# sota-zk-labs/zkp-implementation

Hardware: AMD Instinct MI355X
Metric: G1 MSM scalar-muls/sec (higher is better)
Workload: dtype u32 (unsaturated 28-bit-limb Montgomery, 381-bit Fq; 64-bit accumulate)

## Files before the change

include/zkp_hip.h:

```cpp
#ifndef ZKP_HIP_H
#define ZKP_HIP_H
#include <stddef.h>
#include <stdint.h>

#ifdef __cplusplus
extern "C" {
#endif

#define ZKP_OK 0
#define ZKP_E_ARG (-1)
#define ZKP_E_NOMEM (-2)
#define ZKP_E_DEVICE (-3)
#define ZKP_E_SIZE (-4)

typedef struct zkp_bases zkp_bases;

int zkp_init(int device);
int zkp_init_devices(const int *devices, int n_devices);
int zkp_device_count(void);
int zkp_set_device(int slot);
void zkp_shutdown(void);
const char *zkp_last_error(void);
int zkp_abi_version(void);

void zkp_profile_enable(int on);
void zkp_profile_reset(void);
int zkp_profile_read(const char *name, double *total_ms, uint64_t *count);
int zkp_profile_clock_read(const char *name, uint64_t *cycles, uint64_t *ref_ticks, uint64_t *waves);
int zkp_probe_mad_rate(unsigned launches, double *lane_mads_per_s, double *clock_mhz, double *ms_per_launch);

int zkp_g1_bases_create(const uint64_t *xy, const uint8_t *is_inf, size_t n, zkp_bases **out);
int zkp_g1_bases_create_dev(const void *d_xy, const uint8_t *d_is_inf, size_t n, void *stream, zkp_bases **out);
int zkp_g1_bases_precompute(zkp_bases *b, unsigned window_bits);
size_t zkp_g1_bases_len(const zkp_bases *b);
int zkp_g1_bases_info(const zkp_bases *b, unsigned *window_bits, unsigned *slices);
void zkp_g1_bases_destroy(zkp_bases *b);

int zkp_msm_g1(const zkp_bases *bases, const uint64_t *scalars, size_t n, uint64_t out_xy[12], uint8_t *out_is_inf);
int zkp_msm_g1_dev(const zkp_bases *bases, const void *d_scalars, size_t n, void *stream, uint64_t out_xy[12],
                   uint8_t *out_is_inf);
int zkp_msm_g1_batch_dev(const zkp_bases *bases, const void *const *d_scalars, size_t count, size_t n, void *stream,
                         uint64_t *out_xy, uint8_t *out_is_inf);
int zkp_msm_g1_partial_dev(const zkp_bases *bases, const void *d_scalars, size_t n, void *stream, uint64_t out_xyzz[24]);
int zkp_msm_g1_partial(const zkp_bases *bases, const uint64_t *scalars, size_t n, uint64_t out_xyzz[24]);
int zkp_g1_bases_shard_count(const zkp_bases *b);
int zkp_g1_bases_shard(const zkp_bases *b, size_t i, int *slot, int *device, size_t *offset, size_t *len);
int zkp_msm_g1_sharded_dev(const zkp_bases *bases, const void *const *d_scalars, size_t n, uint64_t out_xy[12],
                           uint8_t *out_is_inf);
int zkp_msm_g1_sharded_dev_after(const zkp_bases *bases, const void *const *d_scalars, void *const *ready_events, size_t n,
                                 uint64_t out_xy[12], uint8_t *out_is_inf);
int zkp_g1_xyzz_sum(const uint64_t *partials, size_t count, uint64_t out_xy[12], uint8_t *out_is_inf);

int zkp_kzg_commit(const zkp_bases *srs, const uint64_t *coeffs, size_t len, uint64_t out_xy[12], uint8_t *out_is_inf);
int zkp_kzg_open(const zkp_bases *srs, const uint64_t *coeffs, size_t len, const uint64_t z[4], uint64_t out_xy[12],
                 uint8_t *out_is_inf, uint64_t out_eval[4]);

int zkp_g1_mul(const uint64_t base_xy[12], uint8_t base_is_inf, const uint64_t scalar[4], uint64_t out_xy[12],
               uint8_t *out_is_inf);
int zkp_g1_fixed_base_mul_dev(const void *d_scalars, size_t n, void *d_out_xy, uint8_t *d_out_is_inf, void *stream);
int zkp_selftest_fq_inverse_dev(const void *d_in, size_t n, int form, void *d_out, void *stream);
int zkp_srs_g1(const uint64_t secret[4], size_t n, uint64_t *out_xy);

int zkp_ntt_fr(uint64_t *data, unsigned log_n, int inverse, const uint64_t *coset );
int zkp_ntt_fr_dev(void *d_data, unsigned log_n, size_t batch, int inverse, const uint64_t *coset, void *stream);

int zkp_ntt_fr_twiddle_dev(void *d_data, size_t rows, size_t cols, size_t row0, unsigned log_n, int inverse, void *stream);

typedef struct {
    unsigned lo_bits, mid_bits;
    size_t mid_stride, hi_stride, batch_stride;
} zkp_ntt_layout;
int zkp_ntt_fr_axis0_dev(const void *d_in, void *d_out, unsigned log_len, size_t cols, int inverse, unsigned tw_log_n,
                         size_t tw_col0, void *stream);
int zkp_ntt_fr_layout_dev(const void *d_in, void *d_out, unsigned log_n, size_t batch, int inverse,
                          const zkp_ntt_layout *in_layout, const zkp_ntt_layout *out_layout, unsigned tw_log_n, size_t tw_row0,
                          void *stream);

#define ZKP_NTT_NATURAL 0
#define ZKP_NTT_K1SLAB 1
#define ZKP_NTT_COLUMNS 2
typedef struct {
    unsigned slots, log_n1, log_n2, chunks;
    size_t r1, r2, cw, slab;
} zkp_ntt_shard_geometry;
int zkp_ntt_fr_sharded_geometry(unsigned log_n, unsigned slots , unsigned chunks,
                                zkp_ntt_shard_geometry *out);
int zkp_ntt_fr_sharded_dev(void *const *d_slabs, unsigned log_n, int inverse, int layout_in, int layout_out, unsigned chunks,
                           void *const *streams);
int zkp_ntt_fr_sharded(uint64_t *data, unsigned log_n, int inverse, const uint64_t *coset );

int zkp_ntt_goldilocks(uint64_t *data, unsigned log_n, int inverse, const uint64_t *coset );
int zkp_ntt_goldilocks_dev(void *d_data, unsigned log_n, size_t batch, int inverse, const uint64_t *coset, void *stream);
int zkp_fri_layer_eval(const uint64_t *coeffs, size_t d, uint64_t coset, unsigned log_D, uint64_t *out);
int zkp_fri_fold(const uint64_t *coeffs, size_t d, uint64_t r, uint64_t *out);

size_t zkp_fri_merkle_node_count(size_t n);
int zkp_fri_merkle_tree(const uint64_t *leaves, size_t n, uint64_t *nodes_out);
int zkp_fri_merkle_tree_dev(const void *d_leaves, size_t n, void *d_nodes, void *stream);
int zkp_fri_challenges(const uint64_t *roots, size_t layers, uint64_t const_val, size_t num_queries, uint64_t *r_out,
                       uint64_t *q_out);
int zkp_fri_prove(const uint64_t *coeffs, size_t d, size_t blowup_factor, size_t num_queries, uint64_t **out_proof,
                  size_t *out_words);
int zkp_fri_verify(const uint64_t *proof, size_t words);
void zkp_free(void *p);

int zkp_fri_layer_eval_fr(const uint64_t *coeffs, size_t d, const uint64_t coset[4], unsigned log_D, uint64_t *out);
int zkp_fri_fold_fr(const uint64_t *coeffs, size_t d, const uint64_t r[4], uint64_t *out);
int zkp_fri_merkle_tree_fr(const uint64_t *leaves, size_t n, uint64_t *nodes_out);
int zkp_fri_merkle_tree_fr_dev(const void *d_leaves, size_t n, void *d_nodes, void *stream);
int zkp_fri_challenges_fr(const uint64_t *roots, size_t layers, const uint64_t const_val[4], size_t num_queries, uint64_t *r_out,
                          uint64_t *q_out);
int zkp_fri_prove_fr(const uint64_t *coeffs, size_t d, size_t blowup_factor, size_t num_queries, uint64_t **out_proof,
                     size_t *out_words);
int zkp_fri_verify_fr(const uint64_t *proof, size_t words);

typedef struct zkp_plonk_transcript zkp_plonk_transcript;
int zkp_plonk_transcript_create(zkp_plonk_transcript **out);
void zkp_plonk_transcript_destroy(zkp_plonk_transcript *t);
int zkp_plonk_transcript_feed(zkp_plonk_transcript *t, const uint64_t xy[12], uint8_t is_inf);
int zkp_plonk_transcript_challenges(zkp_plonk_transcript *t, size_t n, uint64_t *out);

int zkp_poly_mul_fr(const uint64_t *a, size_t la, const uint64_t *b, size_t lb, uint64_t *out);

typedef struct zkp_plonk_prover zkp_plonk_prover;
int zkp_plonk_prover_create(const zkp_bases *srs, unsigned log_n, const uint64_t *const polys[12], const size_t lens[12],
                            const uint64_t k1[4], const uint64_t k2[4], zkp_plonk_prover **out);
void zkp_plonk_prover_destroy(zkp_plonk_prover *p);
int zkp_plonk_round1(zkp_plonk_prover *p, const uint64_t *blinders, uint64_t *out_xy, uint8_t *out_is_inf);
int zkp_plonk_round2(zkp_plonk_prover *p, const uint64_t beta[4], const uint64_t gamma[4], const uint64_t *blinders,
                     uint64_t out_xy[12], uint8_t *out_is_inf);
int zkp_plonk_round3(zkp_plonk_prover *p, const uint64_t alpha[4], uint64_t *out_xy, uint8_t *out_is_inf, size_t *out_degree);
int zkp_plonk_round4(zkp_plonk_prover *p, const uint64_t zeta[4], uint64_t *out_bars);
int zkp_plonk_round5(zkp_plonk_prover *p, const uint64_t v[4], uint64_t *out_xy, uint8_t *out_is_inf);
typedef struct {
    uint64_t commit_xy[9][12];
    uint8_t commit_is_inf[9];
    uint64_t bars[6][4];
    uint64_t u[4];
    uint64_t degree;
} zkp_plonk_proof;
int zkp_plonk_prove(zkp_plonk_prover *p, const uint64_t *blinders, zkp_plonk_proof *out);

int zkp_g2_generator(uint64_t out_xy[24]);
int zkp_g2_mul(const uint64_t q_xy[24], uint8_t q_is_inf, const uint64_t scalar[4], uint64_t out_xy[24], uint8_t *out_is_inf);
int zkp_pairing(const uint64_t p_xy[12], uint8_t p_is_inf, const uint64_t q_xy[24], uint8_t q_is_inf, uint64_t out_fq12[72]);
int zkp_kzg_verify(const uint64_t g2s_xy[24], const uint64_t commit_xy[12], uint8_t commit_is_inf, const uint64_t w_xy[12],
                   uint8_t w_is_inf, const uint64_t y[4], const uint64_t z[4], int *accepted);
int zkp_kzg_batch_verify(const uint64_t g2s_xy[24], size_t n, const uint64_t *commits_xy, const uint8_t *commits_is_inf,
                         const uint64_t *points, const uint64_t *openings_xy, const uint8_t *openings_is_inf,
                         const uint64_t *evals, const uint64_t *r_primes, int *accepted);
int zkp_kzg_aggregate_commitments(const uint64_t *commits_xy, const uint8_t *commits_is_inf, size_t n, const uint64_t challenge[4],
                                  uint64_t out_xy[12], uint8_t *out_is_inf);
int zkp_plonk_verify(zkp_plonk_prover *p, const uint64_t g2s_xy[24], const zkp_plonk_proof *proof, int *accepted);

int zkp_plonk_get_poly(zkp_plonk_prover *p, int which, uint64_t *out, size_t cap_elems, size_t *len);

typedef struct zkp_nova_r1cs zkp_nova_r1cs;
typedef struct {
    const uint64_t *row_ptr;
    const uint32_t *cols;
    const uint64_t *vals;
} zkp_csr;
int zkp_nova_r1cs_create(const zkp_bases *srs, size_t rows, size_t num_vars, size_t num_io, const zkp_csr *a, const zkp_csr *b,
                         const zkp_csr *c, zkp_nova_r1cs **out);
void zkp_nova_r1cs_destroy(zkp_nova_r1cs *r);
typedef struct {
    uint64_t com_e_xy[12];
    uint8_t com_e_is_inf;
    uint64_t u[4];
    uint64_t com_w_xy[12];
    uint8_t com_w_is_inf;
    uint64_t *x;
} zkp_nova_instance;
typedef struct {
    uint64_t r[4];
    uint64_t opening_point[4];
    uint64_t open_e_xy[12];
    uint8_t open_e_is_inf;
    uint64_t eval_e[4];
    uint64_t open_w_xy[12];
    uint8_t open_w_is_inf;
    uint64_t eval_w[4];
} zkp_nova_proof;
int zkp_nova_cross_term_dev(zkp_nova_r1cs *r, const void *d_w1, const uint64_t *x1, const uint64_t u1[4], const void *d_w2,
                            const uint64_t *x2, const uint64_t u2[4], void *d_t, void *stream);
int zkp_nova_fold_witness_dev(zkp_nova_r1cs *r, const uint64_t rr[4], const void *d_e1, const void *d_w1, const void *d_e2,
                              const void *d_w2, const void *d_t, void *d_e_out, void *d_w_out, void *stream);
int zkp_nova_relaxed_residual_dev(zkp_nova_r1cs *r, const void *d_w, const uint64_t *x, const uint64_t u[4], const void *d_e,
                                  void *stream, uint64_t *bad_rows);

typedef struct zkp_nova_transcript zkp_nova_transcript;
int zkp_nova_transcript_create(zkp_nova_transcript **out);
void zkp_nova_transcript_destroy(zkp_nova_transcript *t);
int zkp_nova_transcript_feed(zkp_nova_transcript *t, const uint64_t xy[12], uint8_t is_inf);
int zkp_nova_transcript_feed_scalar(zkp_nova_transcript *t, const uint64_t s[4]);
int zkp_nova_transcript_challenges(zkp_nova_transcript *t, size_t n, uint64_t *out);

int zkp_nova_nifs_prover_dev(zkp_nova_r1cs *r, const void *d_e1, const void *d_w1, const void *d_e2, const void *d_w2,
                             const zkp_nova_instance *fi1, const zkp_nova_instance *fi2, zkp_nova_transcript *t, void *d_e_out,
                             void *d_w_out, void *stream, zkp_nova_instance *out, uint64_t com_t_xy[12], uint8_t *com_t_is_inf,
                             uint64_t r_out[4]);
int zkp_nova_nifs_prover(zkp_nova_r1cs *r, const uint64_t *e1, const uint64_t *w1, const uint64_t *e2, const uint64_t *w2,
                         const zkp_nova_instance *fi1, const zkp_nova_instance *fi2, zkp_nova_transcript *t, uint64_t *e_out,
                         uint64_t *w_out, zkp_nova_instance *out, uint64_t com_t_xy[12], uint8_t *com_t_is_inf, uint64_t r_out[4]);
int zkp_nova_nifs_prove_dev(zkp_nova_r1cs *r, const uint64_t rr[4], const void *d_e, const void *d_w, const zkp_nova_instance *fi,
                            zkp_nova_transcript *t, void *stream, zkp_nova_proof *out);
int zkp_nova_nifs_prove(zkp_nova_r1cs *r, const uint64_t rr[4], const uint64_t *e, const uint64_t *w, const zkp_nova_instance *fi,
                        zkp_nova_transcript *t, zkp_nova_proof *out);
int zkp_nova_nifs_verify(const uint64_t g2s_xy[24], const zkp_nova_proof *proof, const zkp_nova_instance *fi1,
                         const zkp_nova_instance *fi2, const zkp_nova_instance *fi3, const uint64_t com_t_xy[12], uint8_t com_t_is_inf,
                         zkp_nova_transcript *t, int *accepted);

#ifdef __cplusplus
}
#endif
#endif
```

rust/zkp-hip-sys/src/lib.rs:

```rust
#![allow(non_camel_case_types)]
use core::ffi::{c_char, c_void};

pub const ZKP_OK: i32 = 0;
pub const ZKP_E_ARG: i32 = -1;
pub const ZKP_E_NOMEM: i32 = -2;
pub const ZKP_E_DEVICE: i32 = -3;
pub const ZKP_E_SIZE: i32 = -4;

#[repr(C)] pub struct zkp_bases { _private: [u8; 0] }
#[repr(C)] pub struct zkp_plonk_prover { _private: [u8; 0] }
#[repr(C)] pub struct zkp_plonk_transcript { _private: [u8; 0] }
#[repr(C)] pub struct zkp_nova_r1cs { _private: [u8; 0] }
#[repr(C)] pub struct zkp_nova_transcript { _private: [u8; 0] }

#[repr(C)]
pub struct zkp_plonk_proof {
    pub commit_xy: [[u64; 12]; 9],
    pub commit_is_inf: [u8; 9],
    pub bars: [[u64; 4]; 6],
    pub u: [u64; 4],
    pub degree: u64,
}

#[repr(C)]
pub struct zkp_ntt_layout {
    pub lo_bits: u32,
    pub mid_bits: u32,
    pub mid_stride: usize,
    pub hi_stride: usize,
    pub batch_stride: usize,
}

#[repr(C)]
pub struct zkp_ntt_shard_geometry {
    pub slots: u32,
    pub log_n1: u32,
    pub log_n2: u32,
    pub chunks: u32,
    pub r1: usize,
    pub r2: usize,
    pub cw: usize,
    pub slab: usize,
}
#[repr(C)]
pub struct zkp_csr {
    pub row_ptr: *const u64,
    pub cols: *const u32,
    pub vals: *const u64,
}

#[repr(C)]
pub struct zkp_nova_instance {
    pub com_e_xy: [u64; 12],
    pub com_e_is_inf: u8,
    pub u: [u64; 4],
    pub com_w_xy: [u64; 12],
    pub com_w_is_inf: u8,
    pub x: *mut u64,
}

#[repr(C)]
pub struct zkp_nova_proof {
    pub r: [u64; 4],
    pub opening_point: [u64; 4],
    pub open_e_xy: [u64; 12],
    pub open_e_is_inf: u8,
    pub eval_e: [u64; 4],
    pub open_w_xy: [u64; 12],
    pub open_w_is_inf: u8,
    pub eval_w: [u64; 4],
}

pub const ZKP_NTT_NATURAL: i32 = 0;
pub const ZKP_NTT_K1SLAB: i32 = 1;
pub const ZKP_NTT_COLUMNS: i32 = 2;

extern "C" {
    pub fn zkp_init(device: i32) -> i32;
    pub fn zkp_init_devices(devices: *const i32, n_devices: i32) -> i32;
    pub fn zkp_device_count() -> i32;
    pub fn zkp_set_device(slot: i32) -> i32;
    pub fn zkp_shutdown();
    pub fn zkp_last_error() -> *const c_char;
    pub fn zkp_abi_version() -> i32;
    pub fn zkp_profile_enable(on: i32);
    pub fn zkp_profile_reset();
    pub fn zkp_profile_read(name: *const c_char, total_ms: *mut f64, count: *mut u64) -> i32;
    pub fn zkp_profile_clock_read(name: *const c_char, cycles: *mut u64, ref_ticks: *mut u64, waves: *mut u64) -> i32;
    pub fn zkp_probe_mad_rate(launches: u32, lane_mads_per_s: *mut f64, clock_mhz: *mut f64, ms_per_launch: *mut f64) -> i32;
    pub fn zkp_g1_bases_create(xy: *const u64, is_inf: *const u8, n: usize, out: *mut *mut zkp_bases) -> i32;
    pub fn zkp_g1_bases_create_dev(d_xy: *const c_void, d_is_inf: *const u8, n: usize, stream: *mut c_void, out: *mut *mut zkp_bases) -> i32;
    pub fn zkp_g1_bases_precompute(b: *mut zkp_bases, window_bits: u32) -> i32;
    pub fn zkp_g1_bases_len(b: *const zkp_bases) -> usize;
    pub fn zkp_g1_bases_info(b: *const zkp_bases, window_bits: *mut u32, slices: *mut u32) -> i32;
    pub fn zkp_g1_bases_destroy(b: *mut zkp_bases);
    pub fn zkp_msm_g1(bases: *const zkp_bases, scalars: *const u64, n: usize, out_xy: *mut u64, out_is_inf: *mut u8) -> i32;
    pub fn zkp_msm_g1_dev(bases: *const zkp_bases, d_scalars: *const c_void, n: usize, stream: *mut c_void, out_xy: *mut u64, out_is_inf: *mut u8) -> i32;
    pub fn zkp_msm_g1_batch_dev(bases: *const zkp_bases, d_scalars: *const *const c_void, count: usize, n: usize, stream: *mut c_void, out_xy: *mut u64, out_is_inf: *mut u8) -> i32;
    pub fn zkp_msm_g1_partial_dev(bases: *const zkp_bases, d_scalars: *const c_void, n: usize, stream: *mut c_void, out_xyzz: *mut u64) -> i32;
    pub fn zkp_msm_g1_partial(bases: *const zkp_bases, scalars: *const u64, n: usize, out_xyzz: *mut u64) -> i32;
    pub fn zkp_g1_bases_shard_count(b: *const zkp_bases) -> i32;
    pub fn zkp_g1_bases_shard(b: *const zkp_bases, i: usize, slot: *mut i32, device: *mut i32, offset: *mut usize, len: *mut usize) -> i32;
    pub fn zkp_msm_g1_sharded_dev(bases: *const zkp_bases, d_scalars: *const *const c_void, n: usize, out_xy: *mut u64, out_is_inf: *mut u8) -> i32;
    pub fn zkp_msm_g1_sharded_dev_after(bases: *const zkp_bases, d_scalars: *const *const c_void, ready_events: *mut *mut c_void, n: usize, out_xy: *mut u64, out_is_inf: *mut u8) -> i32;
    pub fn zkp_g1_xyzz_sum(partials: *const u64, count: usize, out_xy: *mut u64, out_is_inf: *mut u8) -> i32;
    pub fn zkp_kzg_commit(srs: *const zkp_bases, coeffs: *const u64, len: usize, out_xy: *mut u64, out_is_inf: *mut u8) -> i32;
    pub fn zkp_kzg_open(srs: *const zkp_bases, coeffs: *const u64, len: usize, z: *const u64, out_xy: *mut u64, out_is_inf: *mut u8, out_eval: *mut u64) -> i32;
    pub fn zkp_g1_mul(base_xy: *const u64, base_is_inf: u8, scalar: *const u64, out_xy: *mut u64, out_is_inf: *mut u8) -> i32;
    pub fn zkp_g1_fixed_base_mul_dev(d_scalars: *const c_void, n: usize, d_out_xy: *mut c_void, d_out_is_inf: *mut u8, stream: *mut c_void) -> i32;
    pub fn zkp_selftest_fq_inverse_dev(d_in: *const c_void, n: usize, form: i32, d_out: *mut c_void, stream: *mut c_void) -> i32;
    pub fn zkp_srs_g1(secret: *const u64, n: usize, out_xy: *mut u64) -> i32;
    pub fn zkp_ntt_fr(data: *mut u64, log_n: u32, inverse: i32, coset: *const u64) -> i32;
    pub fn zkp_ntt_fr_dev(d_data: *mut c_void, log_n: u32, batch: usize, inverse: i32, coset: *const u64, stream: *mut c_void) -> i32;
    pub fn zkp_ntt_fr_twiddle_dev(d_data: *mut c_void, rows: usize, cols: usize, row0: usize, log_n: u32, inverse: i32, stream: *mut c_void) -> i32;
    pub fn zkp_ntt_fr_axis0_dev(d_in: *const c_void, d_out: *mut c_void, log_len: u32, cols: usize, inverse: i32, tw_log_n: u32, tw_col0: usize, stream: *mut c_void) -> i32;
    pub fn zkp_ntt_fr_layout_dev(d_in: *const c_void, d_out: *mut c_void, log_n: u32, batch: usize, inverse: i32, in_layout: *const zkp_ntt_layout, out_layout: *const zkp_ntt_layout, tw_log_n: u32, tw_row0: usize, stream: *mut c_void) -> i32;
    pub fn zkp_ntt_fr_sharded_geometry(log_n: u32, slots: u32, chunks: u32, out: *mut zkp_ntt_shard_geometry) -> i32;
    pub fn zkp_ntt_fr_sharded_dev(d_slabs: *mut *mut c_void, log_n: u32, inverse: i32, layout_in: i32, layout_out: i32, chunks: u32, streams: *mut *mut c_void) -> i32;
    pub fn zkp_ntt_fr_sharded(data: *mut u64, log_n: u32, inverse: i32, coset: *const u64) -> i32;
    pub fn zkp_ntt_goldilocks(data: *mut u64, log_n: u32, inverse: i32, coset: *const u64) -> i32;
    pub fn zkp_ntt_goldilocks_dev(d_data: *mut c_void, log_n: u32, batch: usize, inverse: i32, coset: *const u64, stream: *mut c_void) -> i32;
    pub fn zkp_fri_layer_eval(coeffs: *const u64, d: usize, coset: u64, log_D: u32, out: *mut u64) -> i32;
    pub fn zkp_fri_fold(coeffs: *const u64, d: usize, r: u64, out: *mut u64) -> i32;
    pub fn zkp_fri_merkle_node_count(n: usize) -> usize;
    pub fn zkp_fri_merkle_tree(leaves: *const u64, n: usize, nodes_out: *mut u64) -> i32;
    pub fn zkp_fri_merkle_tree_dev(d_leaves: *const c_void, n: usize, d_nodes: *mut c_void, stream: *mut c_void) -> i32;
    pub fn zkp_fri_challenges(roots: *const u64, layers: usize, const_val: u64, num_queries: usize, r_out: *mut u64, q_out: *mut u64) -> i32;
    pub fn zkp_fri_prove(coeffs: *const u64, d: usize, blowup_factor: usize, num_queries: usize, out_proof: *mut *mut u64, out_words: *mut usize) -> i32;
    pub fn zkp_fri_verify(proof: *const u64, words: usize) -> i32;
    pub fn zkp_free(p: *mut c_void);
    pub fn zkp_fri_layer_eval_fr(coeffs: *const u64, d: usize, coset: *const u64, log_D: u32, out: *mut u64) -> i32;
    pub fn zkp_fri_fold_fr(coeffs: *const u64, d: usize, r: *const u64, out: *mut u64) -> i32;
    pub fn zkp_fri_merkle_tree_fr(leaves: *const u64, n: usize, nodes_out: *mut u64) -> i32;
    pub fn zkp_fri_merkle_tree_fr_dev(d_leaves: *const c_void, n: usize, d_nodes: *mut c_void, stream: *mut c_void) -> i32;
    pub fn zkp_fri_challenges_fr(roots: *const u64, layers: usize, const_val: *const u64, num_queries: usize, r_out: *mut u64, q_out: *mut u64) -> i32;
    pub fn zkp_fri_prove_fr(coeffs: *const u64, d: usize, blowup_factor: usize, num_queries: usize, out_proof: *mut *mut u64, out_words: *mut usize) -> i32;
    pub fn zkp_fri_verify_fr(proof: *const u64, words: usize) -> i32;
    pub fn zkp_plonk_transcript_create(out: *mut *mut zkp_plonk_transcript) -> i32;
    pub fn zkp_plonk_transcript_destroy(t: *mut zkp_plonk_transcript);
    pub fn zkp_plonk_transcript_feed(t: *mut zkp_plonk_transcript, xy: *const u64, is_inf: u8) -> i32;
    pub fn zkp_plonk_transcript_challenges(t: *mut zkp_plonk_transcript, n: usize, out: *mut u64) -> i32;
    pub fn zkp_poly_mul_fr(a: *const u64, la: usize, b: *const u64, lb: usize, out: *mut u64) -> i32;
    pub fn zkp_plonk_prover_create(srs: *const zkp_bases, log_n: u32, polys: *const *const u64, lens: *const usize, k1: *const u64, k2: *const u64, out: *mut *mut zkp_plonk_prover) -> i32;
    pub fn zkp_plonk_prover_destroy(p: *mut zkp_plonk_prover);
    pub fn zkp_plonk_round1(p: *mut zkp_plonk_prover, blinders: *const u64, out_xy: *mut u64, out_is_inf: *mut u8) -> i32;
    pub fn zkp_plonk_round2(p: *mut zkp_plonk_prover, beta: *const u64, gamma: *const u64, blinders: *const u64, out_xy: *mut u64, out_is_inf: *mut u8) -> i32;
    pub fn zkp_plonk_round3(p: *mut zkp_plonk_prover, alpha: *const u64, out_xy: *mut u64, out_is_inf: *mut u8, out_degree: *mut usize) -> i32;
    pub fn zkp_plonk_round4(p: *mut zkp_plonk_prover, zeta: *const u64, out_bars: *mut u64) -> i32;
    pub fn zkp_plonk_round5(p: *mut zkp_plonk_prover, v: *const u64, out_xy: *mut u64, out_is_inf: *mut u8) -> i32;
    pub fn zkp_plonk_prove(p: *mut zkp_plonk_prover, blinders: *const u64, out: *mut zkp_plonk_proof) -> i32;
    pub fn zkp_g2_generator(out_xy: *mut u64) -> i32;
    pub fn zkp_g2_mul(q_xy: *const u64, q_is_inf: u8, scalar: *const u64, out_xy: *mut u64, out_is_inf: *mut u8) -> i32;
    pub fn zkp_pairing(p_xy: *const u64, p_is_inf: u8, q_xy: *const u64, q_is_inf: u8, out_fq12: *mut u64) -> i32;
    pub fn zkp_kzg_verify(g2s_xy: *const u64, commit_xy: *const u64, commit_is_inf: u8, w_xy: *const u64, w_is_inf: u8, y: *const u64, z: *const u64, accepted: *mut i32) -> i32;
    pub fn zkp_kzg_batch_verify(g2s_xy: *const u64, n: usize, commits_xy: *const u64, commits_is_inf: *const u8, points: *const u64, openings_xy: *const u64, openings_is_inf: *const u8, evals: *const u64, r_primes: *const u64, accepted: *mut i32) -> i32;
    pub fn zkp_kzg_aggregate_commitments(commits_xy: *const u64, commits_is_inf: *const u8, n: usize, challenge: *const u64, out_xy: *mut u64, out_is_inf: *mut u8) -> i32;
    pub fn zkp_plonk_verify(p: *mut zkp_plonk_prover, g2s_xy: *const u64, proof: *const zkp_plonk_proof, accepted: *mut i32) -> i32;
    pub fn zkp_plonk_get_poly(p: *mut zkp_plonk_prover, which: i32, out: *mut u64, cap_elems: usize, len: *mut usize) -> i32;
    pub fn zkp_nova_r1cs_create(srs: *const zkp_bases, rows: usize, num_vars: usize, num_io: usize, a: *const zkp_csr, b: *const zkp_csr, c: *const zkp_csr, out: *mut *mut zkp_nova_r1cs) -> i32;
    pub fn zkp_nova_r1cs_destroy(r: *mut zkp_nova_r1cs);
    pub fn zkp_nova_cross_term_dev(r: *mut zkp_nova_r1cs, d_w1: *const c_void, x1: *const u64, u1: *const u64, d_w2: *const c_void, x2: *const u64, u2: *const u64, d_t: *mut c_void, stream: *mut c_void) -> i32;
    pub fn zkp_nova_fold_witness_dev(r: *mut zkp_nova_r1cs, rr: *const u64, d_e1: *const c_void, d_w1: *const c_void, d_e2: *const c_void, d_w2: *const c_void, d_t: *const c_void, d_e_out: *mut c_void, d_w_out: *mut c_void, stream: *mut c_void) -> i32;
    pub fn zkp_nova_relaxed_residual_dev(r: *mut zkp_nova_r1cs, d_w: *const c_void, x: *const u64, u: *const u64, d_e: *const c_void, stream: *mut c_void, bad_rows: *mut u64) -> i32;
    pub fn zkp_nova_transcript_create(out: *mut *mut zkp_nova_transcript) -> i32;
    pub fn zkp_nova_transcript_destroy(t: *mut zkp_nova_transcript);
    pub fn zkp_nova_transcript_feed(t: *mut zkp_nova_transcript, xy: *const u64, is_inf: u8) -> i32;
    pub fn zkp_nova_transcript_feed_scalar(t: *mut zkp_nova_transcript, s: *const u64) -> i32;
    pub fn zkp_nova_transcript_challenges(t: *mut zkp_nova_transcript, n: usize, out: *mut u64) -> i32;
    pub fn zkp_nova_nifs_prover_dev(r: *mut zkp_nova_r1cs, d_e1: *const c_void, d_w1: *const c_void, d_e2: *const c_void, d_w2: *const c_void, fi1: *const zkp_nova_instance, fi2: *const zkp_nova_instance, t: *mut zkp_nova_transcript, d_e_out: *mut c_void, d_w_out: *mut c_void, stream: *mut c_void, out: *mut zkp_nova_instance, com_t_xy: *mut u64, com_t_is_inf: *mut u8, r_out: *mut u64) -> i32;
    pub fn zkp_nova_nifs_prover(r: *mut zkp_nova_r1cs, e1: *const u64, w1: *const u64, e2: *const u64, w2: *const u64, fi1: *const zkp_nova_instance, fi2: *const zkp_nova_instance, t: *mut zkp_nova_transcript, e_out: *mut u64, w_out: *mut u64, out: *mut zkp_nova_instance, com_t_xy: *mut u64, com_t_is_inf: *mut u8, r_out: *mut u64) -> i32;
    pub fn zkp_nova_nifs_prove_dev(r: *mut zkp_nova_r1cs, rr: *const u64, d_e: *const c_void, d_w: *const c_void, fi: *const zkp_nova_instance, t: *mut zkp_nova_transcript, stream: *mut c_void, out: *mut zkp_nova_proof) -> i32;
    pub fn zkp_nova_nifs_prove(r: *mut zkp_nova_r1cs, rr: *const u64, e: *const u64, w: *const u64, fi: *const zkp_nova_instance, t: *mut zkp_nova_transcript, out: *mut zkp_nova_proof) -> i32;
    pub fn zkp_nova_nifs_verify(g2s_xy: *const u64, proof: *const zkp_nova_proof, fi1: *const zkp_nova_instance, fi2: *const zkp_nova_instance, fi3: *const zkp_nova_instance, com_t_xy: *const u64, com_t_is_inf: u8, t: *mut zkp_nova_transcript, accepted: *mut i32) -> i32;
}

pub fn last_error() -> String {
    unsafe { std::ffi::CStr::from_ptr(zkp_last_error()).to_string_lossy().into_owned() }
}
```

zkp-implementation_amd/build.py:

```python
#!/usr/bin/env python3
import os
import subprocess
import sys

HERE = os.path.dirname(os.path.abspath(__file__))
SRC = os.path.join(HERE, "csrc")
OUT = os.path.join(HERE, "libzkp_hip.so")
SOURCES = ["api.hip"]
DEPS = ["api.hip", "ff.hpp", "fq28.hpp", "fq28_inv.hpp", "fr29.hpp", "fr29_mul2_asm.inc", "fq28_mul_asm.inc", "fq28_mul2x_asm.inc", "fq28_sqr_asm.inc", "fq28_mul2_asm.inc", "g1.hpp", "g1_28.hpp", "msm.hpp", "ntt.hpp", "plonk.hpp",
        "plonk_host.inc", "ntt_sharded.inc", "fri.hpp", "fri_host.inc", "fri_fr.hpp", "fri_fr_host.inc", "transcript_host.hpp", "pairing_host.hpp", "verify_host.inc", "host_ff.hpp", "kzg_host.hpp", "host_threads.hpp", "msm_plan.hpp", "msm_host.inc", "nova.hpp", "nova_host.inc", "dev_res.hpp",
        os.path.join("..", "..", "include", "zkp_hip.h")]


STAMP = OUT + ".srchash"


def source_hash():
    import hashlib
    h = hashlib.sha256()
    for d in DEPS:
        path = os.path.join(SRC, d)
        if os.path.exists(path):
            h.update(d.encode())
            h.update(open(path, "rb").read())
    return h.hexdigest()


def stale():
    if not os.path.exists(OUT) or not os.path.exists(STAMP):
        return True
    return open(STAMP).read().strip() != source_hash()


def build(force=False, verbose=False, defines=(), out=None):
    variant = out is not None
    if not variant and not force and not stale():
        return OUT
    hipcc = os.environ.get("HIPCC", "/opt/rocm/bin/hipcc")
    cmd = [hipcc, "--offload-arch=gfx950", "-O3", "-std=c++17", "-fPIC", "-shared",
           "-Wno-unused-result", "-pthread"] + [f"-D{d}" for d in defines] + [os.path.join(SRC, s) for s in SOURCES] + ["-o", out or OUT]
    if verbose:
        print(" ".join(cmd))
    subprocess.check_call(cmd)
    if not variant:
        with open(STAMP, "w") as f:
            f.write(source_hash())
    return out or OUT


if __name__ == "__main__":
    defs = [a[2:] for a in sys.argv[1:] if a.startswith("-D")]
    outs = [a[2:] for a in sys.argv[1:] if a.startswith("-o")]
    print(build(force="--force" in sys.argv, verbose=True, defines=defs, out=outs[0] if outs else None))
```

zkp-implementation_amd/csrc/api.hip:

```cpp
#include <hip/hip_runtime.h>

#include <algorithm>
#include <array>
#include <atomic>
#include <chrono>
#include <cstdio>
#include <cstdlib>
#include <cstring>
#include <condition_variable>
#include <functional>
#include <map>
#include <memory>
#include <mutex>
#include <new>
#include <string>
#include <thread>
#include <tuple>
#include <vector>

#include "../../include/zkp_hip.h"
#include "host_ff.hpp"
#include "kzg_host.hpp"
#include "msm.hpp"
#include "ntt.hpp"
#include "plonk.hpp"
#include "nova.hpp"
#include "fri.hpp"
#include "transcript_host.hpp"
#include "pairing_host.hpp"

using namespace zkp;
using namespace zkp::host;

namespace {

thread_local std::string g_err;

int fail(int code, const std::string& msg) {
    g_err = msg;
    return code;
}

int on_exception() noexcept {
    try {
        throw;
    } catch (const std::bad_alloc&) {
        try { g_err = "host allocation failed"; } catch (...) {}
        return ZKP_E_NOMEM;
    } catch (const std::exception& e) {
        try { g_err = std::string("internal error: ") + e.what(); } catch (...) {}
        return ZKP_E_DEVICE;
    } catch (...) {
        try { g_err = "internal error: unknown exception"; } catch (...) {}
        return ZKP_E_DEVICE;
    }
}
#define ZKP_CATCH_INT catch (...) { return on_exception(); }

#define HIPCHK(expr)                                                                                        \
    do {                                                                                                    \
        hipError_t e_ = (expr);                                                                             \
        if (e_ != hipSuccess)                                                                               \
            return fail(e_ == hipErrorOutOfMemory ? ZKP_E_NOMEM : ZKP_E_DEVICE,                             \
                        std::string(#expr) + ": " + hipGetErrorString(e_));                                 \
    } while (0)
int hip_fail(hipError_t e, const std::string& what) {
    return fail(e == hipErrorOutOfMemory ? ZKP_E_NOMEM : ZKP_E_DEVICE, what + hipGetErrorString(e));
}
#define HIPCHK_BARE(expr)                            \
    do {                                             \
        hipError_t e_ = (expr);                      \
        if (e_ != hipSuccess) return hip_fail(e_, ""); \
    } while (0)
#define ZCHK(expr)             \
    do {                       \
        int r_ = (expr);       \
        if (r_ != ZKP_OK) return r_; \
    } while (0)

#include "host_threads.hpp"
#include "dev_res.hpp"
static_assert(ZKP_HOST_THREADS_E_DEVICE == ZKP_E_DEVICE && ZKP_HOST_THREADS_OK == ZKP_OK, "host_threads.hpp error codes");

class DeviceWorkers {
    struct W {
        std::thread th;
        std::mutex mu;
        std::condition_variable cv;
        const std::function<void()>* job = nullptr;
        bool busy = false, quit = false;
    };
    std::mutex run_mu;
    std::vector<W*> ws;
    static void loop(W* w) {
        std::unique_lock<std::mutex> lk(w->mu);
        for (;;) {
            w->cv.wait(lk, [&] { return w->job != nullptr || w->quit; });
            if (w->quit) return;
            const std::function<void()>* j = w->job;
            lk.unlock();
            (*j)();
            lk.lock();
            w->job = nullptr;
            w->busy = false;
            w->cv.notify_all();
        }
    }

public:
    void run(const std::vector<std::function<void()>>& jobs) {
        std::lock_guard<std::mutex> one(run_mu);
        while (ws.size() < jobs.size()) {
            W* w = new W;
            w->th = std::thread(loop, w);
            ws.push_back(w);
        }
        for (size_t i = 0; i < jobs.size(); i++) {
            std::lock_guard<std::mutex> lk(ws[i]->mu);
            ws[i]->job = &jobs[i];
            ws[i]->busy = true;
            ws[i]->cv.notify_all();
        }
        for (size_t i = 0; i < jobs.size(); i++) {
            std::unique_lock<std::mutex> lk(ws[i]->mu);
            ws[i]->cv.wait(lk, [&] { return !ws[i]->busy; });
        }
    }
    void stop() {
        std::lock_guard<std::mutex> one(run_mu);
        for (W* w : ws) {
            {
                std::lock_guard<std::mutex> lk(w->mu);
                w->quit = true;
                w->cv.notify_all();
            }
            w->th.join();
            delete w;
        }
        ws.clear();
    }
};
DeviceWorkers g_workers;
void device_workers_stop() { g_workers.stop(); }

struct ProfRec {
    const char* name = nullptr;
    hipEvent_t a = nullptr;
    Event own_a, b;
    double host_ms = 0;
};
std::atomic<int> g_prof_on{0};
struct Ctx;
Ctx& ctx();
std::vector<ProfRec>& prof_records();
hipStream_t& prof_last_stream();

struct ProfScope {
    ProfRec rec;
    hipStream_t st;
    bool on;
    ProfScope(const char* name, hipStream_t s, bool chain = false) : st(s), on(false) {
        const int level = g_prof_on.load(std::memory_order_relaxed);
        on = level == 1 || (level == 2 && std::strcmp(name, "msm_accumulate") == 0);
        if (!on) return;
        if (level == 2) chain = false;
        rec.name = name;
        std::vector<ProfRec>& recs = prof_records();
        if (chain && !recs.empty() && recs.back().b && prof_last_stream() == s) {
            rec.a = recs.back().b;
            if (rec.b.make(hipEventDefault) != hipSuccess) on = false;
            return;
        }
        if (rec.own_a.make(hipEventDefault) != hipSuccess || rec.b.make(hipEventDefault) != hipSuccess) { on = false; return; }
        rec.a = rec.own_a;
        (void)hipEventRecord(rec.a, st);
    }
    ~ProfScope() {
        if (!on) return;
        (void)hipEventRecord(rec.b, st);
        prof_records().push_back(std::move(rec));
        prof_last_stream() = st;
    }
};
void prof_host(const char* name, double ms) {
    if (g_prof_on.load(std::memory_order_relaxed) != 1) return;
    ProfRec r;
    r.name = name;
    r.host_ms = ms;
    prof_records().push_back(std::move(r));
}

template <class F> struct HostField;
template <> struct HostField<Fr> {
    typedef HFr H;
    static Fr dev(const HFr& x) { Fr r; std::memcpy(r.l, x.l, 32); return r; }
    static Fr29 tw(const HFr& x) {
        HFr y = x;
        for (int i = 0; i < 5; i++) y = y.dbl();
        Fr29 r;
        for (int i = 0; i < 9; i++) {
            const int bit = 29 * i, w = bit >> 6, sh = bit & 63;
            unsigned __int128 v = y.l[w];
            if (w + 1 < 4) v |= (unsigned __int128)y.l[w + 1] << 64;
            r.l[i] = (uint32_t)(v >> sh) & MASK29;
        }
        return r;
    }
    static HFr root(unsigned log_n) { return fr_root_of_unity(log_n); }
    static constexpr int ID = 0;
};
template <> struct HostField<Gl> {
    typedef HGl H;
    static Gl dev(const HGl& x) { return Gl{x.from_mont().l[0]}; }
    static Gl tw(const HGl& x) { return dev(x); }
    static HGl root(unsigned log_n) { return gl_root_of_unity(log_n); }
    static constexpr int ID = 1;
};

template <class F>
struct NttPlan {
    unsigned log_n = 0;
    int passes = 0;
    int r[4] = {0, 0, 0, 0};
    const typename NttOps<F>::W* tw[4] = {nullptr, nullptr, nullptr, nullptr};
    TypedBuf<typename NttOps<F>::W> inter_lo, inter_hi;
    TypedBuf<typename NttOps<F>::W> inter_lo_ninv;
    uint32_t h = 0;
    TypedBuf<typename NttOps<F>::W> direct[4];
    TypedBuf<F> tw_matrix[2];
    typename HostField<F>::H n_inv;
};

template <class F>
struct CosetCache {
    bool valid = false;
    unsigned log_n = 0;
    int inverse = 0;
    uint64_t key[4] = {0, 0, 0, 0};
    uint64_t ckey[4] = {0, 0, 0, 0};
    TypedBuf<typename NttOps<F>::W> lo, hi;
    uint32_t h = 0;
};

struct Ctx {
    int slot = 0;
    int device = -1;
    std::mutex mu;
    Stream stream;
    Stream copy_stream;
    Stream sort_stream;
    Stream xstream;
    Event ws_event;
    hipStream_t ws_stream = nullptr;
    bool ws_pending = false;
    std::vector<ProfRec> prof;
    hipStream_t prof_last = nullptr;
    std::map<std::pair<int, int>, DevBuf> radix_tw[2];
    std::map<std::pair<unsigned, int>, NttPlan<Fr>> plans_fr;
    std::map<std::pair<unsigned, int>, NttPlan<Gl>> plans_gl;
    static constexpr int COSET_WAYS = 8;
    CosetCache<Fr> coset_fr[COSET_WAYS];
    CosetCache<Gl> coset_gl[COSET_WAYS];
    unsigned coset_victim[2] = {0, 0};
    DevBuf ntt_scratch;
    std::map<std::pair<unsigned, int>, DevBuf> axis0_tw[2];
    DevBuf scalars, over;
    TypedBuf<uint32_t> digits, sorted, counts, start, perm, result;
    TypedBuf<uint2> entries;
    TypedBuf<uint4> pieces, buckets, parts, pyr1, odd0, odd1;
    PinnedBuf host_result;
    PinnedBuf fri_small;
    DevBuf fb_table;
    bool fb_ready = false;
    DevBuf tmp;
    Event copy_event;
    std::vector<Event> copy_events;
    Event ev_sort[2], ev_acc[2], ev_begin;
    DevBuf fri_arena, fri_meta;
    DevBuf clk;
    uint32_t tail_max_waves = 2048;
    DevBuf xchg_a, xchg_b;
    std::vector<Event> xev;
    bool peers_enabled = false;
    ~Ctx() {
        std::lock_guard<std::mutex> lk(mu);
        (void)hipSetDevice(device);
        (void)hipDeviceSynchronize();
    }
};
enum { CLK_MSM_ACCUMULATE = 0, CLK_MAD_PROBE = 1, CLK_NTT_FR = 2, CLK_NTT_GL = 3, CLK_COUNT = 4 };
static const char* const kClkNames[CLK_COUNT] = {"msm_accumulate", "mad_probe", "ntt_fr_pass", "ntt_gl_pass"};

struct Runtime {
    std::mutex mu;
    std::vector<std::unique_ptr<Ctx>> slots;
    bool multi = false;
};
Runtime& g_rt = *new Runtime;

ClkRec* clk_record(int which) {
    if (!g_prof_on.load(std::memory_order_relaxed)) return nullptr;
    Ctx& c = ctx();
    if (!c.clk.p) {
        if (c.clk.ensure(sizeof(ClkRec) * CLK_COUNT) != ZKP_OK) return nullptr;
        if (hipMemset(c.clk.p, 0, sizeof(ClkRec) * CLK_COUNT) != hipSuccess) return nullptr;
    }
    return reinterpret_cast<ClkRec*>(c.clk.p) + which;
}
thread_local int t_slot = -1;
thread_local Ctx* t_cur = nullptr;
Ctx& ctx() { return *t_cur; }
std::vector<ProfRec>& prof_records() { return ctx().prof; }
hipStream_t& prof_last_stream() { return ctx().prof_last; }

int create_slot_locked(int device);

struct CtxScope {
    Ctx* prev;
    std::unique_lock<std::mutex> lk;
    int rc = ZKP_OK;
    int restore_device = -1;
    explicit CtxScope(int slot) : prev(t_cur) {
        Ctx* c = nullptr;
        {
            std::lock_guard<std::mutex> g(g_rt.mu);
            if (g_rt.slots.empty()) {
                int dev = 0;
                if (hipGetDevice(&dev) != hipSuccess) dev = 0;
                rc = create_slot_locked(dev);
                if (rc != ZKP_OK) return;
            }
            const int s = slot >= 0 ? slot : (t_slot >= 0 ? t_slot : 0);
            if (s >= (int)g_rt.slots.size()) {
                rc = fail(ZKP_E_ARG, "device slot out of range (zkp_init_devices / zkp_set_device)");
                return;
            }
            c = g_rt.slots[(size_t)s].get();
        }
        lk = std::unique_lock<std::mutex>(c->mu);
        t_cur = c;
        int cur = -1;
        if (hipGetDevice(&cur) == hipSuccess && cur != c->device) restore_device = cur;
        if (cur != c->device && hipSetDevice(c->device) != hipSuccess) rc = fail(ZKP_E_DEVICE, "hipSetDevice failed");
    }
    ~CtxScope() {
        t_cur = prev;
        if (restore_device >= 0 && !prev) (void)hipSetDevice(restore_device);
    }
};
#define CTX_ENTER(slot)           \
    CtxScope ctx_scope_(slot);    \
    if (ctx_scope_.rc != ZKP_OK) return ctx_scope_.rc

struct WsOrder {
    hipStream_t st;
    explicit WsOrder(hipStream_t s) : st(s) {
        Ctx& c = ctx();
        if (c.ws_pending && c.ws_stream != st) (void)hipStreamWaitEvent(st, c.ws_event, 0);
    }
    ~WsOrder() {
        Ctx& c = ctx();
        if (c.ws_event.make(hipEventDisableTiming) != hipSuccess) {
            (void)hipStreamSynchronize(st);
            c.ws_pending = false;
            return;
        }
        (void)hipEventRecord(c.ws_event, st);
        c.ws_stream = st;
        c.ws_pending = true;
    }
};

template <class K>
int allow_big_lds(K kernel) {
    HIPCHK(hipFuncSetAttribute(reinterpret_cast<const void*>(kernel), hipFuncAttributeMaxDynamicSharedMemorySize,
                               160 * 1024));
    return ZKP_OK;
}

template <class F>
std::map<std::pair<unsigned, int>, NttPlan<F>>& plan_map();
template <> std::map<std::pair<unsigned, int>, NttPlan<Fr>>& plan_map<Fr>() { return ctx().plans_fr; }
template <> std::map<std::pair<unsigned, int>, NttPlan<Gl>>& plan_map<Gl>() { return ctx().plans_gl; }
template <class F> CosetCache<F>* coset_cache();
template <> CosetCache<Fr>* coset_cache<Fr>() { return ctx().coset_fr; }
template <> CosetCache<Gl>* coset_cache<Gl>() { return ctx().coset_gl; }

template <class F>
int make_pow_table(const typename HostField<F>::H& base, const typename HostField<F>::H& c, uint32_t shift,
                   uint32_t count, typename NttOps<F>::W* out, hipStream_t st) {
    hipLaunchKernelGGL(pow_table_kernel<F>, dim3((count + 255) / 256), dim3(256), 0, st, HostField<F>::dev(base),
                       HostField<F>::dev(c), shift, count, out);
    HIPCHK(hipGetLastError());
    return ZKP_OK;
}

template <class F>
int build_pow_table(const typename HostField<F>::H& w, uint32_t count, DevBuf* out, hipStream_t st) {
    typedef typename NttOps<F>::W W;
    DevBuf tab;
    ZCHK(tab.ensure(sizeof(W) * count));
    int rc = make_pow_table<F>(w, HostField<F>::H::one(), 0, count, static_cast<W*>(tab.p), st);
    if (rc == ZKP_OK) {
        const hipError_t e = hipStreamSynchronize(st);
        if (e != hipSuccess) rc = hip_fail(e, "hipStreamSynchronize(st): ");
    }
    if (rc != ZKP_OK) {
        (void)hipStreamSynchronize(st);
        return rc;
    }
    *out = std::move(tab);
    return ZKP_OK;
}

template <class F>
int get_radix_table(int log_r, int inverse, const typename NttOps<F>::W** out, hipStream_t st) {
    typedef typename HostField<F>::H H;
    typedef typename NttOps<F>::W W;
    auto& m = ctx().radix_tw[HostField<F>::ID];
    auto key = std::make_pair(log_r, inverse);
    auto it = m.find(key);
    if (it == m.end()) {
        uint32_t count = log_r ? (1u << (log_r - 1)) : 1u;
        H w = HostField<F>::root((unsigned)log_r);
        if (inverse) w = w.inverse();
        DevBuf tab;
        ZCHK(build_pow_table<F>(w, count, &tab, st));
        it = m.emplace(key, std::move(tab)).first;
    }
    *out = static_cast<const W*>(it->second.p);
    return ZKP_OK;
}

static unsigned pass0_matrix_max_log() {
    static const unsigned v = [] {
        const char* e = getenv("ZKP_NTT_TW_MATRIX_MAX_LOG");
        return e ? (unsigned)std::min(30, std::max(0, atoi(e))) : 24u;
    }();
    return v;
}

template <class F>
int get_plan(unsigned log_n, int inverse, bool allow_wide, NttPlan<F>** out, hipStream_t st) {
    typedef typename HostField<F>::H H;
    typedef typename NttOps<F>::W W;
    auto& m = plan_map<F>();
    auto key = std::make_pair(log_n, inverse | (allow_wide ? 2 : 0));
    auto it = m.find(key);
    if (it == m.end()) {
        NttPlan<F> pl;
        pl.log_n = log_n;
        pl.passes = (int)log_n <= NttOps<F>::MAX_TILE_LOG ? 1 : (int)((log_n + NttOps<F>::MAX_PASS_LOG - 1) / NttOps<F>::MAX_PASS_LOG);
        if (pl.passes > 1 && allow_wide && !getenv("ZKP_NTT_NO_WIDE_PASS")) {
            for (int maxr = NttOps<F>::MAX_PASS_LOG + 1; maxr <= NttOps<F>::WIDE_PASS_LOG; maxr++) {
                if ((int)log_n > NttOps<F>::wide_max_log_n(maxr)) break;
                const int wide = (int)((log_n + maxr - 1) / maxr);
                if (wide < pl.passes) pl.passes = wide;
            }
        }
        int base = (int)log_n / pl.passes, rem = (int)log_n % pl.passes;
        for (int p = 0; p < pl.passes; p++) pl.r[p] = base + (p < rem ? 1 : 0);
        for (int p = 0; p < pl.passes; p++) ZCHK(get_radix_table<F>(pl.r[p], inverse, &pl.tw[p], st));
        H w = HostField<F>::root(log_n);
        if (inverse) w = w.inverse();
        H two = H::from_u64(2), ninv = H::one(), half = two.inverse();
        for (unsigned i = 0; i < log_n; i++) ninv = ninv * half;
        pl.n_inv = ninv;
        if (pl.passes > 1) {
            pl.h = (log_n + 1) / 2;
            uint32_t nlo = 1u << pl.h, nhi = 1u << (log_n - pl.h);
            auto build = [&]() -> int {
                ZCHK(pl.inter_lo.ensure(sizeof(W) * nlo));
                ZCHK(pl.inter_hi.ensure(sizeof(W) * nhi));
                ZCHK(make_pow_table<F>(w, H::one(), 0, nlo, pl.inter_lo.get(), st));
                ZCHK(make_pow_table<F>(w, H::one(), pl.h, nhi, pl.inter_hi.get(), st));
                if (inverse) {
                    ZCHK(pl.inter_lo_ninv.ensure(sizeof(W) * nlo));
                    ZCHK(make_pow_table<F>(w, ninv, 0, nlo, pl.inter_lo_ninv.get(), st));
                }
                unsigned outer = pl.r[0];
                for (int p = 1; p + 1 < pl.passes; p++) {
                    const unsigned log_m = log_n - outer;
// ... 824 lines not shown
    }
    *out = b;
    return ZKP_OK;
} ZKP_CATCH_INT

int zkp_g1_bases_precompute(zkp_bases* b, unsigned window_bits) try {
    if (!b) return fail(ZKP_E_ARG, "null argument");
    if (b->shards.empty()) return precompute_single(b, window_bits);
    size_t nmax = 0, expanded = 0;
    for (const auto& sh : b->shards) nmax = std::max(nmax, sh->n), expanded += sh->pre_c ? 1 : 0;
    if (window_bits == 0) {
        if (expanded == b->shards.size() || !(window_bits = auto_window_bits(nmax))) return ZKP_OK;
        if (expanded) window_bits = b->shards[0]->pre_req ? b->shards[0]->pre_req : window_bits;
    }
    ZCHK(for_each_shard(b, [&](size_t i) { return precompute_single(b->shards[i].get(), window_bits, true); }));
    std::vector<uint8_t> was(b->shards.size());
    for (size_t i = 0; i < b->shards.size(); i++) was[i] = b->shards[i]->pre_c ? 1 : 0;
    const int rc = for_each_shard(b, [&](size_t i) { return precompute_single(b->shards[i].get(), window_bits); });
    if (rc != ZKP_OK) {
        const std::string why = zkp_last_error();
        bool mixed = false;
        for (size_t i = 0; i < b->shards.size(); i++)
            if (!was[i] && b->shards[i]->pre_c && unexpand_single(b->shards[i].get()) != ZKP_OK) mixed = true;
        return fail(rc, why + (mixed ? " -- and a finished chunk could not be rolled back: the handle is expanded in part (still usable)"
                                     : " -- every chunk is back to the plain points"));
    }
    return ZKP_OK;
} ZKP_CATCH_INT

size_t zkp_g1_bases_len(const zkp_bases* b) { return b ? b->n : 0; }

int zkp_g1_bases_info(const zkp_bases* b, unsigned* window_bits, unsigned* slices) try {
    if (!b || !window_bits || !slices) return fail(ZKP_E_ARG, "null argument");
    const zkp_bases* s = b->shards.empty() ? b : b->shards[0].get();
    if (!s) return fail(ZKP_E_ARG, "empty handle");
    *window_bits = s->pre_req;
    *slices = s->pre_c ? s->pre_planes : 0;
    return ZKP_OK;
} ZKP_CATCH_INT

void zkp_g1_bases_destroy(zkp_bases* b) {
    if (!b) return;
    for (auto& s : b->shards) zkp_g1_bases_destroy(s.release());
    DeviceRestore restore;
    (void)hipSetDevice(b->device);
    delete b;
}

}

namespace {

const char* const kShardedDev = "bases are sharded over several devices: device-pointer entries take single-device bases "
                                "(zkp_set_device + zkp_g1_bases_create*); use zkp_msm_g1 with host scalars";

int msm_host_scalars(const zkp_bases* bases, const uint64_t* scalars, size_t n, HXyzz* r) {
    CTX_ENTER(bases->slot);
    hipStream_t st = g_rt.multi ? ctx().stream : nullptr;
    WsOrder ord(st);
    if (n > bases->n) return fail(ZKP_E_SIZE, "more scalars than bases (kzg/src/scheme.rs:86)");
    *r = HXyzz::infinity();
    if (!n) return ZKP_OK;
    ZCHK(ctx().scalars.ensure(32 * n));
    const Fr* d_sc = reinterpret_cast<const Fr*>(ctx().scalars.p);
    const bool shared = bases->pre_c != 0;
    if (shared && n >= (1u << 19)) {
        ZCHK(ctx().copy_stream.ensure(hipStreamNonBlocking));
        ZCHK(ctx().copy_event.ensure(hipEventDisableTiming));
        const MsmFeed feed{scalars, ctx().copy_stream, ctx().copy_event, msm_feed_ranges(n)};
        return msm_partial_batch(bases, &d_sc, 1, n, st, r, &feed);
    }
    HIPCHK(hipMemcpyAsync(ctx().scalars.p, scalars, 32 * n, hipMemcpyHostToDevice, st));
    return msm_partial(bases, d_sc, n, st, r);
}

int msm_host_scalars_any(const zkp_bases* bases, const uint64_t* scalars, size_t n, HXyzz* r) {
    if (bases->shards.empty()) return msm_host_scalars(bases, scalars, n, r);
    if (n > bases->n) return fail(ZKP_E_SIZE, "more scalars than bases (kzg/src/scheme.rs:86)");
    const size_t k = bases->shards.size();
    std::vector<HXyzz> part(k, HXyzz::infinity());
    ZCHK(for_each_shard(bases, [&](size_t i) {
        const size_t lo = bases->shard_off[i];
        if (lo >= n) return (int)ZKP_OK;
        const size_t len = std::min(bases->shards[i]->n, n - lo);
        return msm_host_scalars(bases->shards[i].get(), scalars + 4 * lo, len, &part[i]);
    }));
    HXyzz acc = HXyzz::infinity();
    for (size_t i = 0; i < k; i++) acc = acc.add(part[i]);
    *r = acc;
    return ZKP_OK;
}

}

extern "C" {

int zkp_msm_g1_partial_dev(const zkp_bases* bases, const void* d_scalars, size_t n, void* stream, uint64_t out_xyzz[24]) try {
    if (!bases || !out_xyzz || (n && !d_scalars)) return fail(ZKP_E_ARG, "null argument");
    if (!bases->shards.empty()) return fail(ZKP_E_ARG, kShardedDev);
    CTX_ENTER(bases->slot);
    WsOrder ord(reinterpret_cast<hipStream_t>(stream));
    HXyzz r;
    ZCHK(msm_partial(bases, reinterpret_cast<const Fr*>(d_scalars), n, reinterpret_cast<hipStream_t>(stream), &r));
    r.store(out_xyzz);
    return ZKP_OK;
} ZKP_CATCH_INT

int zkp_msm_g1_dev(const zkp_bases* bases, const void* d_scalars, size_t n, void* stream, uint64_t out_xy[12],
                   uint8_t* out_is_inf) try {
    if (!bases || !out_xy || !out_is_inf || (n && !d_scalars)) return fail(ZKP_E_ARG, "null argument");
    if (!bases->shards.empty()) return fail(ZKP_E_ARG, kShardedDev);
    CTX_ENTER(bases->slot);
    WsOrder ord(reinterpret_cast<hipStream_t>(stream));
    HXyzz r;
    ZCHK(msm_partial(bases, reinterpret_cast<const Fr*>(d_scalars), n, reinterpret_cast<hipStream_t>(stream), &r));
    r.to_affine(out_xy, out_is_inf);
    return ZKP_OK;
} ZKP_CATCH_INT

int zkp_msm_g1(const zkp_bases* bases, const uint64_t* scalars, size_t n, uint64_t out_xy[12], uint8_t* out_is_inf) try {
    if (!bases || !out_xy || !out_is_inf || (n && !scalars)) return fail(ZKP_E_ARG, "null argument");
    HXyzz r;
    ZCHK(msm_host_scalars_any(bases, scalars, n, &r));
    r.to_affine(out_xy, out_is_inf);
    return ZKP_OK;
} ZKP_CATCH_INT

int zkp_g1_bases_shard_count(const zkp_bases* b) { return !b ? 0 : b->shards.empty() ? 1 : (int)b->shards.size(); }

int zkp_g1_bases_shard(const zkp_bases* b, size_t i, int* slot, int* device, size_t* offset, size_t* len) try {
    if (!b || !slot || !device || !offset || !len) return fail(ZKP_E_ARG, "null argument");
    if (i >= (size_t)zkp_g1_bases_shard_count(b)) return fail(ZKP_E_ARG, "chunk index out of range");
    const zkp_bases* s = b->shards.empty() ? b : b->shards[i].get();
    *slot = s->slot;
    *device = s->device;
    *offset = b->shards.empty() ? 0 : b->shard_off[i];
    *len = s->n;
    return ZKP_OK;
} ZKP_CATCH_INT

static int order_after_producer(hipStream_t st, void* ready_event) {
    if (ready_event) HIPCHK(hipStreamWaitEvent(st, reinterpret_cast<hipEvent_t>(ready_event), 0));
    else HIPCHK(hipDeviceSynchronize());
    return ZKP_OK;
}

int zkp_msm_g1_sharded_dev_after(const zkp_bases* bases, const void* const* d_scalars, void* const* ready_events, size_t n,
                                 uint64_t out_xy[12], uint8_t* out_is_inf) try {
    if (!bases || !out_xy || !out_is_inf || (n && !d_scalars)) return fail(ZKP_E_ARG, "null argument");
    if (n > bases->n) return fail(ZKP_E_SIZE, "more scalars than bases (kzg/src/scheme.rs:86)");
    HXyzz acc = HXyzz::infinity();
    if (bases->shards.empty()) {
        if (n) {
            if (!d_scalars[0]) return fail(ZKP_E_ARG, "null scalar pointer");
            CTX_ENTER(bases->slot);
            hipStream_t st = g_rt.multi ? ctx().stream : nullptr;
            ZCHK(order_after_producer(st, ready_events ? ready_events[0] : nullptr));
            WsOrder ord(st);
            ZCHK(msm_partial(bases, reinterpret_cast<const Fr*>(d_scalars[0]), n, st, &acc));
        }
    } else {
        const size_t k = bases->shards.size();
        for (size_t i = 0; i < k; i++)
            if (bases->shard_off[i] < n && bases->shards[i]->n && !d_scalars[i]) return fail(ZKP_E_ARG, "null scalar pointer for a chunk in use");
        std::vector<HXyzz> part(k, HXyzz::infinity());
        ZCHK(for_each_shard(bases, [&](size_t i) {
            const size_t lo = bases->shard_off[i];
            const zkp_bases* sh = bases->shards[i].get();
            if (lo >= n || !sh->n) return (int)ZKP_OK;
            const size_t len = std::min(sh->n, n - lo);
            CTX_ENTER(sh->slot);
            ZCHK(order_after_producer(ctx().stream, ready_events ? ready_events[i] : nullptr));
            WsOrder ord(ctx().stream);
            return msm_partial(sh, reinterpret_cast<const Fr*>(d_scalars[i]), len, ctx().stream, &part[i]);
        }));
        for (size_t i = 0; i < k; i++) acc = acc.add(part[i]);
    }
    acc.to_affine(out_xy, out_is_inf);
    return ZKP_OK;
} ZKP_CATCH_INT

int zkp_msm_g1_sharded_dev(const zkp_bases* bases, const void* const* d_scalars, size_t n, uint64_t out_xy[12],
                           uint8_t* out_is_inf) {
    return zkp_msm_g1_sharded_dev_after(bases, d_scalars, nullptr, n, out_xy, out_is_inf);
}

int zkp_msm_g1_partial(const zkp_bases* bases, const uint64_t* scalars, size_t n, uint64_t out_xyzz[24]) try {
    if (!bases || !out_xyzz || (n && !scalars)) return fail(ZKP_E_ARG, "null argument");
    HXyzz r;
    ZCHK(msm_host_scalars_any(bases, scalars, n, &r));
    r.store(out_xyzz);
    return ZKP_OK;
} ZKP_CATCH_INT

int zkp_msm_g1_batch_dev(const zkp_bases* bases, const void* const* d_scalars, size_t count, size_t n, void* stream,
                         uint64_t* out_xy, uint8_t* out_is_inf) try {
    if (!bases || (count && (!d_scalars || !out_xy || !out_is_inf))) return fail(ZKP_E_ARG, "null argument");
    if (!bases->shards.empty()) return fail(ZKP_E_ARG, kShardedDev);
    CTX_ENTER(bases->slot);
    WsOrder ord(reinterpret_cast<hipStream_t>(stream));
    std::vector<HXyzz> r(count);
    ZCHK(msm_partial_batch(bases, reinterpret_cast<const Fr* const*>(d_scalars), count, n, reinterpret_cast<hipStream_t>(stream),
                           r.data()));
    std::vector<HFq> prefix(count);
    HFq run = HFq::one();
    for (size_t m = 0; m < count; m++) {
        prefix[m] = run;
        if (!r[m].is_inf()) run = run * r[m].zzz;
    }
    HFq inv = run.inverse();
    for (size_t m = count; m-- > 0;) {
        if (r[m].is_inf()) {
            std::memset(out_xy + 12 * m, 0, 96);
            out_is_inf[m] = 1;
            continue;
        }
        const HFq zi3 = inv * prefix[m];
        inv = inv * r[m].zzz;
        HFq zi2 = zi3 * r[m].zz;
        zi2 = zi2.sqr();
        (r[m].x * zi2).store(out_xy + 12 * m);
        (r[m].y * zi3).store(out_xy + 12 * m + 6);
        out_is_inf[m] = 0;
    }
    return ZKP_OK;
} ZKP_CATCH_INT

int zkp_g1_xyzz_sum(const uint64_t* partials, size_t count, uint64_t out_xy[12], uint8_t* out_is_inf) try {
    if ((count && !partials) || !out_xy || !out_is_inf) return fail(ZKP_E_ARG, "null argument");
    HXyzz acc = HXyzz::infinity();
    for (size_t i = 0; i < count; i++) acc = acc.add(HXyzz::load(partials + 24 * i));
    acc.to_affine(out_xy, out_is_inf);
    return ZKP_OK;
} ZKP_CATCH_INT

int zkp_kzg_commit(const zkp_bases* srs, const uint64_t* coeffs, size_t len, uint64_t out_xy[12], uint8_t* out_is_inf) try {
    if (!srs || !out_xy || !out_is_inf || (len && !coeffs)) return fail(ZKP_E_ARG, "null argument");
    KzgScheme scheme(srs);
    KzgCommitment cm;
    int rc = scheme.commit(coeffs, len, &cm);
    if (rc == ZKP_E_SIZE && g_err.empty()) g_err = "SRS shorter than the polynomial (kzg/src/scheme.rs:86)";
    if (rc != ZKP_OK) return rc;
    std::memcpy(out_xy, cm.p.xy, 96);
    *out_is_inf = cm.p.infinity;
    return ZKP_OK;
} ZKP_CATCH_INT

int kzg_open_device(const zkp_bases* srs, const uint64_t* coeffs, size_t len, const uint64_t z[4], uint64_t out_xy[12],
                    uint8_t* out_is_inf, uint64_t out_eval[4]);

int zkp_kzg_open(const zkp_bases* srs, const uint64_t* coeffs, size_t len, const uint64_t z[4], uint64_t out_xy[12],
                 uint8_t* out_is_inf, uint64_t out_eval[4]) try {
    if (!srs || !out_xy || !out_is_inf || !out_eval || !z || (len && !coeffs)) return fail(ZKP_E_ARG, "null argument");
    if (len == 0) return fail(ZKP_E_ARG, "open of an empty polynomial (kzg/src/scheme.rs:112 expects at least 1)");
    if (len >= 4096) return kzg_open_device(srs, coeffs, len, z, out_xy, out_is_inf, out_eval);
    KzgScheme scheme(srs);
    KzgOpening op;
    int rc = scheme.open(coeffs, len, z, &op);
    if (rc != ZKP_OK) return rc;
    std::memcpy(out_xy, op.p.xy, 96);
    *out_is_inf = op.p.infinity;
    op.eval.store(out_eval);
    return ZKP_OK;
} ZKP_CATCH_INT

int zkp_g1_mul(const uint64_t base_xy[12], uint8_t base_is_inf, const uint64_t scalar[4], uint64_t out_xy[12],
               uint8_t* out_is_inf) try {
    if (!base_xy || !scalar || !out_xy || !out_is_inf) return fail(ZKP_E_ARG, "null argument");
    HFr k = HFr::load(scalar).from_mont();
    HXyzz r = HXyzz::from_affine(base_xy, base_is_inf != 0).mul(k.l);
    r.to_affine(out_xy, out_is_inf);
    return ZKP_OK;
} ZKP_CATCH_INT

static int fixed_base_mul_locked(const void* d_scalars, size_t n, void* d_out_xy, uint8_t* d_out_is_inf, hipStream_t st) {
    ZCHK(ensure_fixed_base_table(st));
    hipLaunchKernelGGL(g1_fixed_base_kernel, dim3((unsigned)((n + MSM_THREADS - 1) / MSM_THREADS)), dim3(MSM_THREADS), 0,
                       st, reinterpret_cast<const Fr*>(d_scalars), (uint64_t)n,
                       reinterpret_cast<const uint4*>(ctx().fb_table.p), reinterpret_cast<uint4*>(d_out_xy), d_out_is_inf);
    HIPCHK(hipGetLastError());
    return ZKP_OK;
}

int zkp_g1_fixed_base_mul_dev(const void* d_scalars, size_t n, void* d_out_xy, uint8_t* d_out_is_inf, void* stream) try {
    if (n && (!d_scalars || !d_out_xy)) return fail(ZKP_E_ARG, "null argument");
    CTX_ENTER(-1);
    if (!n) return ZKP_OK;
    WsOrder ord(reinterpret_cast<hipStream_t>(stream));
    return fixed_base_mul_locked(d_scalars, n, d_out_xy, d_out_is_inf, reinterpret_cast<hipStream_t>(stream));
} ZKP_CATCH_INT

int zkp_selftest_fq_inverse_dev(const void* d_in, size_t n, int form, void* d_out, void* stream) try {
    if (n && (!d_in || !d_out)) return fail(ZKP_E_ARG, "null argument");
    if (form != 0 && form != 1) return fail(ZKP_E_ARG, "form must be 0 (12 x u32, radix 2^384) or 1 (14 x 28 bit + 2 pad words, radix 2^392)");
    CTX_ENTER(-1);
    if (!n) return ZKP_OK;
    hipLaunchKernelGGL(fq_inverse_selftest_kernel, dim3((unsigned)((n + MSM_THREADS - 1) / MSM_THREADS)), dim3(MSM_THREADS), 0,
                       reinterpret_cast<hipStream_t>(stream), reinterpret_cast<const uint32_t*>(d_in), reinterpret_cast<uint32_t*>(d_out),
                       (uint64_t)n, form);
    HIPCHK(hipGetLastError());
    return ZKP_OK;
} ZKP_CATCH_INT

int zkp_srs_g1(const uint64_t secret[4], size_t n, uint64_t* out_xy) try {
    if (!secret || (n && !out_xy)) return fail(ZKP_E_ARG, "null argument");
    if (!n) return ZKP_OK;
    std::vector<uint64_t> pw(4 * n);
    HFr s = HFr::load(secret), cur = HFr::one();
    for (size_t i = 0; i < n; i++) {
        cur.store(&pw[4 * i]);
        cur = cur * s;
    }
    CTX_ENTER(-1);
    WsOrder ord(nullptr);
    ZCHK(ctx().tmp.ensure(32 * n + 96 * n));
    char* d = reinterpret_cast<char*>(ctx().tmp.p);
    HIPCHK(hipMemcpy(d, pw.data(), 32 * n, hipMemcpyHostToDevice));
    ZCHK(fixed_base_mul_locked(d, n, d + 32 * n, nullptr, nullptr));
    HIPCHK(hipMemcpy(out_xy, d + 32 * n, 96 * n, hipMemcpyDeviceToHost));
    return ZKP_OK;
} ZKP_CATCH_INT

}
bool ntt_should_shard(unsigned log_n);
int ntt_fr_sharded_host(uint64_t* data, unsigned log_n, int inverse, const uint64_t* coset);
extern "C" {
int zkp_ntt_fr(uint64_t* data, unsigned log_n, int inverse, const uint64_t* coset) try {
    if (ntt_should_shard(log_n)) return ntt_fr_sharded_host(data, log_n, inverse, coset);
    return ntt_host_entry<Fr>(data, log_n, inverse, coset);
} ZKP_CATCH_INT
int zkp_ntt_goldilocks(uint64_t* data, unsigned log_n, int inverse, const uint64_t* coset) try {
    return ntt_host_entry<Gl>(data, log_n, inverse, coset);
} ZKP_CATCH_INT
int zkp_ntt_fr_dev(void* d_data, unsigned log_n, size_t batch, int inverse, const uint64_t* coset, void* stream) try {
    if (!d_data) return fail(ZKP_E_ARG, "data is null");
    CTX_ENTER(-1);
    WsOrder ord(reinterpret_cast<hipStream_t>(stream));
    return run_ntt<Fr>(reinterpret_cast<Fr*>(d_data), log_n, batch, inverse, coset, reinterpret_cast<hipStream_t>(stream));
} ZKP_CATCH_INT
int zkp_ntt_goldilocks_dev(void* d_data, unsigned log_n, size_t batch, int inverse, const uint64_t* coset, void* stream) try {
    if (!d_data) return fail(ZKP_E_ARG, "data is null");
    CTX_ENTER(-1);
    WsOrder ord(reinterpret_cast<hipStream_t>(stream));
    return run_ntt<Gl>(reinterpret_cast<Gl*>(d_data), log_n, batch, inverse, coset, reinterpret_cast<hipStream_t>(stream));
} ZKP_CATCH_INT

int zkp_ntt_fr_twiddle_dev(void* d_data, size_t rows, size_t cols, size_t row0, unsigned log_n, int inverse, void* stream) try {
    if (!d_data) return fail(ZKP_E_ARG, "data is null");
    if (log_n > 32 || log_n == 0) return fail(ZKP_E_ARG, "log_n out of range");
    if ((uint64_t)(row0 + rows - 1) * (cols - 1) >= (1ull << log_n) && rows && cols)
        return fail(ZKP_E_ARG, "twiddle exponent (row0 + rows - 1) * (cols - 1) must stay below n");
    CTX_ENTER(-1);
    if (!rows || !cols) return ZKP_OK;
    hipStream_t st = reinterpret_cast<hipStream_t>(stream);
    WsOrder ord(st);
    PowTab<Fr> tab;
    HFr w = fr_root_of_unity(log_n);
    ZCHK(get_coset_tables<Fr>(log_n, inverse ? 1 : 0, w.l, HFr::one(), &tab, st));
    const uint64_t total = (uint64_t)rows * cols;
    hipLaunchKernelGGL(twiddle_rows_kernel<Fr>, dim3((unsigned)((total + 255) / 256)), dim3(256), 0, st,
                       reinterpret_cast<Fr*>(d_data), (uint64_t)rows, (uint64_t)cols, (uint64_t)row0, tab);
    HIPCHK(hipGetLastError());
    return ZKP_OK;
} ZKP_CATCH_INT

int zkp_ntt_fr_axis0_dev(const void* d_in, void* d_out, unsigned log_len, size_t cols, int inverse, unsigned tw_log_n,
                         size_t tw_col0, void* stream) try {
    if (!d_in || !d_out) return fail(ZKP_E_ARG, "data is null");
    CTX_ENTER(-1);
    hipStream_t st = reinterpret_cast<hipStream_t>(stream);
    WsOrder ord(st);
    return run_ntt_axis0<Fr>(reinterpret_cast<const Fr*>(d_in), reinterpret_cast<Fr*>(d_out), log_len, cols, inverse, tw_log_n,
                             (uint64_t)tw_col0, st);
} ZKP_CATCH_INT

int zkp_ntt_fr_layout_dev(const void* d_in, void* d_out, unsigned log_n, size_t batch, int inverse, const zkp_ntt_layout* in_layout,
                          const zkp_ntt_layout* out_layout, unsigned tw_log_n, size_t tw_row0, void* stream) try {
    if (!d_in || !d_out) return fail(ZKP_E_ARG, "data is null");
    if (log_n > 32) return fail(ZKP_E_ARG, "log_n > 32");
    NttRemap rin, rout;
    const zkp_ntt_layout* ls[2] = {in_layout, out_layout};
    NttRemap* rs[2] = {&rin, &rout};
    for (int i = 0; i < 2; i++) {
        std::memset(rs[i], 0, sizeof(NttRemap));
        if (!ls[i]) continue;
        if (ls[i]->lo_bits + ls[i]->mid_bits > log_n || ls[i]->lo_bits < 2)
            return fail(ZKP_E_ARG, "layout: lo_bits must be >= 2 (16-byte runs of four elements) and lo_bits + mid_bits <= log_n");
        rs[i]->on = 1;
        rs[i]->lo_bits = ls[i]->lo_bits;
        rs[i]->mid_bits = ls[i]->mid_bits;
        rs[i]->mid_stride = ls[i]->mid_stride;
        rs[i]->hi_stride = ls[i]->hi_stride;
        rs[i]->batch_stride = ls[i]->batch_stride;
    }
    if (d_in == d_out && (in_layout || out_layout))
        return fail(ZKP_E_ARG, "a transform with a gathered or scattered layout cannot run in place");
    CTX_ENTER(-1);
    hipStream_t st = reinterpret_cast<hipStream_t>(stream);
    WsOrder ord(st);
    NttIo io;
    io.in_remap = in_layout ? &rin : nullptr;
    io.out_remap = out_layout ? &rout : nullptr;
    io.tw_log_n = tw_log_n;
    io.tw_row0 = (uint64_t)tw_row0;
    return run_ntt<Fr>(reinterpret_cast<const Fr*>(d_in), reinterpret_cast<Fr*>(d_out), log_n, batch, inverse, nullptr, st, &io);
} ZKP_CATCH_INT

int zkp_fri_layer_eval(const uint64_t* coeffs, size_t d, uint64_t coset, unsigned log_D, uint64_t* out) try {
    if ((d && !coeffs) || !out) return fail(ZKP_E_ARG, "null argument");
    if (log_D > 32) return fail(ZKP_E_ARG, "log_D > 32");
    const size_t D = (size_t)1 << log_D;
    if (d > D) return fail(ZKP_E_ARG, "more coefficients than domain points");
    CTX_ENTER(-1);
    WsOrder ord(nullptr);
    ZCHK(ctx().tmp.ensure(8 * D));
    HIPCHK(hipMemsetAsync(ctx().tmp.p, 0, 8 * D, nullptr));
    if (d) HIPCHK(hipMemcpyAsync(ctx().tmp.p, coeffs, 8 * d, hipMemcpyHostToDevice, nullptr));
    ZCHK(run_ntt<Gl>(reinterpret_cast<Gl*>(ctx().tmp.p), log_D, 1, 0, &coset, nullptr));
    HIPCHK(hipMemcpyAsync(out, ctx().tmp.p, 8 * D, hipMemcpyDeviceToHost, nullptr));
    HIPCHK(hipStreamSynchronize(nullptr));
    return ZKP_OK;
} ZKP_CATCH_INT

}

namespace {
__global__ void fri_fold_kernel(const uint64_t* c, uint64_t d, uint64_t r, uint64_t* out) {
    uint64_t j = (uint64_t)blockIdx.x * blockDim.x + threadIdx.x;
    if (2 * j >= d) return;
    Gl v{c[2 * j]};
    if (2 * j + 1 < d) v = v + Gl{r} * Gl{c[2 * j + 1]};
    out[j] = v.v;
}
}

extern "C" {

int zkp_fri_fold(const uint64_t* coeffs, size_t d, uint64_t r, uint64_t* out) try {
    if (d && (!coeffs || !out)) return fail(ZKP_E_ARG, "null argument");
    if (!d) return ZKP_OK;
    CTX_ENTER(-1);
    WsOrder ord(nullptr);
    const size_t m = (d + 1) / 2;
    ZCHK(ctx().tmp.ensure(8 * d + 8 * m));
    uint64_t* dc = reinterpret_cast<uint64_t*>(ctx().tmp.p);
    HIPCHK(hipMemcpyAsync(dc, coeffs, 8 * d, hipMemcpyHostToDevice, nullptr));
    HGl rr = HGl::load(&r).from_mont();
    hipLaunchKernelGGL(fri_fold_kernel, dim3((unsigned)((m + 255) / 256)), dim3(256), 0, nullptr, dc, (uint64_t)d, rr.l[0],
                       dc + d);
    HIPCHK(hipGetLastError());
    HIPCHK(hipMemcpyAsync(out, dc + d, 8 * m, hipMemcpyDeviceToHost, nullptr));
    HIPCHK(hipStreamSynchronize(nullptr));
    return ZKP_OK;
} ZKP_CATCH_INT

int zkp_poly_mul_fr(const uint64_t* a, size_t la, const uint64_t* b, size_t lb, uint64_t* out) try {
    if (la == 0 || lb == 0) return ZKP_OK;
    if (!a || !b || !out) return fail(ZKP_E_ARG, "null argument");
    const size_t lo = la + lb - 1;
    unsigned log_n = 0;
    while (((size_t)1 << log_n) < lo) log_n++;
    const size_t n = (size_t)1 << log_n;
    CTX_ENTER(-1);
    WsOrder ord(nullptr);
    ZCHK(ctx().tmp.ensure(2 * 32 * n));
    char* d = reinterpret_cast<char*>(ctx().tmp.p);
    HIPCHK(hipMemsetAsync(d, 0, 2 * 32 * n, nullptr));
    HIPCHK(hipMemcpyAsync(d, a, 32 * la, hipMemcpyHostToDevice, nullptr));
    HIPCHK(hipMemcpyAsync(d + 32 * n, b, 32 * lb, hipMemcpyHostToDevice, nullptr));
    ZCHK(run_ntt<Fr>(reinterpret_cast<Fr*>(d), log_n, 2, 0, nullptr, nullptr));
    hipLaunchKernelGGL(pointwise_mul_kernel<Fr>, dim3((unsigned)((n + 255) / 256)), dim3(256), 0, nullptr,
                       reinterpret_cast<const Fr*>(d), reinterpret_cast<const Fr*>(d + 32 * n), reinterpret_cast<Fr*>(d),
                       (uint64_t)n);
    HIPCHK(hipGetLastError());
    ZCHK(run_ntt<Fr>(reinterpret_cast<Fr*>(d), log_n, 1, 1, nullptr, nullptr));
    HIPCHK(hipMemcpyAsync(out, d, 32 * lo, hipMemcpyDeviceToHost, nullptr));
    HIPCHK(hipStreamSynchronize(nullptr));
    return ZKP_OK;
} ZKP_CATCH_INT

}

#include "ntt_sharded.inc"
#include "plonk_host.inc"
#include "fri_host.inc"
#include "verify_host.inc"
#include "nova_host.inc"
#include "fri_fr.hpp"
#include "fri_fr_host.inc"
```

zkp-implementation_amd/csrc/msm.hpp:

```cpp
#pragma once
#include "g1.hpp"
#include "g1_28.hpp"
#include "fq28_inv.hpp"
#include "msm_plan.hpp"

namespace zkp {

constexpr int MSM_THREADS = 256;
constexpr int ACC_THREADS = 256;
#define ZKP_AT(f, o) offsetof(MsmGeom, f) == o
static_assert(sizeof(MsmGeom) == 152 && ZKP_AT(c, 0) && ZKP_AT(nwin, 4) && ZKP_AT(nb, 8) && ZKP_AT(nchunk, 12) && ZKP_AT(n, 16) && ZKP_AT(chunk, 24) &&
              ZKP_AT(ns, 32) && ZKP_AT(plane_stride, 40) && ZKP_AT(nslice, 48) && ZKP_AT(shared, 52) && ZKP_AT(run_limit, 56) && ZKP_AT(piece, 60) &&
              ZKP_AT(resume, 64) && ZKP_AT(off, 68) && ZKP_AT(interleave, 140) && ZKP_AT(split_log, 144) && ZKP_AT(more, 148), "MsmGeom layout");
#undef ZKP_AT
static_assert(sizeof(SortGeom) == 8 && offsetof(SortGeom, lo_bits) == 0 && offsetof(SortGeom, nhi) == 4, "SortGeom layout");

ZKP_DEV uint64_t bucket_cap(const MsmGeom& g) { return (uint64_t)g.nwin * g.nb; }

#ifdef ZKP_MSM_CHECK
__device__ uint32_t g_msm_check[32];
ZKP_DEV bool msm_check_fail(int cls, uint32_t v0, uint32_t v1) {
    if (atomicAdd(&g_msm_check[cls * 4], 1u) == 0) { g_msm_check[cls * 4 + 1] = v0; g_msm_check[cls * 4 + 2] = v1; }
    return true;
}
#endif
struct DigitSources {
    const Fr* scalars[MSM_MAX_BATCH];
};
__global__ __launch_bounds__(MSM_THREADS) void msm_digits_kernel(DigitSources src, const uint8_t* __restrict__ base_inf, MsmGeom g,
                                                                uint32_t nwin1, uint32_t* __restrict__ digits) {
    const uint64_t i = (uint64_t)blockIdx.x * MSM_THREADS + threadIdx.x;
    if (i >= g.ns) return;
    const uint32_t win_off = blockIdx.y * nwin1;
    Fr k = from_mont(src.scalars[blockIdx.y][i]);
    const bool skip = base_inf != nullptr && base_inf[i] != 0;
    uint32_t carry = 0;
    for (uint32_t w = 0; w < nwin1; w++) {
        const uint32_t lo = g.off[w], width = (uint32_t)g.off[w + 1] - lo;
        const uint32_t limb = lo >> 5, sh = lo & 31;
        uint64_t v = 0;
#pragma unroll
        for (int q = 0; q < 8; q++) {
            if (q == (int)limb) v |= (uint64_t)k.l[q];
            if (q == (int)limb + 1) v |= (uint64_t)k.l[q] << 32;
        }
        uint32_t u = ((uint32_t)(v >> sh) & ((1u << width) - 1)) + carry;
        uint32_t enc;
        if (u > (1u << (width - 1))) {
            enc = (((1u << width) - u) << 1) | 1u;
            carry = 1;
        } else {
            enc = u << 1;
            carry = 0;
        }
        digits[(uint64_t)(win_off + w) * g.ns + i] = skip ? 0u : enc;
    }
}


ZKP_DEV void wave_exclusive_scan(const uint32_t* cnt, uint32_t* base, uint32_t nbins, uint32_t lane) {
    const uint32_t per = (nbins + 63) / 64;
    const uint32_t b0 = lane * per < nbins ? lane * per : nbins;
    const uint32_t b1 = b0 + per < nbins ? b0 + per : nbins;
    uint32_t sum = 0;
    for (uint32_t k = b0; k < b1; k++) sum += cnt[k];
    uint32_t inc = sum;
#pragma unroll
    for (int off = 1; off < 64; off <<= 1) {
        const uint32_t t = __shfl_up(inc, off);
        if (lane >= (uint32_t)off) inc += t;
    }
    uint32_t run = inc - sum;
    for (uint32_t k = b0; k < b1; k++) {
        const uint32_t v = cnt[k];
        base[k] = run;
        run += v;
    }
    if (lane == 63) base[nbins] = run;
}

__global__ __launch_bounds__(1024) void msm_parthist_kernel(const uint32_t* __restrict__ digits, MsmGeom g, SortGeom sg,
                                                            uint32_t* __restrict__ cntA) {
    __shared__ uint32_t h[SORT_MAX_PART];
    const uint32_t q = blockIdx.x, w = blockIdx.y;
    for (uint32_t k = threadIdx.x; k < sg.nhi; k += blockDim.x) h[k] = 0;
    __syncthreads();
    const uint64_t begin = (uint64_t)q * g.chunk;
    const uint64_t end = begin + g.chunk < g.n ? begin + g.chunk : g.n;
    const uint32_t* d = digits + (uint64_t)w * g.n;
    const uint64_t nt = blockDim.x;
    for (uint64_t i = begin + threadIdx.x; i < end; i += 4 * nt) {
        uint32_t e[4];
#pragma unroll
        for (int k = 0; k < 4; k++) e[k] = i + k * nt < end ? d[i + k * nt] : 0u;
#pragma unroll
        for (int k = 0; k < 4; k++) {
            const uint32_t b = e[k] >> 1;
            if (b) atomicAdd(&h[(b - 1) >> sg.lo_bits], 1u);
        }
    }
    __syncthreads();
    uint32_t* out = cntA + ((uint64_t)w * g.nchunk + q) * sg.nhi;
    for (uint32_t k = threadIdx.x; k < sg.nhi; k += blockDim.x) out[k] = h[k];
}

__global__ __launch_bounds__(1024) void msm_partprefix_kernel(uint32_t* __restrict__ cntA, MsmGeom g, SortGeom sg,
                                                              uint32_t* __restrict__ tot) {
    __shared__ uint32_t part[16][64];
    const uint32_t w = blockIdx.y, h = threadIdx.x & 63, qg = threadIdx.x >> 6;
    const uint32_t hi = blockIdx.x * 64 + h;
    const bool live = hi < sg.nhi;
    uint32_t* cw = cntA + (uint64_t)w * g.nchunk * sg.nhi;
    const uint32_t per = (g.nchunk + 15) / 16;
    const uint32_t q0 = qg * per < g.nchunk ? qg * per : g.nchunk;
    const uint32_t q1 = q0 + per < g.nchunk ? q0 + per : g.nchunk;
    uint32_t sum = 0;
    if (live)
        for (uint32_t q = q0; q < q1; q++) sum += cw[(uint64_t)q * sg.nhi + hi];
    part[qg][h] = sum;
    __syncthreads();
    uint32_t run = 0, total = 0;
    for (uint32_t k = 0; k < 16; k++) {
        if (k < qg) run += part[k][h];
        total += part[k][h];
    }
    if (live) {
        for (uint32_t q = q0; q < q1; q++) {
            uint32_t* p = cw + (uint64_t)q * sg.nhi + hi;
            const uint32_t v = *p;
            *p = run;
            run += v;
        }
        if (qg == 0) tot[(uint64_t)w * sg.nhi + hi] = total;
    }
}

__global__ __launch_bounds__(64) void msm_partstart_kernel(const uint32_t* __restrict__ tot, SortGeom sg,
                                                           uint32_t* __restrict__ pstart, uint32_t* __restrict__ ghist,
                                                           uint32_t* __restrict__ tail_barrier) {
    __shared__ uint32_t t[SORT_MAX_PART + 1];
    uint32_t* base = t;
    const uint32_t w = blockIdx.x;
    for (uint32_t k = threadIdx.x; k < 256; k += 64) {
        ghist[w * 256 + k] = 0;
        ghist[(gridDim.x + w) * 256 + k] = 0;
    }
    if (threadIdx.x == 0) tail_barrier[w * PYR_BAR_STRIDE] = 0;
    for (uint32_t k = threadIdx.x; k < sg.nhi; k += 64) t[k] = tot[(uint64_t)w * sg.nhi + k];
    __syncthreads();
    wave_exclusive_scan(t, base, sg.nhi, threadIdx.x);
    __syncthreads();
    for (uint32_t k = threadIdx.x; k <= sg.nhi; k += 64) pstart[(uint64_t)w * (sg.nhi + 1) + k] = base[k];
}

#ifndef ZKP_BS_TILE
#define ZKP_BS_TILE 16384
#endif
constexpr int BS_TILE = ZKP_BS_TILE;
constexpr int BS_PER = BS_TILE / 1024;
constexpr int SORT_MAX_BINS = 1024;
#ifndef ZKP_PS_TILE
#define ZKP_PS_TILE 12288
#endif
constexpr int PS_TILE_BIG = ZKP_PS_TILE, PS_TILE_MID = 8192, PS_TILE_SMALL = 4096;
ZKP_HD size_t partscatter_lds_bytes(uint32_t nhi, int tile) { return 8 * (size_t)tile + 2 * (size_t)tile + 4 * (size_t)(3 * nhi + 1); }
ZKP_HD int partscatter_tile(uint32_t nhi) { return nhi <= 2048 ? PS_TILE_BIG : nhi <= 4096 ? PS_TILE_MID : PS_TILE_SMALL; }

template <int PS_TILE>
__global__ __launch_bounds__(1024) void msm_partscatter_kernel(const uint32_t* __restrict__ digits, MsmGeom g, SortGeom sg,
                                                               const uint32_t* __restrict__ cntA,
                                                               const uint32_t* __restrict__ pstart,
                                                               uint2* __restrict__ entries) {
    constexpr int PS_PER = PS_TILE / 1024;
    extern __shared__ uint4 zkp_smem[];
    uint2* stage = reinterpret_cast<uint2*>(zkp_smem);
    uint16_t* part = reinterpret_cast<uint16_t*>(stage + PS_TILE);
    uint32_t* cur = reinterpret_cast<uint32_t*>(part + PS_TILE);
    uint32_t* cnt = cur + sg.nhi;
    uint32_t* base = cnt + sg.nhi;
    const uint32_t q = blockIdx.x, w = blockIdx.y, tid = threadIdx.x;
    for (uint32_t k = tid; k < sg.nhi; k += 1024)
        cur[k] = pstart[(uint64_t)w * (sg.nhi + 1) + k] + cntA[((uint64_t)w * g.nchunk + q) * sg.nhi + k];
    const uint64_t begin = (uint64_t)q * g.chunk;
    const uint64_t end = begin + g.chunk < g.n ? begin + g.chunk : g.n;
    const uint32_t* d = digits + (uint64_t)w * g.n;
    uint2* out = entries + (uint64_t)w * g.n;
    const uint32_t lo_mask = (1u << sg.lo_bits) - 1;
    for (uint64_t t0 = begin; t0 < end; t0 += PS_TILE) {
        for (uint32_t k = tid; k < sg.nhi; k += 1024) cnt[k] = 0;
        __syncthreads();
        uint32_t e[PS_PER], rk[PS_PER];
#pragma unroll
        for (int k = 0; k < PS_PER; k++) {
            const uint64_t i = t0 + tid + (uint64_t)k * 1024;
            e[k] = i < end ? d[i] : 0u;
        }
#pragma unroll
        for (int k = 0; k < PS_PER; k++) {
            const uint32_t b = e[k] >> 1;
            rk[k] = b ? atomicAdd(&cnt[(b - 1) >> sg.lo_bits], 1u) : 0u;
        }
        __syncthreads();
        if (tid < 64) wave_exclusive_scan(cnt, base, sg.nhi, tid);
        __syncthreads();
#pragma unroll
        for (int k = 0; k < PS_PER; k++) {
            const uint32_t b = e[k] >> 1;
            if (b) {
                const uint32_t p = (b - 1) >> sg.lo_bits;
                const uint32_t pos = base[p] + rk[k];
                stage[pos] = make_uint2((uint32_t)(t0 - 0 + tid + (uint64_t)k * 1024) | ((e[k] & 1u) << 31), (b - 1) & lo_mask);
                part[pos] = (uint16_t)p;
            }
        }
        __syncthreads();
        const uint32_t total = base[sg.nhi];
        for (uint32_t j = tid; j < total; j += 1024) {
            const uint32_t p = part[j];
#ifdef ZKP_MSM_CHECK
            if ((uint64_t)cur[p] + (j - base[p]) >= g.n && msm_check_fail(0, cur[p] + (j - base[p]), p)) continue;
#endif
            out[cur[p] + (j - base[p])] = stage[j];
        }
        __syncthreads();
        for (uint32_t k = tid; k < sg.nhi; k += 1024) cur[k] += cnt[k];
    }
}

__global__ __launch_bounds__(1024) void msm_binsort_kernel(const uint2* __restrict__ entries, MsmGeom g, SortGeom sg,
                                                           const uint32_t* __restrict__ pstart,
                                                           uint32_t* __restrict__ start, uint32_t* __restrict__ sorted,
                                                           uint32_t* __restrict__ ghist) {
    __shared__ uint32_t h[SORT_MAX_BINS + 1], cnt[SORT_MAX_BINS], base[SORT_MAX_BINS + 1];
    __shared__ uint32_t szh[256];
    __shared__ uint32_t stage[BS_TILE];
    __shared__ uint16_t bin[BS_TILE];
    const uint32_t hi = blockIdx.x, w = blockIdx.y, tid = threadIdx.x;
    const uint32_t lo_n = 1u << sg.lo_bits;
    const uint32_t* ps = pstart + (uint64_t)w * (sg.nhi + 1);
    const uint32_t begin = ps[hi], end = ps[hi + 1];
    const uint2* in = entries + (uint64_t)w * g.n;
    if (tid < lo_n) cnt[tid] = 0;
    if (tid < 256) szh[tid] = 0;
    __syncthreads();
    const uint32_t nt = blockDim.x;
    for (uint32_t i = begin + tid; i < end; i += 4 * nt) {
        uint32_t y[4];
#pragma unroll
        for (int k = 0; k < 4; k++) y[k] = i + k * nt < end ? in[i + k * nt].y : 0xffffffffu;
#pragma unroll
        for (int k = 0; k < 4; k++)
            if (y[k] != 0xffffffffu) atomicAdd(&cnt[y[k]], 1u);
    }
    __syncthreads();
    if (tid < lo_n) atomicAdd(&szh[255 - (cnt[tid] < 255 ? cnt[tid] : 255)], 1u);
    if (tid < 64) wave_exclusive_scan(cnt, h, lo_n, tid);
    __syncthreads();
    if (tid < 256 && szh[tid]) atomicAdd(&ghist[w * 256 + tid], szh[tid]);
    if (tid < lo_n) h[tid] += begin;
    __syncthreads();
    uint32_t* sw = start + (uint64_t)w * (g.nb + 2);
    if (tid < lo_n) sw[(hi << sg.lo_bits) + tid + 1] = h[tid];
    if (hi == 0 && tid == 0) sw[0] = 0;
    if (hi == sg.nhi - 1 && tid == 0) sw[g.nb + 1] = end;
    __syncthreads();
    uint32_t* out = sorted + (uint64_t)w * g.n;
    for (uint32_t t0 = begin; t0 < end; t0 += BS_TILE) {
        if (tid < lo_n) cnt[tid] = 0;
        __syncthreads();
        uint2 e[BS_PER];
        uint32_t rk[BS_PER];
#pragma unroll
        for (int k = 0; k < BS_PER; k++) {
            const uint32_t i = t0 + tid + k * 1024;
            e[k] = i < end ? in[i] : make_uint2(0u, 0xffffffffu);
        }
#pragma unroll
        for (int k = 0; k < BS_PER; k++) rk[k] = e[k].y != 0xffffffffu ? atomicAdd(&cnt[e[k].y], 1u) : 0u;
        __syncthreads();
        if (tid < 64) wave_exclusive_scan(cnt, base, lo_n, tid);
        __syncthreads();
#pragma unroll
        for (int k = 0; k < BS_PER; k++)
            if (e[k].y != 0xffffffffu) {
                const uint32_t pos = base[e[k].y] + rk[k];
                stage[pos] = e[k].x;
                bin[pos] = (uint16_t)e[k].y;
            }
        __syncthreads();
        const uint32_t total = base[lo_n];
        for (uint32_t j = tid; j < total; j += 1024) {
            const uint32_t p = bin[j];
#ifdef ZKP_MSM_CHECK
            if ((uint64_t)h[p] + (j - base[p]) >= g.n && msm_check_fail(1, h[p] + (j - base[p]), p)) continue;
#endif
            out[h[p] + (j - base[p])] = stage[j];
        }
        __syncthreads();
        if (tid < lo_n) h[tid] += cnt[tid];
    }
}


__global__ __launch_bounds__(1024) void msm_rank_kernel(const uint32_t* __restrict__ start, MsmGeom g,
                                                        const uint32_t* __restrict__ ghist, uint32_t* __restrict__ gcur,
                                                        uint32_t* __restrict__ perm) {
    __shared__ uint32_t hist[256], base[256], gh[256], first[257];
    const uint32_t w = blockIdx.y, tid = threadIdx.x;
    const uint32_t* sw = start + (uint64_t)w * (g.nb + 2);
    if (tid < 256) {
        hist[tid] = 0;
        gh[tid] = ghist[w * 256 + tid];
    }
    __syncthreads();
    if (tid < 64) wave_exclusive_scan(gh, first, 256, tid);
    const uint32_t b = 1 + blockIdx.x * 1024 + tid;
    uint32_t bin = 0, rk = 0;
    if (b <= g.nb) {
        const uint32_t sz = sw[b + 1] - sw[b];
        bin = 255 - (sz < 255 ? sz : 255);
        rk = atomicAdd(&hist[bin], 1u);
    }
    __syncthreads();
    if (tid < 256 && hist[tid]) base[tid] = first[tid] + atomicAdd(&gcur[w * 256 + tid], hist[tid]);
    __syncthreads();
#ifdef ZKP_MSM_CHECK
    if (b <= g.nb && base[bin] + rk >= g.nb && msm_check_fail(5, base[bin] + rk, b)) return;
#endif
    if (b <= g.nb) perm[(uint64_t)w * g.nb + base[bin] + rk] = b;
}

__global__ __launch_bounds__(1024) void msm_order_kernel(const uint32_t* __restrict__ start, MsmGeom g,
                                                         const uint32_t* __restrict__ ghist,
                                                         const uint32_t* __restrict__ perm, uint32_t* __restrict__ over,
                                                         uint32_t* __restrict__ over_b, uint32_t* __restrict__ over_off,
                                                         uint4* __restrict__ desc, uint32_t over_cap, uint32_t desc_cap) {
    __shared__ uint32_t s_over[2], gh[256], first[257];
    const uint32_t w = blockIdx.x, tid = threadIdx.x, nt = blockDim.x;
    const uint32_t* sw = start + (uint64_t)w * (g.nb + 2);
    const uint32_t* pw = perm + (uint64_t)w * g.nb;
    if (tid < 256) gh[tid] = ghist[w * 256 + tid];
    __syncthreads();
    if (tid < 64) wave_exclusive_scan(gh, first, 256, tid);
    __syncthreads();
    if (tid == 0) {
        const uint32_t limit_bin = g.run_limit < 254 ? g.run_limit : 254;
        s_over[0] = first[255 - limit_bin];
    }
    __syncthreads();
    const uint32_t n_over = s_over[0] < over_cap ? s_over[0] : over_cap;
#ifdef ZKP_MSM_CHECK
    if (tid == 0 && s_over[0] > g.nb) msm_check_fail(7, s_over[0], over_cap);
#endif
    uint32_t* ob = over_b + (uint64_t)w * over_cap;
    uint32_t* oo = over_off + (uint64_t)w * (over_cap + 1);
    {
        __shared__ uint32_t part[1024];
        const uint32_t per = (n_over + nt - 1) / nt;
        const uint32_t r0 = tid * per < n_over ? tid * per : n_over;
        const uint32_t r1 = r0 + per < n_over ? r0 + per : n_over;
        uint32_t local = 0;
        for (uint32_t r = r0; r < r1; r++) {
            const uint32_t b = pw[r];
#ifdef ZKP_MSM_CHECK
            if ((b == 0 || b > g.nb) && msm_check_fail(6, b, r)) continue;
#endif
            const uint32_t sz = sw[b + 1] - sw[b];
            local += sz > g.run_limit ? (sz + g.piece - 1) / g.piece : 0;
        }
        part[tid] = local;
        __syncthreads();
        for (uint32_t off = 1; off < nt; off <<= 1) {
            const uint32_t v = tid >= off ? part[tid - off] : 0;
            __syncthreads();
            part[tid] += v;
            __syncthreads();
        }
        uint32_t run = tid ? part[tid - 1] : 0;
        for (uint32_t r = r0; r < r1; r++) {
            const uint32_t b = pw[r];
#ifdef ZKP_MSM_CHECK
            if (b == 0 || b > g.nb) { ob[r] = 1; oo[r] = run; continue; }
#endif
            const uint32_t sz = sw[b + 1] - sw[b];
            ob[r] = b;
            oo[r] = run;
            run += sz > g.run_limit ? (sz + g.piece - 1) / g.piece : 0;
        }
        if (tid == nt - 1) {
            const uint32_t total = part[nt - 1];
            oo[n_over] = total;
            s_over[1] = total;
            over[2 * w] = n_over;
            over[2 * w + 1] = total < desc_cap ? total : desc_cap;
        }
    }
    __syncthreads();
    const uint32_t n_pieces = s_over[1] < desc_cap ? s_over[1] : desc_cap;
    uint4* dw = desc + (uint64_t)w * desc_cap;
    for (uint32_t j = tid; j < n_pieces; j += nt) {
        uint32_t lo = 0, hi = n_over;
        while (hi - lo > 1) {
            const uint32_t mid = (lo + hi) >> 1;
            if (oo[mid] <= j) lo = mid; else hi = mid;
        }
        const uint32_t b = ob[lo], p = j - oo[lo];
        const uint32_t first = sw[b] + p * g.piece;
        const uint32_t last = first + g.piece < sw[b + 1] ? first + g.piece : sw[b + 1];
        dw[j] = make_uint4(b, p, first, last);
    }
}

__global__ __launch_bounds__(MSM_THREADS) void g1_to_internal_kernel(const uint4* __restrict__ in, uint64_t n,
                                                                    uint4* __restrict__ out) {
    const uint64_t i = (uint64_t)blockIdx.x * MSM_THREADS + threadIdx.x;
    if (i >= n) return;
    G1Affine p = G1Affine::load(in + i * 6);
#pragma unroll 1
    for (int k = 0; k < 8; k++) {
        p.x = dbl(p.x);
        p.y = dbl(p.y);
    }
    A28 q;
    q.x = fq28_from_sat(p.x);
    q.y = fq28_from_sat(p.y);
    q.store(out + i * 8);
}

struct SliceOffsets {
    uint16_t off[36];
};
__global__ __launch_bounds__(MSM_THREADS) void g1_expand_planes_kernel(uint4* __restrict__ planes, uint4* __restrict__ scratch,
                                                                      uint64_t off, uint64_t cnt, uint64_t plane_stride,
                                                                      uint32_t nplanes, SliceOffsets so) {
    const uint64_t j = (uint64_t)blockIdx.x * MSM_THREADS + threadIdx.x;
    if (j >= cnt) return;
    const uint64_t i = off + j;
    auto slot = [&](uint32_t s, uint32_t t) { return scratch + (((uint64_t)s * 3 + t) * cnt + j) * 4; };
    const A28 p0 = A28::load(planes + i * 8);
    X28 x = g1_28_double_affine(p0);
    Fq28 run = Fq28::one();
#pragma unroll 1
    for (uint32_t s = 1; s < nplanes; s++) {
#pragma unroll 1
        for (uint32_t k = (s == 1 ? 1u : 0u), c = (uint32_t)so.off[s] - so.off[s - 1]; k < c; k++) x = g1_28_double(x);
        A28 raw;
        raw.x = x.x;
        raw.y = x.y;
        raw.store(planes + (s * plane_stride + i) * 8);
        run.store(slot(s, 2));
        x.zz.store(slot(s, 0));
        x.zzz.store(slot(s, 1));
        run = run * x.zzz;
    }
    Fq28 inv = fq28_inverse_gcd(run);
// ... 90 lines not shown
    const uint32_t slot = g.interleave ? blockIdx.x / g.nwin : blockIdx.x % per_set;
    const uint32_t* sw = start + (uint64_t)w * (g.nb + 2);
    const uint32_t* idx = sorted + (uint64_t)w * g.n;
    if (slot < bucket_blocks) {
        const uint32_t unit = slot * ACC_THREADS + threadIdx.x;
        const uint32_t rank = unit >> g.split_log, part = unit & ((1u << g.split_log) - 1);
        if (rank >= g.nb) return;
        const uint32_t b = perm[(uint64_t)w * g.nb + rank];
#ifdef ZKP_MSM_CHECK
        if ((b == 0 || b > g.nb) && msm_check_fail(3, b, rank | 0x80000000u)) return;
#endif
        uint32_t lo = sw[b], hi = sw[b + 1];
        const uint64_t e = (uint64_t)w * g.nb + pyr_pos(b - 1, g.nb);
        uint4* dst = g.more ? carry + e * 16 : split_dst(g, buckets, parts, part) + e;
        if (hi - lo > g.run_limit && rank < over[2 * w]) {
            if (part) hi = lo;
            else return;
        }
        split_run(g, part, lo, hi);
        msm_accumulate_run(bases28, idx, lo, hi, g, dst, g.more ? 1 : bucket_cap(g), g.resume != 0, carry + e * 16, 1);
    } else {
        const uint32_t n_pieces = over[2 * w + 1];
#ifdef ZKP_MSM_CHECK
        if (n_pieces > desc_cap && msm_check_fail(4, n_pieces, desc_cap)) return;
#endif
        const uint32_t stride = extra_blocks * ACC_THREADS;
        for (uint32_t j = (slot - bucket_blocks) * ACC_THREADS + threadIdx.x; j < n_pieces; j += stride) {
            const uint4 d = desc[(uint64_t)w * desc_cap + j];
            msm_accumulate_run(bases28, idx, d.z, d.w, g, pieces + ((uint64_t)w * desc_cap + j) * 16, 1, false);
        }
    }
}

__global__ __launch_bounds__(ACC_THREADS) __attribute__((amdgpu_waves_per_eu(3))) void msm_accumulate_kernel(const uint4* __restrict__ bases28,
                                                                    const uint32_t* __restrict__ sorted,
                                                                    const uint32_t* __restrict__ start,
                                                                    const uint32_t* __restrict__ perm,
                                                                    const uint32_t* __restrict__ over,
                                                                    const uint4* __restrict__ desc, uint32_t desc_cap,
                                                                    uint32_t bucket_blocks, uint32_t extra_blocks, MsmGeom g,
                                                                    uint4* __restrict__ buckets,
                                                                    uint4* __restrict__ pieces, uint4* __restrict__ parts,
                                                                    uint4* __restrict__ carry, ClkRec* __restrict__ clk) {
    uint64_t t0 = 0, r0 = 0;
    clk_begin(clk, t0, r0);
    msm_accumulate_body(bases28, sorted, start, perm, over, desc, desc_cap, bucket_blocks, extra_blocks, g, buckets, pieces, parts, carry);
    clk_end(clk, t0, r0);
}

constexpr int MAD_PROBE_ITERS = 8192, MAD_PROBE_CHAINS = 8;
__global__ __launch_bounds__(256) void mad_rate_probe_kernel(uint32_t* __restrict__ out, uint32_t seed, ClkRec* __restrict__ clk) {
    uint64_t t0 = 0, r0 = 0;
    clk_begin(clk, t0, r0);
    const uint32_t a = seed + threadIdx.x, b = seed * 3 + blockIdx.x;
    uint64_t acc[MAD_PROBE_CHAINS];
    uint32_t lo[MAD_PROBE_CHAINS];
#pragma unroll
    for (int c = 0; c < MAD_PROBE_CHAINS; c++) { acc[c] = a + c; lo[c] = b + c; }
#pragma unroll 1
    for (int it = 0; it < MAD_PROBE_ITERS; it++) {
#pragma unroll
        for (int c = 0; c < MAD_PROBE_CHAINS; c++)
            asm volatile("v_mad_u64_u32 %0, vcc, %1, %2, %0" : "+v"(acc[c]) : "v"(a), "v"(lo[c]) : "vcc");
    }
    uint32_t r = 0;
#pragma unroll
    for (int c = 0; c < MAD_PROBE_CHAINS; c++) r ^= (uint32_t)acc[c] ^ (uint32_t)(acc[c] >> 32);
    out[blockIdx.x * blockDim.x + threadIdx.x] = r;
    clk_end(clk, t0, r0);
}

ZKP_DEV void msm_accumulate_quad_run(const uint4* __restrict__ bases28, const uint32_t* __restrict__ idx, uint32_t lo,
                                     uint32_t hi, const MsmGeom& g, uint4* __restrict__ dst, uint64_t dst_stride, int j) {
    const bool odd = (j & 1) != 0, up = (j & 2) != 0;
    Fq28 own = Fq28::zero();
    bool inf = true, fresh = false;
    auto point_of = [&](uint32_t e) -> const uint4* {
        uint64_t pt = e & 0x7fffffffu;
        if (g.shared) {
            const uint32_t ns32 = (uint32_t)g.ns, s = (uint32_t)pt / ns32;
            pt = (uint64_t)s * g.plane_stride + ((uint32_t)pt - s * ns32);
        }
        return bases28 + pt * 8;
    };
    uint32_t e_next = lo < hi ? idx[lo] : 0u, e_next2 = lo + 1 < hi ? idx[lo + 1] : 0u;
    Fq28 c_next = Fq28::zero();
    if (lo < hi) c_next = Fq28::load(point_of(e_next) + (up ? 4 : 0));
    for (uint32_t k = lo; k < hi; k++) {
        const uint32_t e = e_next;
        const uint4* src = point_of(e);
        Fq28 coord = c_next;
        if (k + 1 < hi) {
            e_next = e_next2;
            c_next = Fq28::load(point_of(e_next) + (up ? 4 : 0));
        }
        if (k + 2 < hi) e_next2 = idx[k + 2];
        if (up && (e >> 31)) coord = neg4(coord);
        if (inf) {
            own = odd ? Fq28::one() : (up ? normalise(coord) : coord);
            inf = false;
            fresh = true;
            continue;
        }
        Fq28 m1;
        if (fresh) m1 = normalise(coord);
        else m1 = coord * own;
        fresh = false;
        const Fq28 d = sub16(quad_xor1(m1), own);
        const Fq28 m2 = d * d;
        const Fq28 pp = quad_bcast(m2, 0);
        if (quad_bcast0(tight_is_zero_mod_p(m2) ? 1 : 0)) {
            X28 acc;
            acc.x = quad_bcast(own, 0); acc.zz = quad_bcast(own, 1); acc.y = quad_bcast(own, 2); acc.zzz = quad_bcast(own, 3);
            A28 q = A28::load(src);
            if (e >> 31) q.y = neg4(q.y);
            g1_28_madd(acc, q);
            inf = acc.is_inf();
            own = up ? (odd ? acc.zzz : acc.y) : (odd ? acc.zz : acc.x);
            continue;
        }
        const Fq28 x1 = quad_bcast(own, 0);
        const Fq28 m3 = fq28_select(j == 0, d, fq28_select(j == 3, x1, own)) * pp;
        const Fq28 ppp = quad_bcast(m3, 0), q = quad_bcast(m3, 3);
        const Fq28 x3 = normalise(sub8w(sub4(m2, ppp), q + q));
        const Fq28 t = sub16(q, x3);
        const Fq28 y1 = quad_bcast(own, 2);
        const Fq28 m4 = fq28_select(j == 0, y1, fq28_select(j == 2, d, own)) * fq28_select(j == 2, t, ppp);
        const Fq28 v = quad_bcast(m4, 0);
        const Fq28 x3b = quad_bcast(x3, 2);
        own = up ? (odd ? m4 : normalise(sub4(m4, v))) : (odd ? m3 : x3b);
    }
    uint4* part = dst + (up ? (odd ? 12 : 4) : (odd ? 8 : 0)) * dst_stride;
    if (inf) own = Fq28::zero();
    own.store_s(part, dst_stride);
}

ZKP_DEV void msm_accumulate_quad_body(const uint4* __restrict__ bases28, const uint32_t* __restrict__ sorted,
                                      const uint32_t* __restrict__ start, const uint32_t* __restrict__ perm,
                                      const uint32_t* __restrict__ over, const uint4* __restrict__ desc, uint32_t desc_cap,
                                      uint32_t bucket_blocks, uint32_t extra_blocks, const MsmGeom& g, uint4* __restrict__ buckets,
                                      uint4* __restrict__ pieces, uint4* __restrict__ parts) {
    constexpr uint32_t QUADS = ACC_THREADS / 4;
    const uint32_t per_set = bucket_blocks + extra_blocks;
    const uint32_t w = g.interleave ? blockIdx.x % g.nwin : blockIdx.x / per_set;
    const uint32_t slot = g.interleave ? blockIdx.x / g.nwin : blockIdx.x % per_set;
    const uint32_t* sw = start + (uint64_t)w * (g.nb + 2);
    const uint32_t* idx = sorted + (uint64_t)w * g.n;
    const int j = threadIdx.x & 3;
    const uint32_t quad = threadIdx.x >> 2;
    if (slot < bucket_blocks) {
        const uint32_t unit = slot * QUADS + quad;
        const uint32_t rank = unit >> g.split_log, part = unit & ((1u << g.split_log) - 1);
        if (rank >= g.nb) return;
        const uint32_t b = perm[(uint64_t)w * g.nb + rank];
        uint32_t lo = sw[b], hi = sw[b + 1];
        uint4* dst = split_dst(g, buckets, parts, part) + ((uint64_t)w * g.nb + pyr_pos(b - 1, g.nb));
        if (hi - lo > g.run_limit && rank < over[2 * w]) {
            if (part) hi = lo;
            else return;
        }
        split_run(g, part, lo, hi);
        msm_accumulate_quad_run(bases28, idx, lo, hi, g, dst, bucket_cap(g), j);
    } else {
        const uint32_t n_pieces = over[2 * w + 1];
        const uint32_t stride = extra_blocks * QUADS;
        for (uint32_t p = (slot - bucket_blocks) * QUADS + quad; p < n_pieces; p += stride) {
            const uint4 d = desc[(uint64_t)w * desc_cap + p];
            msm_accumulate_quad_run(bases28, idx, d.z, d.w, g, pieces + ((uint64_t)w * desc_cap + p) * 16, 1, j);
        }
    }
}
__global__ __launch_bounds__(ACC_THREADS) void msm_accumulate_quad_kernel(const uint4* __restrict__ bases28,
                                                                         const uint32_t* __restrict__ sorted,
                                                                         const uint32_t* __restrict__ start,
                                                                         const uint32_t* __restrict__ perm,
                                                                         const uint32_t* __restrict__ over,
                                                                         const uint4* __restrict__ desc, uint32_t desc_cap,
                                                                         uint32_t bucket_blocks, uint32_t extra_blocks, MsmGeom g,
                                                                         uint4* __restrict__ buckets,
                                                                         uint4* __restrict__ pieces, uint4* __restrict__ parts,
                                                                         ClkRec* __restrict__ clk) {
    uint64_t t0 = 0, r0 = 0;
    clk_begin(clk, t0, r0);
    msm_accumulate_quad_body(bases28, sorted, start, perm, over, desc, desc_cap, bucket_blocks, extra_blocks, g, buckets, pieces, parts);
    clk_end(clk, t0, r0);
}

__global__ __launch_bounds__(MSM_THREADS) void msm_fold_parts_kernel(uint4* __restrict__ buckets, uint4* __restrict__ parts,
                                                                    uint64_t cap, uint32_t step) {
    const uint64_t e = (uint64_t)blockIdx.x * (MSM_THREADS / 4) + (threadIdx.x >> 2);
    if (e >= cap) return;
    const uint32_t ia = blockIdx.y << (step + 1), ib = ia + (1u << step);
    uint4* pa = (ia ? parts + (uint64_t)(ia - 1) * 16 * cap : buckets) + e;
    const uint4* pb = parts + (uint64_t)(ib - 1) * 16 * cap + e;
    g1_28_add_quad(pa, pb, pa, cap, threadIdx.x & 3);
}

__global__ __launch_bounds__(MSM_THREADS) void msm_fold_parts_lane_kernel(uint4* __restrict__ buckets, uint4* __restrict__ parts,
                                                                         uint64_t cap, uint32_t step) {
    const uint64_t e = (uint64_t)blockIdx.x * MSM_THREADS + threadIdx.x;
    if (e >= cap) return;
    const uint32_t ia = blockIdx.y << (step + 1), ib = ia + (1u << step);
    uint4* pa = (ia ? parts + (uint64_t)(ia - 1) * 16 * cap : buckets) + e;
    const uint4* pb = parts + (uint64_t)(ib - 1) * 16 * cap + e;
    g1_28_add_stream_inplace<ACC_CHAIN>(pa, pb, cap);
}

__global__ __launch_bounds__(64) void msm_combine_kernel(const uint32_t* __restrict__ over, const uint32_t* __restrict__ over_b,
                                                         const uint32_t* __restrict__ over_off, uint32_t over_cap,
                                                         uint32_t desc_cap, MsmGeom g, const uint4* __restrict__ pieces,
                                                         uint4* __restrict__ buckets, uint4* __restrict__ carry) {
    __shared__ uint4 sh[64 * 16];
    const uint32_t w = blockIdx.y, lane = threadIdx.x;
    for (uint32_t r = blockIdx.x; r < over[2 * w]; r += gridDim.x) {
    const uint32_t b = over_b[(uint64_t)w * over_cap + r];
    const uint32_t* oo = over_off + (uint64_t)w * (over_cap + 1);
    uint32_t p0 = oo[r], p1 = oo[r + 1];
    if (p1 > desc_cap) p1 = desc_cap;
    if (p1 <= p0) continue;
    const uint4* pw = pieces + (uint64_t)w * desc_cap * 16;
    X28 acc = X28::infinity();
    for (uint32_t p = p0 + lane; p < p1; p += 64) {
        X28 x = X28::load(pw + (uint64_t)p * 16);
        g1_28_add(acc, x);
    }
    for (uint32_t off = 32; off > 0; off >>= 1) {
        acc.store(sh + lane * 16);
        __syncthreads();
        if (lane < off) {
            X28 x = X28::load(sh + (lane + off) * 16);
            g1_28_add(acc, x);
        }
        __syncthreads();
    }
    if (lane == 0) {
        const uint64_t e = (uint64_t)w * g.nb + pyr_pos(b - 1, g.nb);
        if (g.resume) {
            X28 x = X28::load_s(carry + e * 16, 1);
            g1_28_add(acc, x);
        }
        if (g.more) acc.store_s(carry + e * 16, 1);
        else acc.store_s(buckets + e, bucket_cap(g));
    }
    __syncthreads();
    }
}

struct PyrLevel {
    uint32_t level;
    uint32_t half;
    uint32_t nb;
    uint32_t nwin;
};
ZKP_DEV uint64_t odd_off(uint32_t nb, uint32_t j) { return (uint64_t)nb - (nb >> j); }
struct PyrItem {
    uint64_t a, b, d;
    bool src_is_pyr_out;
};
ZKP_DEV PyrItem pyr_item(uint32_t nb, uint32_t level, uint32_t half, uint32_t kind, uint32_t s, uint64_t wbase) {
    PyrItem it;
    if (kind == 0) {
        it.a = wbase + s;
        it.b = wbase + half + s;
        it.d = wbase + pyr_pos(s, half);
        it.src_is_pyr_out = false;
    } else {
        const uint64_t o = wbase + odd_off(nb, kind - 1);
        it.src_is_pyr_out = kind == level;
        const uint64_t src = it.src_is_pyr_out ? wbase + 2 * (uint64_t)half : o;
        it.a = src + s;
        it.b = src + half + s;
        it.d = o + s;
    }
    return it;
}

__global__ __launch_bounds__(MSM_THREADS) void msm_pyramid_kernel(const uint4* __restrict__ pyr_in,
                                                                  uint4* pyr_out,
                                                                  const uint4* __restrict__ odd_in,
                                                                  uint4* __restrict__ odd_out, PyrLevel L) {
    const uint32_t s = blockIdx.x * MSM_THREADS + threadIdx.x;
    if (s >= L.half) return;
    const uint32_t kind = blockIdx.y, w = blockIdx.z;
    const uint64_t cap = (uint64_t)L.nwin * L.nb;
    const PyrItem it = pyr_item(L.nb, L.level, L.half, kind, s, (uint64_t)w * L.nb);
    const uint4* src = kind == 0 ? pyr_in : (it.src_is_pyr_out ? pyr_out : odd_in);
    g1_28_add_stream<ACC_CHAIN>(src + it.a, src + it.b, (kind ? odd_out : pyr_out) + it.d, cap);
}

__global__ __launch_bounds__(MSM_THREADS) void msm_pyramid_quad_kernel(const uint4* __restrict__ pyr_in,
                                                                       uint4* pyr_out,
                                                                       const uint4* __restrict__ odd_in,
                                                                       uint4* __restrict__ odd_out, PyrLevel L) {
    const uint32_t s = blockIdx.x * (MSM_THREADS / 4) + (threadIdx.x >> 2);
    const int j = threadIdx.x & 3;
    if (s >= L.half) return;
    const uint32_t kind = blockIdx.y, w = blockIdx.z;
    const uint64_t cap = (uint64_t)L.nwin * L.nb;
    const PyrItem it = pyr_item(L.nb, L.level, L.half, kind, s, (uint64_t)w * L.nb);
    const uint4* src = kind == 0 ? pyr_in : (it.src_is_pyr_out ? pyr_out : odd_in);
    g1_28_add_quad(src + it.a, src + it.b, (kind ? odd_out : pyr_out) + it.d, cap, j);
}

constexpr uint32_t MSM_TAIL_TIMEOUT = 0x80000000u;
constexpr uint32_t MSM_FLAG_PENDING = 0x40000000u;
constexpr uint32_t MSM_FLAG_PENDING_MASK = 0x40000000u;
constexpr uint32_t PYR_TAIL_THREADS = 256;
constexpr uint32_t PYR_TAIL_BLOCKS = 16;
constexpr uint32_t PYR_TAIL_SPIN_LIMIT = 1u << 24;
__global__ __launch_bounds__(512) void msm_pyramid_tail_kernel(uint4* __restrict__ pyr0, uint4* __restrict__ pyr1,
                                                               uint4* __restrict__ odd0, uint4* __restrict__ odd1,
                                                               uint32_t level0, uint32_t c, uint32_t nb,
                                                               uint32_t* __restrict__ barrier ,
                                                               uint4* __restrict__ result ,
                                                               uint32_t* __restrict__ flags ,
                                                               uint32_t expect_blocks ,
                                                               uint32_t spin_limit) {
    const uint32_t w = blockIdx.y;
    const uint64_t wbase = (uint64_t)w * nb;
    const uint64_t cap = (uint64_t)gridDim.y * nb;
    const int j = threadIdx.x & 3;
    const uint32_t quad = blockIdx.x * (blockDim.x >> 2) + (threadIdx.x >> 2), nquad = gridDim.x * (blockDim.x >> 2);
    uint32_t epoch = 0;
    for (uint32_t l = level0; l + 1 < c; l++) {
        const uint32_t half = nb >> (l + 1);
        const uint4* pyr_in = (l & 1) ? pyr1 : pyr0;
        uint4* pyr_out = (l & 1) ? pyr0 : pyr1;
        const uint4* odd_in = (l & 1) ? odd1 : odd0;
        uint4* odd_out = (l & 1) ? odd0 : odd1;
        for (uint32_t item = quad; item < (l + 1) * half; item += nquad) {
            const uint32_t kind = item / half, s = item % half;
            const PyrItem it = pyr_item(nb, l, half, kind, s, wbase);
            const uint4* src = kind == 0 ? pyr_in : (it.src_is_pyr_out ? pyr_out : odd_in);
            g1_28_add_quad(src + it.a, src + it.b, (kind ? odd_out : pyr_out) + it.d, cap, j);
        }
        epoch++;
        __syncthreads();
        if (threadIdx.x == 0) {
            uint32_t* bar = barrier + (uint64_t)w * PYR_BAR_STRIDE;
            __builtin_amdgcn_fence(__ATOMIC_RELEASE, "agent");
            __hip_atomic_fetch_add(bar, 1u, __ATOMIC_RELAXED, __HIP_MEMORY_SCOPE_AGENT);
            bool arrived = false;
            for (uint32_t spin = 0; spin < spin_limit; spin++) {
                if (__hip_atomic_load(bar, __ATOMIC_RELAXED, __HIP_MEMORY_SCOPE_AGENT) >= epoch * expect_blocks) {
                    arrived = true;
                    break;
                }
                __builtin_amdgcn_s_sleep(1);
            }
            if (!arrived) __hip_atomic_fetch_or(bar, MSM_TAIL_TIMEOUT, __ATOMIC_RELAXED, __HIP_MEMORY_SCOPE_AGENT);
            __builtin_amdgcn_fence(__ATOMIC_ACQUIRE, "agent");
        }
        __syncthreads();
    }
    if (blockIdx.x == 0) {
        const uint4* pyr_final = ((c - 1) & 1) ? pyr1 : pyr0;
        const uint4* pyr_prev = ((c - 1) & 1) ? pyr0 : pyr1;
        const uint4* odd_final = ((c - 1) & 1) ? odd1 : odd0;
        for (uint32_t t = threadIdx.x; t < c * 16; t += blockDim.x) {
            const uint32_t e = t >> 4, q = t & 15;
            const uint4* src = e == 0 ? pyr_final + wbase : e == c - 1 ? pyr_prev + (wbase + 1) : odd_final + (wbase + odd_off(nb, e - 1));
            result[((uint64_t)w * c + e) * 16 + q] = src[q * cap];
        }
        __threadfence_system();
        __syncthreads();
        if (threadIdx.x == 0) {
            const uint32_t v = __hip_atomic_load(barrier + (uint64_t)w * PYR_BAR_STRIDE, __ATOMIC_RELAXED, __HIP_MEMORY_SCOPE_AGENT);
            __hip_atomic_store(flags + w, v & ~MSM_FLAG_PENDING_MASK, __ATOMIC_RELEASE, __HIP_MEMORY_SCOPE_SYSTEM);
        }
    }
}

__global__ void msm_collect_kernel(const uint4* __restrict__ pyr_final, const uint4* __restrict__ pyr_prev,
                                   const uint4* __restrict__ odd_final, uint32_t nb, uint32_t c, uint4* __restrict__ result,
                                   uint32_t* __restrict__ flags) {
    const uint32_t w = blockIdx.x, j = threadIdx.x;
    if (j < c) {
        const uint64_t wbase = (uint64_t)w * nb;
        const uint64_t cap = (uint64_t)gridDim.x * nb;
        const uint4* src = j == 0 ? pyr_final + wbase : j == c - 1 ? pyr_prev + (wbase + 1) : odd_final + (wbase + odd_off(nb, j - 1));
        uint4* dst = result + ((uint64_t)w * c + j) * 16;
        for (int q = 0; q < 16; q++) dst[q] = src[q * cap];
    }
    __threadfence_system();
    __syncthreads();
    if (j == 0) __hip_atomic_store(flags + w, 0u, __ATOMIC_RELEASE, __HIP_MEMORY_SCOPE_SYSTEM);
}

__global__ __launch_bounds__(MSM_THREADS) void g1_fixed_base_kernel(const Fr* __restrict__ scalars, uint64_t n,
                                                                   const uint4* __restrict__ table,
                                                                   uint4* __restrict__ out_xy,
                                                                   uint8_t* __restrict__ out_inf) {
    const uint64_t i = (uint64_t)blockIdx.x * MSM_THREADS + threadIdx.x;
    if (i >= n) return;
    Fr k = from_mont(scalars[i]);
    G1Xyzz acc = G1Xyzz::infinity();
#pragma unroll 1
    for (int w = 0; w < 32; w++) {
        uint32_t limb = 0;
#pragma unroll
        for (int q = 0; q < 8; q++)
            if (q == (w >> 2)) limb = k.l[q];
        const uint32_t d = (limb >> ((w & 3) * 8)) & 0xffu;
        if (d) {
            G1Affine p = G1Affine::load(table + ((uint64_t)w * 255 + (d - 1)) * 6);
            g1_madd(acc, p);
        }
    }
    G1Affine r;
    const bool inf = acc.is_inf();
    if (inf) {
        r.x = Fq::zero();
        r.y = Fq::zero();
    } else {
        Fq zi3 = fq_inverse_gcd(acc.zzz);
        Fq zi2 = sqr(zi3 * acc.zz);
        r.x = acc.x * zi2;
        r.y = acc.y * zi3;
    }
    r.store(out_xy + i * 6);
    if (out_inf) out_inf[i] = inf ? 1 : 0;
}

__global__ __launch_bounds__(MSM_THREADS) void fq_inverse_selftest_kernel(const uint32_t* __restrict__ in, uint32_t* __restrict__ out,
                                                                         uint64_t n, int form) {
    const uint64_t i = (uint64_t)blockIdx.x * MSM_THREADS + threadIdx.x;
    if (i >= n) return;
    if (form == 0) {
        Fq a;
#pragma unroll
        for (int w = 0; w < 12; w++) a.l[w] = in[12 * i + w];
        const Fq r = fq_inverse_gcd(a);
#pragma unroll
        for (int w = 0; w < 12; w++) out[12 * i + w] = r.l[w];
    } else {
        const Fq28 a = Fq28::load(reinterpret_cast<const uint4*>(in) + 4 * i);
        fq28_inverse_gcd(a).store(reinterpret_cast<uint4*>(out) + 4 * i);
    }
}

}
```

zkp-implementation_amd/csrc/msm_host.inc:

```

#ifdef ZKP_MSM_CHECK
#define MSM_TRACE(stream, ridx, what) do { hipError_t e_ = hipStreamSynchronize(stream); fprintf(stderr, "ZKP_MSM_CHECK range %llu: %s done (%d)\n", (unsigned long long)(ridx), what, (int)e_); } while (0)
#else
#define MSM_TRACE(stream, ridx, what) do { } while (0)
#endif

struct MsmFeed {
    const uint64_t* h_scalars;
    hipStream_t copy_stream;
    hipEvent_t ev;
    MsmFeedRanges ranges;
};

struct RangeBuffers {
    uint32_t *sorted, *start, *perm;
    uint4* desc;
    uint32_t *over, *over_b, *over_off;
};

struct MsmPass {
    const MsmPlan& p;
    MsmGeom g;
    const zkp_bases* bases;
    const Fr* const* scalars;
    size_t count;
    const MsmFeed* feed;
    hipStream_t st, sst;
    Ctx& cx = ctx();
    const size_t W = p.g.nwin, nhi = p.sg.nhi;
    uint32_t *ptot, *pstart, *ghist, *gcur;
    uint4* result_out;
    uint32_t* result_flags;
    RangeUpload up;

    std::array<std::tuple<const char*, DevBuf*, size_t>, 14> buffers() {
        const MsmSizes& b = p.bytes;
        return {{{"digits", &cx.digits, b.digits}, {"sorted", &cx.sorted, b.sorted}, {"counts", &cx.counts, b.counts},
                 {"entries", &cx.entries, b.entries}, {"start", &cx.start, b.start}, {"perm", &cx.perm, b.perm}, {"over", &cx.over, b.over},
                 {"pieces", &cx.pieces, b.pieces}, {"buckets", &cx.buckets, b.buckets}, {"parts", &cx.parts, b.parts},
                 {"pyr1", &cx.pyr1, b.pyr1}, {"odd0", &cx.odd0, b.odd0}, {"odd1", &cx.odd1, b.odd1}, {"result", &cx.result, b.result}}};
    }
    int grow() {
        for (const auto& [name, buf, bytes] : buffers()) ZCHK(buf->ensure(bytes));
        ZCHK(cx.host_result.ensure(p.bytes.host_result, hipHostMallocPortable | hipHostMallocMapped));
        ptot = cx.counts.get() + W * g.nchunk * nhi;
        pstart = ptot + W * nhi;
        ghist = pstart + W * (nhi + 1);
        gcur = ghist + W * 256;
        result_out = static_cast<uint4*>(cx.host_result.p);
        result_flags = reinterpret_cast<uint32_t*>(result_out + 16 * W * g.c);
        return ZKP_OK;
    }
    RangeBuffers range_buffers(size_t par) const {
        uint4* desc = reinterpret_cast<uint4*>(static_cast<char*>(cx.over.p) + par * p.over_bytes);
        uint32_t* over = reinterpret_cast<uint32_t*>(desc + W * p.desc_cap);
        return {cx.sorted.get() + par * W * p.g.n, cx.start.get() + par * W * (p.g.nb + 2), cx.perm.get() + par * W * p.g.nb, desc, over,
                over + 2 * W, over + 2 * W + W * p.over_cap};
    }
#ifdef ZKP_MSM_CHECK
    void dump(size_t n) {
        static bool once = false;
        if (once) return;
        once = true;
        auto show = [](const char* name, const void* q, size_t bytes) {
            fprintf(stderr, "ZKP_MSM_CHECK %-10s %p .. %p (%zu bytes)\n", name, q, static_cast<const char*>(q) + bytes, bytes);
        };
        show("bases", bases->d_xy.p, (size_t)bases->n * 128 * std::max(bases->pre_planes, 1u));
        show("scalars", scalars[0], 32 * n);
        for (const auto& [name, buf, bytes] : buffers()) show(name, buf->p, buf->cap);
        show("host_res", cx.host_result.p, cx.host_result.cap);
        fprintf(stderr, "ZKP_MSM_CHECK geometry: n %zu range %llu first %llu rest %llu entries %llu nb %u nchunk %u over_cap %u desc_cap %u run_limit %u piece %u\n",
                n, (unsigned long long)p.range, (unsigned long long)p.lens[0], (unsigned long long)p.lens.back(), (unsigned long long)p.g.n,
                p.g.nb, p.g.nchunk, p.over_cap, p.desc_cap, p.g.run_limit, p.g.piece);
    }
#endif

    int feed_first_range() {
        Fr* const dst = const_cast<Fr*>(scalars[0]);
        if (p.lens.size() > 1) {
            while (cx.copy_events.size() < p.lens.size() - 1) {
                Event e;
                ZCHK(e.ensure(hipEventDisableTiming));
                cx.copy_events.push_back(std::move(e));
            }
            up.submit(uploader(cx.slot), std::vector<uint64_t>(p.lens.begin() + 1, p.lens.end()), p.lens[0],
                      [device = cx.device] { return hipSetDevice(device) == hipSuccess ? (int)ZKP_OK : (int)ZKP_E_DEVICE; },
                      [dst, f = *feed, evs = cx.copy_events.data()](size_t k, uint64_t o, uint64_t l) {
                          const bool ok = hipMemcpyAsync(dst + o, f.h_scalars + 4 * o, 32 * l, hipMemcpyHostToDevice, f.copy_stream) == hipSuccess &&
                                          hipEventRecord(evs[k], f.copy_stream) == hipSuccess;
                          return ok ? (int)ZKP_OK : (int)ZKP_E_DEVICE;
                      });
        }
        hipError_t e1 = hipMemcpyAsync(dst, feed->h_scalars, 32 * p.lens[0], hipMemcpyHostToDevice, feed->copy_stream);
        if (e1 == hipSuccess) e1 = hipEventRecord(feed->ev, feed->copy_stream);
        up.release(e1 == hipSuccess);
        HIPCHK(e1);
        return ZKP_OK;
    }

    int walk() {
        if (p.overlap) {
            ZCHK(cx.sort_stream.ensure(hipStreamNonBlocking));
            for (Event* e : {&cx.ev_sort[0], &cx.ev_sort[1], &cx.ev_acc[0], &cx.ev_acc[1], &cx.ev_begin}) ZCHK(e->ensure(hipEventDisableTiming));
            sst = cx.sort_stream;
            HIPCHK(hipEventRecord(cx.ev_begin, st));
            HIPCHK(hipStreamWaitEvent(sst, cx.ev_begin, 0));
        }
        for (size_t ridx = 0, off = 0; ridx < p.lens.size(); off += p.lens[ridx++]) {
            const uint64_t len = p.lens[ridx];
            const size_t par = p.overlap ? (ridx & 1) : 0;
            const RangeBuffers rb = range_buffers(par);
            if (p.overlap && ridx >= 2) HIPCHK(hipStreamWaitEvent(sst, cx.ev_acc[par], 0));
            if (len != g.ns) {
                g.ns = len;
                g.n = (uint64_t)p.nwin1 * len;
                g.chunk = (g.n + g.nchunk - 1) / g.nchunk;
            }
            g.resume = off ? 1u : 0u;
            g.more = ridx + 1 < p.lens.size() ? 1u : 0u;
            if (feed) {
                if (ridx == 0)
                    ZCHK(feed_first_range());
                else if (!up.wait_issued(ridx))
                    return fail(ZKP_E_DEVICE, "upload of a scalar range failed");
                HIPCHK(hipStreamWaitEvent(sst, ridx == 0 ? feed->ev : cx.copy_events[ridx - 1], 0));
            }
            launch_sort(rb, off, ridx);
            if (p.overlap) {
                HIPCHK(hipEventRecord(cx.ev_sort[par], sst));
                HIPCHK(hipStreamWaitEvent(st, cx.ev_sort[par], 0));
            }
            launch_accumulate(rb, off, ridx);
            if (p.overlap) HIPCHK(hipEventRecord(cx.ev_acc[par], st));
        }
        return ZKP_OK;
    }

    template <int TILE> void launch_partscatter() {
        hipLaunchKernelGGL(msm_partscatter_kernel<TILE>, dim3(g.nchunk, g.nwin), dim3(1024), partscatter_lds_bytes(nhi, TILE), sst,
                           cx.digits.get(), g, p.sg, cx.counts.get(), pstart, cx.entries.get());
    }
    void launch_sort(const RangeBuffers& rb, uint64_t off, size_t ridx) {
        const SortGeom& sg = p.sg;
        {
            ProfScope ps("msm_digits", sst);
            DigitSources ds;
            for (size_t m = 0; m < count; m++) ds.scalars[m] = scalars[m] + off;
            hipLaunchKernelGGL(msm_digits_kernel, dim3((unsigned)((g.ns + MSM_THREADS - 1) / MSM_THREADS), (unsigned)count), dim3(MSM_THREADS), 0,
                               sst, ds, bases->d_inf.p ? bases->d_inf.get() + off : nullptr, g, p.nwin1, cx.digits.get());
            MSM_TRACE(sst, ridx, "digits");
        }
        ProfScope ps("msm_sort", sst, true);
        hipLaunchKernelGGL(msm_parthist_kernel, dim3(g.nchunk, g.nwin), dim3(1024), 0, sst, cx.digits.get(), g, sg, cx.counts.get());
        MSM_TRACE(sst, ridx, "parthist");
        hipLaunchKernelGGL(msm_partprefix_kernel, dim3((sg.nhi + 63) / 64, g.nwin), dim3(1024), 0, sst, cx.counts.get(), g, sg, ptot);
        hipLaunchKernelGGL(msm_partstart_kernel, dim3(g.nwin), dim3(64), 0, sst, ptot, sg, pstart, ghist, cx.result.get());
        MSM_TRACE(sst, ridx, "partprefix + partstart");
        switch (partscatter_tile(sg.nhi)) {
            case PS_TILE_SMALL: launch_partscatter<PS_TILE_SMALL>(); break;
            case PS_TILE_MID: launch_partscatter<PS_TILE_MID>(); break;
            default: launch_partscatter<PS_TILE_BIG>(); break;
        }
        MSM_TRACE(sst, ridx, "partscatter");
        hipLaunchKernelGGL(msm_binsort_kernel, dim3(sg.nhi, g.nwin), dim3(1024), 0, sst, cx.entries.get(), g, sg, pstart, rb.start, rb.sorted, ghist);
        MSM_TRACE(sst, ridx, "binsort");
        hipLaunchKernelGGL(msm_rank_kernel, dim3((g.nb + 1023) / 1024, g.nwin), dim3(1024), 0, sst, rb.start, g, ghist, gcur, rb.perm);
        MSM_TRACE(sst, ridx, "rank");
        hipLaunchKernelGGL(msm_order_kernel, dim3(g.nwin), dim3(1024), 0, sst, rb.start, g, ghist, rb.perm, rb.over, rb.over_b, rb.over_off,
                           rb.desc, p.over_cap, p.desc_cap);
        MSM_TRACE(sst, ridx, "order");
    }

    void launch_accumulate(const RangeBuffers& rb, uint64_t off, size_t ridx) {
        ProfScope ps("msm_accumulate", st, true);
        const bool quad = !g.resume && !g.more && (uint64_t)g.n * g.nwin <= (1ull << 20);
        const uint32_t per_block = quad ? ACC_THREADS / 4 : ACC_THREADS;
        const uint32_t bucket_blocks = (uint32_t)((((uint64_t)g.nb << g.split_log) + per_block - 1) / per_block);
        const uint32_t extra_blocks = std::min<uint32_t>((p.desc_cap + per_block - 1) / per_block, 64);
        const dim3 grid((bucket_blocks + extra_blocks) * g.nwin);
        const uint4* xy = static_cast<const uint4*>(bases->d_xy.p) + off * 8;
        uint4 *buckets = cx.buckets.get(), *pieces = cx.pieces.get(), *parts = cx.parts.get(), *carry = cx.pyr1.get();
        if (quad)
            hipLaunchKernelGGL(msm_accumulate_quad_kernel, grid, dim3(ACC_THREADS), 0, st, xy, rb.sorted, rb.start, rb.perm, rb.over, rb.desc,
                               p.desc_cap, bucket_blocks, extra_blocks, g, buckets, pieces, parts, clk_record(CLK_MSM_ACCUMULATE));
        else
            hipLaunchKernelGGL(msm_accumulate_kernel, grid, dim3(ACC_THREADS), 0, st, xy, rb.sorted, rb.start, rb.perm, rb.over, rb.desc,
                               p.desc_cap, bucket_blocks, extra_blocks, g, buckets, pieces, parts, carry, clk_record(CLK_MSM_ACCUMULATE));
        MSM_TRACE(st, ridx, "accumulate");
        hipLaunchKernelGGL(msm_combine_kernel, dim3(std::min<uint32_t>(p.over_cap, 64), g.nwin), dim3(64), 0, st, rb.over, rb.over_b,
                           rb.over_off, p.over_cap, p.desc_cap, g, pieces, buckets, carry);
        MSM_TRACE(st, ridx, "combine");
        const uint64_t cap = (uint64_t)g.nwin * g.nb;
        static const uint64_t lane_from = getenv("ZKP_FOLD_LANE_MIN") ? strtoull(getenv("ZKP_FOLD_LANE_MIN"), nullptr, 10) : FOLD_LANE_MIN_ADDS;
        for (uint32_t t = 0; t < g.split_log; t++) {
            const unsigned pairs = 1u << (g.split_log - 1 - t), per = cap * pairs >= lane_from ? MSM_THREADS : MSM_THREADS / 4;
            hipLaunchKernelGGL(per == MSM_THREADS ? msm_fold_parts_lane_kernel : msm_fold_parts_kernel, dim3((unsigned)((cap + per - 1) / per), pairs),
                               dim3(MSM_THREADS), 0, st, buckets, parts, cap, t);
        }
    }

    int reduce() {
        static const uint32_t tail_threads = getenv("ZKP_PYR_TAIL_THREADS") ? (uint32_t)atoi(getenv("ZKP_PYR_TAIL_THREADS")) : PYR_TAIL_THREADS;
        static const uint32_t tail_blocks = getenv("ZKP_PYR_TAIL_BLOCKS") ? (uint32_t)atoi(getenv("ZKP_PYR_TAIL_BLOCKS")) : PYR_TAIL_BLOCKS;
        static const uint32_t tail_half = getenv("ZKP_PYR_TAIL_HALF") ? (uint32_t)atoi(getenv("ZKP_PYR_TAIL_HALF")) : 64u;
        if (tail_threads < 64 || tail_threads > 512 || (tail_threads & 63) || !tail_blocks || tail_blocks > 256 || !tail_half)
            return fail(ZKP_E_ARG, "ZKP_PYR_TAIL_THREADS must be a multiple of 64 up to 512, ZKP_PYR_TAIL_BLOCKS 1..256, ZKP_PYR_TAIL_HALF >= 1");
        for (size_t w = 0; w < W; w++) __atomic_store_n(result_flags + w, MSM_FLAG_PENDING, __ATOMIC_RELEASE);
        uint4* pyr[2] = {cx.buckets.get(), cx.pyr1.get()};
        uint4* odd[2] = {cx.odd0.get(), cx.odd1.get()};
        ProfScope ps("msm_bucket_reduce", st, true);
        uint32_t level_tail = 0;
        while (level_tail + 1 < g.c && (g.nb >> (level_tail + 1)) > tail_half) level_tail++;
        const uint32_t max_waves = cx.tail_max_waves;
        if ((uint64_t)g.nwin * (tail_threads / 64) > max_waves) level_tail = g.c - 1;
        for (uint32_t l = 0; l < level_tail; l++) {
            const PyrLevel L{l, g.nb >> (l + 1), g.nb, g.nwin};
            const bool quad = (uint64_t)L.half * (l + 1) * g.nwin <= (1u << 16);
            const uint32_t per = quad ? MSM_THREADS / 4 : MSM_THREADS;
            hipLaunchKernelGGL(quad ? msm_pyramid_quad_kernel : msm_pyramid_kernel, dim3((L.half + per - 1) / per, l + 1, g.nwin),
                               dim3(MSM_THREADS), 0, st, pyr[l & 1], pyr[(l + 1) & 1], odd[l & 1], odd[(l + 1) & 1], L);
        }
        if (level_tail + 1 < g.c) {
            uint32_t tb = tail_blocks;
            while (tb > 1 && (uint64_t)tb * g.nwin * (tail_threads / 64) > max_waves) tb >>= 1;
            const bool starve = getenv("ZKP_TEST_TAIL_STARVE") != nullptr;
            hipLaunchKernelGGL(msm_pyramid_tail_kernel, dim3(tb, g.nwin), dim3(tail_threads), 0, st, pyr[0], pyr[1], odd[0], odd[1], level_tail,
                               g.c, g.nb, cx.result.get(), result_out, result_flags, starve ? tb + 1 : tb, starve ? (1u << 12) : PYR_TAIL_SPIN_LIMIT);
        } else {
            const uint32_t fin = (g.c - 1) & 1;
            hipLaunchKernelGGL(msm_collect_kernel, dim3(g.nwin), dim3(64), 0, st, pyr[fin], pyr[fin ^ 1], odd[fin], g.nb, g.c, result_out,
                               result_flags);
        }
        return ZKP_OK;
    }
};

int wait_msm_result(const MsmGeom& g, const uint32_t* flags, hipStream_t st) {
    bool seen = false;
    if (g.n <= (1ull << 24) && !getenv("ZKP_MSM_NO_POLL")) {
        const auto t_poll0 = std::chrono::steady_clock::now();
        for (uint64_t spins = 0;; __builtin_ia32_pause()) {
            bool all = true;
            for (size_t w = 0; w < g.nwin && all; w++) all = (__atomic_load_n(flags + w, __ATOMIC_ACQUIRE) & MSM_FLAG_PENDING) == 0;
            if ((seen = all)) break;
            if ((++spins & 1023) == 0 && std::chrono::steady_clock::now() - t_poll0 > std::chrono::seconds(2)) break;
        }
    }
    if (!seen) HIPCHK(hipStreamSynchronize(st));
    for (size_t w = 0; w < g.nwin; w++)
        if (flags[w] & MSM_TAIL_TIMEOUT)
            return fail(ZKP_E_DEVICE, "bucket reduction: the workgroups of the last levels did not all become resident (device shared "
                                      "with another job?); no result was produced");
    return ZKP_OK;
}

void msm_host_tail(const uint32_t* host_res, size_t count, uint32_t wins_per_msm, uint32_t c, HXyzz* out) {
    const auto t_tail0 = std::chrono::steady_clock::now();
    auto tail = [&](size_t m) {
        const uint32_t* res = host_res + m * wins_per_msm * c * 64;
        HXyzz total = HXyzz::infinity();
        for (int pos = (int)(wins_per_msm * c) - 1; pos >= 0; pos--) {
            total = total.dbl();
            const int w = pos / (int)c, l = pos % (int)c;
            const uint32_t* rw = res + (size_t)w * c * 64;
            if (l <= (int)c - 2) total = total.add(xyzz_from_internal(rw + (size_t)(1 + l) * 64));
            if (l == 0) total = total.add(xyzz_from_internal(rw));
        }
        out[m] = total;
    };
    if (count == 1)
        tail(0);
    else
        host_pool().run(std::function<void(size_t)>(tail), count);
    prof_host("msm_tail_host", std::chrono::duration<double, std::milli>(std::chrono::steady_clock::now() - t_tail0).count());
}

int msm_partial_batch(const zkp_bases* bases, const Fr* const* d_scalars, size_t count, size_t n, hipStream_t st, HXyzz* out,
                      const MsmFeed* feed = nullptr) {
    MsmPlan p;
    if (const int rc = plan_msm({bases->n, bases->pre_c, bases->pre_planes, bases->pre_off}, count, n, feed ? &feed->ranges : nullptr, &p))
        return fail(rc, p.error);
    if (p.lens.empty()) {
        for (size_t m = 0; m < count; m++) out[m] = HXyzz::infinity();
        return ZKP_OK;
    }
    MsmPass pass{p, p.g, bases, d_scalars, count, feed, st, st};
    ZCHK(pass.grow());
#ifdef ZKP_MSM_CHECK
    pass.dump(n);
#endif
    const int walk_rc = pass.walk(), up_rc = pass.up.join();
    if (walk_rc != ZKP_OK || up_rc != ZKP_OK) {
        if (p.overlap) (void)hipStreamSynchronize(pass.sst);
        if (feed) (void)hipStreamSynchronize(feed->copy_stream);
        return walk_rc != ZKP_OK ? walk_rc : fail(ZKP_E_DEVICE, "upload of a scalar range failed");
    }
    HIPCHK(hipGetLastError());
    ZCHK(pass.reduce());
    HIPCHK(hipGetLastError());
#ifdef ZKP_MSM_CHECK
    {
        uint32_t chk[32];
        HIPCHK(hipStreamSynchronize(st));
        HIPCHK(hipMemcpyFromSymbol(chk, HIP_SYMBOL(g_msm_check), sizeof(chk)));
        for (int k = 0; k < 8; k++)
            if (chk[4 * k]) fprintf(stderr, "ZKP_MSM_CHECK class %d: %u violations, first (%u, %u)\n", k, chk[4 * k], chk[4 * k + 1], chk[4 * k + 2]);
    }
#endif
    if (count > 1 && !getenv("ZKP_POOL_NO_WARM")) host_pool().warm(std::chrono::microseconds(3000));
    ZCHK(wait_msm_result(pass.g, pass.result_flags, st));
    msm_host_tail(reinterpret_cast<const uint32_t*>(pass.result_out), count, p.g.shared ? 1u : p.nwin1, p.g.c, out);
    return ZKP_OK;
}

int msm_partial(const zkp_bases* bases, const Fr* d_scalars, size_t n, hipStream_t st, HXyzz* out) {
    return msm_partial_batch(bases, &d_scalars, 1, n, st, out);
}
```

zkp-implementation_amd/zkp_hip/__init__.py:

```python
import ctypes as C
import os
import sys

import numpy as np

_PKG = os.path.dirname(os.path.abspath(__file__))
_ROOT = os.path.dirname(_PKG)
LIB_PATH = os.path.join(_ROOT, "libzkp_hip.so")
if os.environ.get("ZKP_HIP_LIB"):
    LIB_PATH = os.environ["ZKP_HIP_LIB"]

ZKP_OK, ZKP_E_ARG, ZKP_E_NOMEM, ZKP_E_DEVICE, ZKP_E_SIZE = 0, -1, -2, -3, -4


class ZkpError(RuntimeError):
    def __init__(self, code, msg):
        super().__init__(f"zkp_hip error {code}: {msg}")
        self.code = code


_lib = None

_VP, _SZ, _U8P = C.c_void_p, C.c_size_t, C.c_void_p
_SIGS = {
    "zkp_init": ([C.c_int], C.c_int),
    "zkp_init_devices": ([_VP, C.c_int], C.c_int),
    "zkp_device_count": ([], C.c_int),
    "zkp_set_device": ([C.c_int], C.c_int),
    "zkp_shutdown": ([], None),
    "zkp_last_error": ([], C.c_char_p),
    "zkp_abi_version": ([], C.c_int),
    "zkp_profile_enable": ([C.c_int], None),
    "zkp_profile_reset": ([], None),
    "zkp_profile_read": ([C.c_char_p, C.POINTER(C.c_double), C.POINTER(C.c_uint64)], C.c_int),
    "zkp_profile_clock_read": ([C.c_char_p, C.POINTER(C.c_uint64), C.POINTER(C.c_uint64), C.POINTER(C.c_uint64)], C.c_int),
    "zkp_probe_mad_rate": ([C.c_uint, C.POINTER(C.c_double), C.POINTER(C.c_double), C.POINTER(C.c_double)], C.c_int),
    "zkp_g1_bases_create": ([_VP, _U8P, _SZ, C.POINTER(_VP)], C.c_int),
    "zkp_g1_bases_create_dev": ([_VP, _U8P, _SZ, _VP, C.POINTER(_VP)], C.c_int),
    "zkp_g1_bases_precompute": ([_VP, C.c_uint], C.c_int),
    "zkp_g1_bases_len": ([_VP], _SZ),
    "zkp_g1_bases_info": ([_VP, C.POINTER(C.c_uint), C.POINTER(C.c_uint)], C.c_int),
    "zkp_g1_bases_destroy": ([_VP], None),
    "zkp_msm_g1": ([_VP, _VP, _SZ, _VP, _VP], C.c_int),
    "zkp_msm_g1_dev": ([_VP, _VP, _SZ, _VP, _VP, _VP], C.c_int),
    "zkp_msm_g1_batch_dev": ([_VP, _VP, _SZ, _SZ, _VP, _VP, _VP], C.c_int),
    "zkp_msm_g1_partial_dev": ([_VP, _VP, _SZ, _VP, _VP], C.c_int),
    "zkp_msm_g1_partial": ([_VP, _VP, _SZ, _VP], C.c_int),
    "zkp_g1_bases_shard_count": ([_VP], C.c_int),
    "zkp_g1_bases_shard": ([_VP, _SZ, C.POINTER(C.c_int), C.POINTER(C.c_int), C.POINTER(_SZ), C.POINTER(_SZ)], C.c_int),
    "zkp_msm_g1_sharded_dev": ([_VP, _VP, _SZ, _VP, _VP], C.c_int),
    "zkp_msm_g1_sharded_dev_after": ([_VP, _VP, _VP, _SZ, _VP, _VP], C.c_int),
    "zkp_g1_xyzz_sum": ([_VP, _SZ, _VP, _VP], C.c_int),
    "zkp_g1_mul": ([_VP, C.c_uint8, _VP, _VP, _VP], C.c_int),
    "zkp_g1_fixed_base_mul_dev": ([_VP, _SZ, _VP, _U8P, _VP], C.c_int),
    "zkp_selftest_fq_inverse_dev": ([_VP, _SZ, C.c_int, _VP, _VP], C.c_int),
    "zkp_srs_g1": ([_VP, _SZ, _VP], C.c_int),
    "zkp_ntt_fr": ([_VP, C.c_uint, C.c_int, _VP], C.c_int),
    "zkp_ntt_fr_dev": ([_VP, C.c_uint, _SZ, C.c_int, _VP, _VP], C.c_int),
    "zkp_ntt_fr_twiddle_dev": ([_VP, _SZ, _SZ, _SZ, C.c_uint, C.c_int, _VP], C.c_int),
    "zkp_ntt_fr_axis0_dev": ([_VP, _VP, C.c_uint, _SZ, C.c_int, C.c_uint, _SZ, _VP], C.c_int),
    "zkp_ntt_fr_layout_dev": ([_VP, _VP, C.c_uint, _SZ, C.c_int, _VP, _VP, C.c_uint, _SZ, _VP], C.c_int),
    "zkp_ntt_fr_sharded_geometry": ([C.c_uint, C.c_uint, C.c_uint, _VP], C.c_int),
    "zkp_ntt_fr_sharded_dev": ([_VP, C.c_uint, C.c_int, C.c_int, C.c_int, C.c_uint, _VP], C.c_int),
    "zkp_ntt_fr_sharded": ([_VP, C.c_uint, C.c_int, _VP], C.c_int),
    "zkp_ntt_goldilocks": ([_VP, C.c_uint, C.c_int, _VP], C.c_int),
    "zkp_ntt_goldilocks_dev": ([_VP, C.c_uint, _SZ, C.c_int, _VP, _VP], C.c_int),
    "zkp_fri_layer_eval": ([_VP, _SZ, C.c_uint64, C.c_uint, _VP], C.c_int),
    "zkp_fri_fold": ([_VP, _SZ, C.c_uint64, _VP], C.c_int),
    "zkp_fri_merkle_node_count": ([_SZ], _SZ),
    "zkp_fri_merkle_tree": ([_VP, _SZ, _VP], C.c_int),
    "zkp_fri_merkle_tree_dev": ([_VP, _SZ, _VP, _VP], C.c_int),
    "zkp_fri_challenges": ([_VP, _SZ, C.c_uint64, _SZ, _VP, _VP], C.c_int),
    "zkp_fri_prove": ([_VP, _SZ, _SZ, _SZ, C.POINTER(_VP), C.POINTER(_SZ)], C.c_int),
    "zkp_fri_verify": ([_VP, _SZ], C.c_int),
    "zkp_fri_layer_eval_fr": ([_VP, _SZ, _VP, C.c_uint, _VP], C.c_int),
    "zkp_fri_fold_fr": ([_VP, _SZ, _VP, _VP], C.c_int),
    "zkp_fri_merkle_tree_fr": ([_VP, _SZ, _VP], C.c_int),
    "zkp_fri_merkle_tree_fr_dev": ([_VP, _SZ, _VP, _VP], C.c_int),
    "zkp_fri_challenges_fr": ([_VP, _SZ, _VP, _SZ, _VP, _VP], C.c_int),
    "zkp_fri_prove_fr": ([_VP, _SZ, _SZ, _SZ, C.POINTER(_VP), C.POINTER(_SZ)], C.c_int),
    "zkp_fri_verify_fr": ([_VP, _SZ], C.c_int),
    "zkp_free": ([_VP], None),
    "zkp_plonk_prove": ([_VP, _VP, _VP], C.c_int),
    "zkp_g2_generator": ([_VP], C.c_int),
    "zkp_g2_mul": ([_VP, C.c_uint8, _VP, _VP, _U8P], C.c_int),
    "zkp_pairing": ([_VP, C.c_uint8, _VP, C.c_uint8, _VP], C.c_int),
    "zkp_kzg_verify": ([_VP, _VP, C.c_uint8, _VP, C.c_uint8, _VP, _VP, C.POINTER(C.c_int)], C.c_int),
    "zkp_kzg_batch_verify": ([_VP, _SZ, _VP, _U8P, _VP, _VP, _U8P, _VP, _VP, C.POINTER(C.c_int)], C.c_int),
    "zkp_kzg_aggregate_commitments": ([_VP, _U8P, _SZ, _VP, _VP, _VP], C.c_int),
    "zkp_plonk_verify": ([_VP, _VP, _VP, C.POINTER(C.c_int)], C.c_int),
    "zkp_plonk_transcript_create": ([C.POINTER(_VP)], C.c_int),
    "zkp_plonk_transcript_destroy": ([_VP], None),
    "zkp_plonk_transcript_feed": ([_VP, _VP, C.c_uint8], C.c_int),
    "zkp_plonk_transcript_challenges": ([_VP, _SZ, _VP], C.c_int),
    "zkp_poly_mul_fr": ([_VP, _SZ, _VP, _SZ, _VP], C.c_int),
    "zkp_plonk_prover_create": ([_VP, C.c_uint, _VP, _VP, _VP, _VP, C.POINTER(_VP)], C.c_int),
    "zkp_plonk_prover_destroy": ([_VP], None),
    "zkp_plonk_round1": ([_VP, _VP, _VP, _VP], C.c_int),
    "zkp_plonk_round2": ([_VP, _VP, _VP, _VP, _VP, _VP], C.c_int),
    "zkp_plonk_round3": ([_VP, _VP, _VP, _VP, C.POINTER(C.c_size_t)], C.c_int),
    "zkp_plonk_round4": ([_VP, _VP, _VP], C.c_int),
    "zkp_plonk_round5": ([_VP, _VP, _VP, _VP], C.c_int),
    "zkp_plonk_get_poly": ([_VP, C.c_int, _VP, _SZ, C.POINTER(C.c_size_t)], C.c_int),
    "zkp_kzg_commit": ([_VP, _VP, _SZ, _VP, _VP], C.c_int),
    "zkp_kzg_open": ([_VP, _VP, _SZ, _VP, _VP, _VP, _VP], C.c_int),
    "zkp_nova_r1cs_create": ([_VP, _SZ, _SZ, _SZ, _VP, _VP, _VP, C.POINTER(_VP)], C.c_int),
    "zkp_nova_r1cs_destroy": ([_VP], None),
    "zkp_nova_cross_term_dev": ([_VP, _VP, _VP, _VP, _VP, _VP, _VP, _VP, _VP], C.c_int),
    "zkp_nova_fold_witness_dev": ([_VP, _VP, _VP, _VP, _VP, _VP, _VP, _VP, _VP, _VP], C.c_int),
    "zkp_nova_relaxed_residual_dev": ([_VP, _VP, _VP, _VP, _VP, _VP, C.POINTER(C.c_uint64)], C.c_int),
    "zkp_nova_transcript_create": ([C.POINTER(_VP)], C.c_int),
    "zkp_nova_transcript_destroy": ([_VP], None),
    "zkp_nova_transcript_feed": ([_VP, _VP, C.c_uint8], C.c_int),
    "zkp_nova_transcript_feed_scalar": ([_VP, _VP], C.c_int),
    "zkp_nova_transcript_challenges": ([_VP, _SZ, _VP], C.c_int),
    "zkp_nova_nifs_prover_dev": ([_VP] * 15, C.c_int),
    "zkp_nova_nifs_prover": ([_VP] * 14, C.c_int),
    "zkp_nova_nifs_prove_dev": ([_VP] * 8, C.c_int),
    "zkp_nova_nifs_prove": ([_VP] * 7, C.c_int),
    "zkp_nova_nifs_verify": ([_VP, _VP, _VP, _VP, _VP, _VP, C.c_uint8, _VP, C.POINTER(C.c_int)], C.c_int),
}


def exported_symbols():
    return sorted(_SIGS)


def lib():
    global _lib
    if _lib is None:
        if not os.path.exists(LIB_PATH):
            raise ZkpError(ZKP_E_DEVICE, f"{LIB_PATH} not found: run `python zkp-implementation_amd/build.py` "
                           "(hipcc --offload-arch=gfx950); there is no CPU fallback")
        if "torch" not in sys.modules:
            try:
                import torch
            except ImportError:
                pass
        l = C.CDLL(LIB_PATH)
        for name, (args, res) in _SIGS.items():
            fn = getattr(l, name)
            fn.argtypes = args
            fn.restype = res
        _lib = l
    return _lib


def _chk(code):
    if code != ZKP_OK:
        raise ZkpError(code, lib().zkp_last_error().decode())


def init(device=-1):
    _chk(lib().zkp_init(device))


def init_devices(devices=None, n=0):
    if devices is None:
        _chk(lib().zkp_init_devices(None, int(n)))
    else:
        arr = (C.c_int * len(devices))(*[int(d) for d in devices])
        _chk(lib().zkp_init_devices(C.cast(arr, C.c_void_p), len(devices)))


def device_count():
    return int(lib().zkp_device_count())


def set_device(slot):
    _chk(lib().zkp_set_device(int(slot)))


def shutdown():
    lib().zkp_shutdown()


def profile_enable(on=True):
    lib().zkp_profile_enable(2 if on == 2 and on is not True else int(bool(on)))


def profile_reset():
    lib().zkp_profile_reset()


def profile_read(name):
    ms, cnt = C.c_double(0), C.c_uint64(0)
    _chk(lib().zkp_profile_read(name.encode(), C.byref(ms), C.byref(cnt)))
    return ms.value, int(cnt.value)


def profile_clock_read(name):
    cyc, ref, waves = C.c_uint64(0), C.c_uint64(0), C.c_uint64(0)
    _chk(lib().zkp_profile_clock_read(name.encode(), C.byref(cyc), C.byref(ref), C.byref(waves)))
    return int(cyc.value), int(ref.value), int(waves.value)


def probe_mad_rate(launches=20):
    rate, mhz, ms = C.c_double(0), C.c_double(0), C.c_double(0)
    _chk(lib().zkp_probe_mad_rate(launches, C.byref(rate), C.byref(mhz), C.byref(ms)))
    return rate.value, mhz.value, ms.value


def _np(a, dtype, shape=None):
    a = np.ascontiguousarray(a, dtype=dtype)
    return a.reshape(shape) if shape is not None else a


def _ptr(a):
    return a.ctypes.data_as(C.c_void_p) if a is not None else None


def _stream_ptr(stream):
    if stream is None:
        try:
            import torch
            if torch.cuda.is_available():
                return C.c_void_p(torch.cuda.current_stream().cuda_stream)
        except ImportError:
            pass
        return None
    return C.c_void_p(int(stream))


def _dev_ptr(t, min_bytes):
    if not t.is_cuda or not t.is_contiguous():
        raise ZkpError(ZKP_E_ARG, "expected a contiguous CUDA tensor")
    if t.numel() * t.element_size() < min_bytes:
        raise ZkpError(ZKP_E_ARG, "tensor smaller than the operation needs")
    return C.c_void_p(t.data_ptr())


class G1Bases:

    def __init__(self, handle):
        self._h = handle

    @classmethod
    def from_host(cls, xy, is_inf=None):
        xy = _np(xy, np.uint64, (-1, 12))
        inf = _np(is_inf, np.uint8) if is_inf is not None else None
        h = C.c_void_p()
        _chk(lib().zkp_g1_bases_create(_ptr(xy), _ptr(inf), xy.shape[0], C.byref(h)))
        return cls(h)

    @classmethod
    def from_device(cls, xy_tensor, n, is_inf_tensor=None, stream=None):
        h = C.c_void_p()
        inf = C.c_void_p(is_inf_tensor.data_ptr()) if is_inf_tensor is not None else None
        _chk(lib().zkp_g1_bases_create_dev(_dev_ptr(xy_tensor, 96 * n), inf, n, _stream_ptr(stream), C.byref(h)))
        return cls(h)

    def precompute(self, window_bits=20):
        _chk(lib().zkp_g1_bases_precompute(self._h, window_bits))
        return self

    def shards(self):
        out = []
        for i in range(lib().zkp_g1_bases_shard_count(self._h)):
            slot, dev, off, ln = C.c_int(0), C.c_int(0), C.c_size_t(0), C.c_size_t(0)
            _chk(lib().zkp_g1_bases_shard(self._h, i, C.byref(slot), C.byref(dev), C.byref(off), C.byref(ln)))
            out.append((int(slot.value), int(dev.value), int(off.value), int(ln.value)))
        return out

    def info(self):
        w, sl = C.c_uint(0), C.c_uint(0)
        _chk(lib().zkp_g1_bases_info(self._h, C.byref(w), C.byref(sl)))
        return int(w.value), int(sl.value)

    def __len__(self):
        return int(lib().zkp_g1_bases_len(self._h))

    def close(self):
        if self._h:
            lib().zkp_g1_bases_destroy(self._h)
            self._h = None

    def __del__(self):
        try:
            self.close()
        except Exception:
            pass


def msm_g1(bases, scalars):
    scalars = _np(scalars, np.uint64, (-1, 4))
    out = np.zeros(12, dtype=np.uint64)
    inf = C.c_uint8(0)
    _chk(lib().zkp_msm_g1(bases._h, _ptr(scalars), scalars.shape[0], _ptr(out), C.byref(inf)))
    return out, int(inf.value)


def msm_g1_partial(bases, scalars):
    scalars = _np(scalars, np.uint64, (-1, 4))
    out = np.zeros(24, dtype=np.uint64)
    _chk(lib().zkp_msm_g1_partial(bases._h, _ptr(scalars), scalars.shape[0], _ptr(out)))
    return out


def msm_g1_sharded_dev(bases, scalar_tensors, n, events=None):
    k = len(scalar_tensors)
    ptrs = (C.c_void_p * k)(*[(t.data_ptr() if t is not None else None) for t in scalar_tensors])
    out = np.zeros(12, dtype=np.uint64)
    inf = C.c_uint8(0)
    if events is None:
        _chk(lib().zkp_msm_g1_sharded_dev(bases._h, ptrs, n, _ptr(out), C.byref(inf)))
    else:
        if len(events) != k:
            raise ValueError("one event (or None) per chunk")
        evs = (C.c_void_p * k)(*[(e.cuda_event if e is not None else None) for e in events])
        _chk(lib().zkp_msm_g1_sharded_dev_after(bases._h, ptrs, evs, n, _ptr(out), C.byref(inf)))
    return out, int(inf.value)


def selftest_fq_inverse_dev(in_tensor, n, form, out_tensor, stream=None):
    words = 12 if form == 0 else 16
    _chk(lib().zkp_selftest_fq_inverse_dev(_dev_ptr(in_tensor, 4 * words * n), n, form, _dev_ptr(out_tensor, 4 * words * n),
                                           _stream_ptr(stream)))


def msm_g1_dev(bases, scalars_tensor, n, stream=None):
    out = np.zeros(12, dtype=np.uint64)
    inf = C.c_uint8(0)
    _chk(lib().zkp_msm_g1_dev(bases._h, _dev_ptr(scalars_tensor, 32 * n), n, _stream_ptr(stream), _ptr(out),
                              C.byref(inf)))
    return out, int(inf.value)


def msm_g1_batch_dev(bases, scalar_tensors, n, stream=None):
    k = len(scalar_tensors)
    ptrs = (C.c_void_p * k)(*[_dev_ptr(t, 32 * n).value for t in scalar_tensors])
    xy, inf = np.zeros((k, 12), dtype=np.uint64), np.zeros(k, dtype=np.uint8)
    _chk(lib().zkp_msm_g1_batch_dev(bases._h, ptrs, k, n, _stream_ptr(stream), _ptr(xy), _ptr(inf)))
    return [(xy[i].copy(), int(inf[i])) for i in range(k)]


def msm_g1_partial_dev(bases, scalars_tensor, n, stream=None):
    out = np.zeros(24, dtype=np.uint64)
    _chk(lib().zkp_msm_g1_partial_dev(bases._h, _dev_ptr(scalars_tensor, 32 * n), n, _stream_ptr(stream), _ptr(out)))
    return out


def g1_xyzz_sum(partials):
    partials = _np(partials, np.uint64, (-1, 24))
    out = np.zeros(12, dtype=np.uint64)
    inf = C.c_uint8(0)
    _chk(lib().zkp_g1_xyzz_sum(_ptr(partials), partials.shape[0], _ptr(out), C.byref(inf)))
    return out, int(inf.value)


def g1_mul(base_xy, base_inf, scalar):
    base_xy, scalar = _np(base_xy, np.uint64, (12,)), _np(scalar, np.uint64, (4,))
    out = np.zeros(12, dtype=np.uint64)
    inf = C.c_uint8(0)
    _chk(lib().zkp_g1_mul(_ptr(base_xy), int(base_inf), _ptr(scalar), _ptr(out), C.byref(inf)))
    return out, int(inf.value)


def g1_fixed_base_mul_dev(scalars_tensor, n, out_xy_tensor, out_inf_tensor=None, stream=None):
    inf = C.c_void_p(out_inf_tensor.data_ptr()) if out_inf_tensor is not None else None
    _chk(lib().zkp_g1_fixed_base_mul_dev(_dev_ptr(scalars_tensor, 32 * n), n, _dev_ptr(out_xy_tensor, 96 * n), inf,
                                         _stream_ptr(stream)))


def srs_g1(secret, n):
    secret = _np(secret, np.uint64, (4,))
    out = np.zeros((n, 12), dtype=np.uint64)
    _chk(lib().zkp_srs_g1(_ptr(secret), n, _ptr(out)))
    return out


def _log2(n):
    lg = int(n).bit_length() - 1
    if n <= 0 or (1 << lg) != n:
        raise ZkpError(ZKP_E_ARG, "size must be a power of two")
    return lg


def ntt_fr(data, inverse=False, coset=None):
    a = _np(data, np.uint64, (-1, 4)).copy()
    cs = _np(coset, np.uint64, (4,)) if coset is not None else None
    _chk(lib().zkp_ntt_fr(_ptr(a), _log2(a.shape[0]), int(bool(inverse)), _ptr(cs)))
    return a


def ntt_goldilocks(data, inverse=False, coset=None):
    a = _np(data, np.uint64).reshape(-1).copy()
    cs = _np(coset, np.uint64, (1,)) if coset is not None else None
    _chk(lib().zkp_ntt_goldilocks(_ptr(a), _log2(a.shape[0]), int(bool(inverse)), _ptr(cs)))
    return a


def ntt_fr_dev(tensor, log_n, batch=1, inverse=False, coset=None, stream=None):
    cs = _np(coset, np.uint64, (4,)) if coset is not None else None
    _chk(lib().zkp_ntt_fr_dev(_dev_ptr(tensor, (32 << log_n) * batch), log_n, batch, int(bool(inverse)), _ptr(cs),
                              _stream_ptr(stream)))


def ntt_fr_twiddle_dev(tensor, rows, cols, row0, log_n, inverse=False, stream=None):
    _chk(lib().zkp_ntt_fr_twiddle_dev(_dev_ptr(tensor, 32 * rows * cols), rows, cols, row0, log_n, int(bool(inverse)),
                                      _stream_ptr(stream)))


class NttLayout(C.Structure):
    _fields_ = [("lo_bits", C.c_uint), ("mid_bits", C.c_uint), ("mid_stride", C.c_size_t), ("hi_stride", C.c_size_t),
                ("batch_stride", C.c_size_t)]


def ntt_fr_axis0_dev(t_in, t_out, log_len, cols, inverse=False, tw_log_n=0, tw_col0=0, stream=None):
    nbytes = 32 * (cols << log_len)
    _chk(lib().zkp_ntt_fr_axis0_dev(_dev_ptr(t_in, nbytes), _dev_ptr(t_out, nbytes), log_len, cols, int(inverse), tw_log_n,
                                    tw_col0, _stream_ptr(stream)))


def ntt_fr_layout_dev(t_in, t_out, log_n, batch, inverse=False, in_layout=None, out_layout=None, tw_log_n=0, tw_row0=0,
                      stream=None):
    nbytes = 32 * (batch << log_n)
    li = C.byref(in_layout) if in_layout is not None else None
    lo = C.byref(out_layout) if out_layout is not None else None
    _chk(lib().zkp_ntt_fr_layout_dev(_dev_ptr(t_in, nbytes), _dev_ptr(t_out, nbytes), log_n, batch, int(inverse),
                                     C.cast(li, C.c_void_p) if li is not None else None,
                                     C.cast(lo, C.c_void_p) if lo is not None else None, tw_log_n, tw_row0, _stream_ptr(stream)))


NTT_NATURAL, NTT_K1SLAB, NTT_COLUMNS = 0, 1, 2


class NttShardGeometry(C.Structure):
    _fields_ = [("slots", C.c_uint), ("log_n1", C.c_uint), ("log_n2", C.c_uint), ("chunks", C.c_uint), ("r1", C.c_size_t),
                ("r2", C.c_size_t), ("cw", C.c_size_t), ("slab", C.c_size_t)]


def ntt_fr_sharded_geometry(log_n, slots=0, chunks=0):
    g = NttShardGeometry()
    _chk(lib().zkp_ntt_fr_sharded_geometry(log_n, slots, chunks, C.cast(C.byref(g), C.c_void_p)))
    return {k: int(getattr(g, k)) for k, _ in NttShardGeometry._fields_}


def ntt_fr_sharded_dev(slab_tensors, log_n, inverse=False, layout_in=NTT_NATURAL, layout_out=NTT_K1SLAB, chunks=0, streams=None):
    k = len(slab_tensors)
    nbytes = (32 << log_n) // k
    ptrs = (C.c_void_p * k)(*[_dev_ptr(t, nbytes).value for t in slab_tensors])
    sts = None
    if streams is not None:
        if len(streams) != k:
            raise ValueError("one stream per slot")
        sts = (C.c_void_p * k)(*[int(getattr(s, "cuda_stream", s)) for s in streams])
    _chk(lib().zkp_ntt_fr_sharded_dev(ptrs, log_n, int(bool(inverse)), layout_in, layout_out, chunks, sts))


def ntt_fr_sharded(data, inverse=False, coset=None, inplace=False):
    a = _np(data, np.uint64, (-1, 4))
    if not inplace:
        a = a.copy()
    cs = _np(coset, np.uint64, (4,)) if coset is not None else None
    _chk(lib().zkp_ntt_fr_sharded(_ptr(a), _log2(a.shape[0]), int(bool(inverse)), _ptr(cs)))
    return a


def ntt_goldilocks_dev(tensor, log_n, batch=1, inverse=False, coset=None, stream=None):
    cs = _np(coset, np.uint64, (1,)) if coset is not None else None
    _chk(lib().zkp_ntt_goldilocks_dev(_dev_ptr(tensor, (8 << log_n) * batch), log_n, batch, int(bool(inverse)),
                                      _ptr(cs), _stream_ptr(stream)))


def fri_layer_eval(coeffs, coset, log_d):
    coeffs = _np(coeffs, np.uint64).reshape(-1)
    out = np.zeros(1 << log_d, dtype=np.uint64)
    _chk(lib().zkp_fri_layer_eval(_ptr(coeffs), coeffs.size, int(coset), log_d, _ptr(out)))
    return out


def fri_fold(coeffs, r):
    coeffs = _np(coeffs, np.uint64).reshape(-1)
    out = np.zeros((coeffs.size + 1) // 2, dtype=np.uint64)
    _chk(lib().zkp_fri_fold(_ptr(coeffs), coeffs.size, int(r), _ptr(out)))
    return out


def fri_merkle_node_count(n):
    return int(lib().zkp_fri_merkle_node_count(n))


def fri_merkle_tree(leaves):
    leaves = _np(leaves, np.uint64).reshape(-1)
    out = np.zeros(fri_merkle_node_count(leaves.size), dtype=np.uint64)
    _chk(lib().zkp_fri_merkle_tree(_ptr(leaves), leaves.size, _ptr(out)))
    return out


def fri_merkle_tree_dev(leaves_tensor, n, nodes_tensor, stream=None):
    _chk(lib().zkp_fri_merkle_tree_dev(_dev_ptr(leaves_tensor, 8 * n), n, _dev_ptr(nodes_tensor, 8 * fri_merkle_node_count(n)),
                                       _stream_ptr(stream)))


def fri_challenges(roots, const_val, num_queries):
    roots = _np(roots, np.uint64).reshape(-1)
    r_out = np.zeros(roots.size, dtype=np.uint64)
    q_out = np.zeros(num_queries, dtype=np.uint64)
    _chk(lib().zkp_fri_challenges(_ptr(roots), roots.size, int(const_val), num_queries, _ptr(r_out), _ptr(q_out)))
    return r_out, q_out


def fri_prove(coeffs, blowup_factor, num_queries):
    coeffs = _np(coeffs, np.uint64).reshape(-1)
    p, words = C.c_void_p(), C.c_size_t()
    _chk(lib().zkp_fri_prove(_ptr(coeffs), coeffs.size, blowup_factor, num_queries, C.byref(p), C.byref(words)))
    try:
        return np.ctypeslib.as_array(C.cast(p, C.POINTER(C.c_uint64)), shape=(words.value,)).copy()
    finally:
        lib().zkp_free(p)


def fri_verify(proof):
    proof = _np(proof, np.uint64).reshape(-1)
    _chk(lib().zkp_fri_verify(_ptr(proof), proof.size))
    return True


def fri_layer_eval_fr(coeffs, coset, log_d):
    coeffs = _np(coeffs, np.uint64, (-1, 4))
    cs = _np(coset, np.uint64, (4,))
    out = np.zeros((1 << log_d, 4), dtype=np.uint64)
    _chk(lib().zkp_fri_layer_eval_fr(_ptr(coeffs), coeffs.shape[0], _ptr(cs), log_d, _ptr(out)))
    return out


def fri_fold_fr(coeffs, r):
    coeffs = _np(coeffs, np.uint64, (-1, 4))
    rr = _np(r, np.uint64, (4,))
    out = np.zeros(((coeffs.shape[0] + 1) // 2, 4), dtype=np.uint64)
    _chk(lib().zkp_fri_fold_fr(_ptr(coeffs), coeffs.shape[0], _ptr(rr), _ptr(out)))
    return out


def fri_merkle_tree_fr(leaves):
    leaves = _np(leaves, np.uint64, (-1, 4))
    out = np.zeros((fri_merkle_node_count(leaves.shape[0]), 4), dtype=np.uint64)
    _chk(lib().zkp_fri_merkle_tree_fr(_ptr(leaves), leaves.shape[0], _ptr(out)))
    return out


def fri_merkle_tree_fr_dev(leaves_tensor, n, nodes_tensor, stream=None):
    _chk(lib().zkp_fri_merkle_tree_fr_dev(_dev_ptr(leaves_tensor, 32 * n), n,
                                          _dev_ptr(nodes_tensor, 32 * fri_merkle_node_count(n)), _stream_ptr(stream)))


def fri_challenges_fr(roots, const_val, num_queries):
    roots = _np(roots, np.uint64, (-1, 4))
    cv = _np(const_val, np.uint64, (4,))
    r_out = np.zeros((roots.shape[0], 4), dtype=np.uint64)
    q_out = np.zeros(num_queries, dtype=np.uint64)
    _chk(lib().zkp_fri_challenges_fr(_ptr(roots), roots.shape[0], _ptr(cv), num_queries, _ptr(r_out), _ptr(q_out)))
    return r_out, q_out


def fri_prove_fr(coeffs, blowup_factor, num_queries):
    coeffs = _np(coeffs, np.uint64, (-1, 4))
    p, words = C.c_void_p(), C.c_size_t()
    _chk(lib().zkp_fri_prove_fr(_ptr(coeffs), coeffs.shape[0], blowup_factor, num_queries, C.byref(p), C.byref(words)))
    try:
        return np.ctypeslib.as_array(C.cast(p, C.POINTER(C.c_uint64)), shape=(words.value,)).copy()
    finally:
        lib().zkp_free(p)


def fri_verify_fr(proof):
    proof = _np(proof, np.uint64).reshape(-1)
    _chk(lib().zkp_fri_verify_fr(_ptr(proof), proof.size))
    return True


def g2_generator():
    out = np.zeros(24, dtype=np.uint64)
    _chk(lib().zkp_g2_generator(_ptr(out)))
    return out


def g2_mul(q_xy, scalar, q_is_inf=0):
    q = _np(q_xy, np.uint64).reshape(24)
    s = _np(scalar, np.uint64).reshape(4)
    out = np.zeros(24, dtype=np.uint64)
    inf = C.c_uint8(0)
    _chk(lib().zkp_g2_mul(_ptr(q), int(q_is_inf), _ptr(s), _ptr(out), C.byref(inf)))
    return out, int(inf.value)


def pairing(p_xy, q_xy, p_is_inf=0, q_is_inf=0):
    p = _np(p_xy, np.uint64).reshape(12)
    q = _np(q_xy, np.uint64).reshape(24)
    out = np.zeros((12, 6), dtype=np.uint64)
    _chk(lib().zkp_pairing(_ptr(p), int(p_is_inf), _ptr(q), int(q_is_inf), _ptr(out)))
    return out


def kzg_verify(g2s_xy, commitment, opening, y, z):
    acc = C.c_int(0)
    g2s = _np(g2s_xy, np.uint64).reshape(24)
    c, w = _np(commitment[0], np.uint64).reshape(12), _np(opening[0], np.uint64).reshape(12)
    yy, zz = _np(y, np.uint64).reshape(4), _np(z, np.uint64).reshape(4)
    _chk(lib().zkp_kzg_verify(_ptr(g2s), _ptr(c), int(commitment[1]), _ptr(w), int(opening[1]), _ptr(yy), _ptr(zz), C.byref(acc)))
    return bool(acc.value)


def kzg_batch_verify(g2s_xy, commitments, points, openings, evals, r_primes):
    g2s = _np(g2s_xy, np.uint64).reshape(24)
    cm, op = _np(commitments, np.uint64, (-1, 12)), _np(openings, np.uint64, (-1, 12))
    pts, ev, rp = _np(points, np.uint64, (-1, 4)), _np(evals, np.uint64, (-1, 4)), _np(r_primes, np.uint64, (-1, 4))
    acc = C.c_int(0)
    _chk(lib().zkp_kzg_batch_verify(_ptr(g2s), cm.shape[0], _ptr(cm), None, _ptr(pts), _ptr(op), None, _ptr(ev), _ptr(rp), C.byref(acc)))
    return bool(acc.value)


def kzg_aggregate_commitments(commitments, challenge, is_inf=None):
    cm = _np(commitments, np.uint64, (-1, 12))
    ch = _np(challenge, np.uint64).reshape(4)
    inf = _np(is_inf, np.uint8) if is_inf is not None else None
    out = np.zeros(12, dtype=np.uint64)
    oinf = C.c_uint8(0)
    _chk(lib().zkp_kzg_aggregate_commitments(_ptr(cm), _ptr(inf) if inf is not None else None, cm.shape[0], _ptr(ch), _ptr(out), C.byref(oinf)))
    return out, int(oinf.value)


# ... 192 lines not shown
```

Before: 446.1 million.

## Add wave-per-add row-parallel XYZZ pyramid kernel and fuse partstart into partprefix

Adds a row-parallel G1 XYZZ add in which a whole wave computes one point add: each 16-lane row holds one 28-bit-limb field element and multiplies with DPP broadcasts. This is used for small pyramid levels and for the tail kernel, replacing quad-per-add mapping, and aims to cut latency when there are few adds to spread across the GPU. It also merges the partstart kernel into partprefix using a last-block atomic counter, removing one launch. Tail block and half defaults change, profiling events move into hipExtLaunchKernelGGL, and a selftest entry point is added. The row path carries a scalar fallback for special cases and adds normalisation loops that could add overhead.

```diff
diff --git a/include/zkp_hip.h b/include/zkp_hip.h
--- a/include/zkp_hip.h
+++ b/include/zkp_hip.h
@@ -59,6 +59,7 @@
                uint8_t *out_is_inf);
 int zkp_g1_fixed_base_mul_dev(const void *d_scalars, size_t n, void *d_out_xy, uint8_t *d_out_is_inf, void *stream);
 int zkp_selftest_fq_inverse_dev(const void *d_in, size_t n, int form, void *d_out, void *stream);
+int zkp_selftest_fq28_row_dev(const void *d_a, const void *d_b, size_t n, int op, void *d_out, void *stream);
 int zkp_srs_g1(const uint64_t secret[4], size_t n, uint64_t *out_xy);
 
 int zkp_ntt_fr(uint64_t *data, unsigned log_n, int inverse, const uint64_t *coset );
diff --git a/rust/zkp-hip-sys/src/lib.rs b/rust/zkp-hip-sys/src/lib.rs
--- a/rust/zkp-hip-sys/src/lib.rs
+++ b/rust/zkp-hip-sys/src/lib.rs
@@ -109,6 +109,7 @@
     pub fn zkp_g1_mul(base_xy: *const u64, base_is_inf: u8, scalar: *const u64, out_xy: *mut u64, out_is_inf: *mut u8) -> i32;
     pub fn zkp_g1_fixed_base_mul_dev(d_scalars: *const c_void, n: usize, d_out_xy: *mut c_void, d_out_is_inf: *mut u8, stream: *mut c_void) -> i32;
     pub fn zkp_selftest_fq_inverse_dev(d_in: *const c_void, n: usize, form: i32, d_out: *mut c_void, stream: *mut c_void) -> i32;
+    pub fn zkp_selftest_fq28_row_dev(d_a: *const c_void, d_b: *const c_void, n: usize, op: i32, d_out: *mut c_void, stream: *mut c_void) -> i32;
     pub fn zkp_srs_g1(secret: *const u64, n: usize, out_xy: *mut u64) -> i32;
     pub fn zkp_ntt_fr(data: *mut u64, log_n: u32, inverse: i32, coset: *const u64) -> i32;
     pub fn zkp_ntt_fr_dev(d_data: *mut c_void, log_n: u32, batch: usize, inverse: i32, coset: *const u64, stream: *mut c_void) -> i32;
diff --git a/zkp-implementation_amd/build.py b/zkp-implementation_amd/build.py
--- a/zkp-implementation_amd/build.py
+++ b/zkp-implementation_amd/build.py
@@ -7,7 +7,7 @@
 SRC = os.path.join(HERE, "csrc")
 OUT = os.path.join(HERE, "libzkp_hip.so")
 SOURCES = ["api.hip"]
-DEPS = ["api.hip", "ff.hpp", "fq28.hpp", "fq28_inv.hpp", "fr29.hpp", "fr29_mul2_asm.inc", "fq28_mul_asm.inc", "fq28_mul2x_asm.inc", "fq28_sqr_asm.inc", "fq28_mul2_asm.inc", "g1.hpp", "g1_28.hpp", "msm.hpp", "ntt.hpp", "plonk.hpp",
+DEPS = ["api.hip", "ff.hpp", "fq28.hpp", "fq28_inv.hpp", "fr29.hpp", "fr29_mul2_asm.inc", "fq28_mul_asm.inc", "fq28_mul2x_asm.inc", "fq28_sqr_asm.inc", "fq28_mul2_asm.inc", "g1.hpp", "g1_28.hpp", "g1_28_row.hpp", "msm.hpp", "ntt.hpp", "plonk.hpp",
         "plonk_host.inc", "ntt_sharded.inc", "fri.hpp", "fri_host.inc", "fri_fr.hpp", "fri_fr_host.inc", "transcript_host.hpp", "pairing_host.hpp", "verify_host.inc", "host_ff.hpp", "kzg_host.hpp", "host_threads.hpp", "msm_plan.hpp", "msm_host.inc", "nova.hpp", "nova_host.inc", "dev_res.hpp",
         os.path.join("..", "..", "include", "zkp_hip.h")]
 
diff --git a/zkp-implementation_amd/csrc/api.hip b/zkp-implementation_amd/csrc/api.hip
--- a/zkp-implementation_amd/csrc/api.hip
+++ b/zkp-implementation_amd/csrc/api.hip
@@ -1,4 +1,5 @@
 #include <hip/hip_runtime.h>
+#include <hip/hip_ext.h>
 
 #include <algorithm>
 #include <array>
@@ -158,12 +159,13 @@
 struct ProfScope {
     ProfRec rec;
     hipStream_t st;
-    bool on;
-    ProfScope(const char* name, hipStream_t s, bool chain = false) : st(s), on(false) {
+    bool on, in_launch;
+    ProfScope(const char* name, hipStream_t s, bool chain = false, bool launch = false) : st(s), on(false), in_launch(false) {
         const int level = g_prof_on.load(std::memory_order_relaxed);
         on = level == 1 || (level == 2 && std::strcmp(name, "msm_accumulate") == 0);
         if (!on) return;
         if (level == 2) chain = false;
+        in_launch = launch && level == 2;
         rec.name = name;
         std::vector<ProfRec>& recs = prof_records();
         if (chain && !recs.empty() && recs.back().b && prof_last_stream() == s) {
@@ -173,11 +175,13 @@
         }
         if (rec.own_a.make(hipEventDefault) != hipSuccess || rec.b.make(hipEventDefault) != hipSuccess) { on = false; return; }
         rec.a = rec.own_a;
-        (void)hipEventRecord(rec.a, st);
-    }
+        if (!in_launch) (void)hipEventRecord(rec.a, st);
+    }
+    hipEvent_t start() const { return in_launch ? rec.a : nullptr; }
+    hipEvent_t stop() const { return in_launch ? (hipEvent_t)rec.b : nullptr; }
     ~ProfScope() {
         if (!on) return;
-        (void)hipEventRecord(rec.b, st);
+        if (!in_launch) (void)hipEventRecord(rec.b, st);
         prof_records().push_back(std::move(rec));
         prof_last_stream() = st;
     }
@@ -1608,6 +1612,18 @@
     return ZKP_OK;
 } ZKP_CATCH_INT
 
+int zkp_selftest_fq28_row_dev(const void* d_a, const void* d_b, size_t n, int op, void* d_out, void* stream) try {
+    if (n && (!d_a || !d_b || !d_out)) return fail(ZKP_E_ARG, "null argument");
+    if (op != 0 && op != 1) return fail(ZKP_E_ARG, "op must be 0 (product) or 1 (XYZZ add)");
+    if (n > 0x7fffffffu) return fail(ZKP_E_ARG, "n too large");
+    CTX_ENTER(-1);
+    if (!n) return ZKP_OK;
+    hipLaunchKernelGGL(fq28_row_selftest_kernel, dim3((unsigned)n), dim3(64), 0, reinterpret_cast<hipStream_t>(stream),
+                       static_cast<const uint4*>(d_a), static_cast<const uint4*>(d_b), static_cast<uint4*>(d_out), (uint64_t)n, op);
+    HIPCHK(hipGetLastError());
+    return ZKP_OK;
+} ZKP_CATCH_INT
+
 int zkp_srs_g1(const uint64_t secret[4], size_t n, uint64_t* out_xy) try {
     if (!secret || (n && !out_xy)) return fail(ZKP_E_ARG, "null argument");
     if (!n) return ZKP_OK;
diff --git a/zkp-implementation_amd/csrc/g1_28_row.hpp b/zkp-implementation_amd/csrc/g1_28_row.hpp
--- /dev/null
+++ b/zkp-implementation_amd/csrc/g1_28_row.hpp
@@ -0,0 +1,125 @@
+#pragma once
+#include "g1_28.hpp"
+
+namespace zkp {
+
+struct RowLane {
+    uint32_t k, mod, kp4, kp16, kp8w;
+    static ZKP_DEV RowLane make() {
+        RowLane r;
+        r.k = __lane_id() & 15;
+        const uint32_t i = r.k < NL28 ? r.k : 0;
+        const bool live = r.k < NL28;
+        r.mod = live ? Fq28C::MOD[i] : 0u;
+        r.kp4 = live ? Fq28C::KP4_29[i] : 0u;
+        r.kp16 = live ? Fq28C::KP16_29[i] : 0u;
+        r.kp8w = live ? Fq28C::KP8_30[i] : 0u;
+        return r;
+    }
+};
+
+ZKP_DEV uint32_t row_bcast(uint32_t v, int src) {
+#define ZKP_ROW_BC(I) case I: return (uint32_t)__builtin_amdgcn_mov_dpp((int)v, 0x150 + I, 0xf, 0xf, false);
+    switch (src) {
+        ZKP_ROW_BC(0) ZKP_ROW_BC(1) ZKP_ROW_BC(2) ZKP_ROW_BC(3) ZKP_ROW_BC(4) ZKP_ROW_BC(5) ZKP_ROW_BC(6)
+        ZKP_ROW_BC(7) ZKP_ROW_BC(8) ZKP_ROW_BC(9) ZKP_ROW_BC(10) ZKP_ROW_BC(11) ZKP_ROW_BC(12) default: ZKP_ROW_BC(13)
+    }
+#undef ZKP_ROW_BC
+}
+ZKP_DEV uint32_t row_from_next(uint32_t v) { return (uint32_t)__builtin_amdgcn_mov_dpp((int)v, 0x101, 0xf, 0xf, true); }
+ZKP_DEV uint32_t row_from_prev(uint32_t v) { return (uint32_t)__builtin_amdgcn_mov_dpp((int)v, 0x111, 0xf, 0xf, true); }
+ZKP_DEV uint64_t row_from_next64(uint64_t v) { return (uint64_t)row_from_next((uint32_t)v) | (uint64_t)row_from_next((uint32_t)(v >> 32)) << 32; }
+ZKP_DEV uint64_t row_from_prev64(uint64_t v) { return (uint64_t)row_from_prev((uint32_t)v) | (uint64_t)row_from_prev((uint32_t)(v >> 32)) << 32; }
+ZKP_DEV uint32_t rows_bcast(uint32_t v, int r) { return (uint32_t)__shfl((int)v, (int)(__lane_id() & 15) | (r << 4)); }
+ZKP_DEV uint32_t rows_xor1(uint32_t v) { return (uint32_t)__shfl_xor((int)v, 16); }
+ZKP_DEV uint32_t row_bits(bool pred, int r) { return (uint32_t)(__ballot(pred) >> (16 * r)) & 0xffffu; }
+
+ZKP_DEV uint32_t row_normalise64(uint64_t t, const RowLane& L) {
+    while (__ballot(L.k < NL28 - 1 && t > MASK28)) {
+        const uint64_t c = L.k < NL28 - 1 ? t >> 28 : 0;
+        if (L.k < NL28 - 1) t &= MASK28;
+        t += row_from_prev64(c);
+    }
+    return (uint32_t)t;
+}
+ZKP_DEV uint32_t row_normalise(uint32_t v, const RowLane& L) {
+    while (__ballot(L.k < NL28 - 1 && v > MASK28)) {
+        const uint32_t c = L.k < NL28 - 1 ? v >> 28 : 0;
+        if (L.k < NL28 - 1) v &= MASK28;
+        v += row_from_prev(c);
+    }
+    return v;
+}
+
+ZKP_DEV uint32_t fq28_mul_row(uint32_t a, uint32_t b, const RowLane& L) {
+    uint64_t t = 0;
+    const uint64_t lane0 = L.k == 0 ? ~0ull : 0ull;
+#pragma unroll
+    for (int i = 0; i < NL28; i++) {
+        t += (uint64_t)row_bcast(a, i) * b;
+        const uint32_t m = (row_bcast((uint32_t)t, 0) * Fq28C::INV) & MASK28;
+        t += (uint64_t)m * L.mod;
+        t = row_from_next64(t) + ((t >> 28) & lane0);
+    }
+    return row_normalise64(t, L);
+}
+
+ZKP_DEV uint32_t row_sub4(uint32_t a, uint32_t b, const RowLane& L) { return a + (L.kp4 - b); }
+ZKP_DEV uint32_t row_sub16(uint32_t a, uint32_t b, const RowLane& L) { return a + (L.kp16 - b); }
+ZKP_DEV uint32_t row_sub8w(uint32_t a, uint32_t b, const RowLane& L) { return a + (L.kp8w - b); }
+
+ZKP_DEV uint32_t row_load(const uint4* p, uint64_t stride, const RowLane& L) {
+    const uint32_t v = reinterpret_cast<const uint32_t*>(p + (L.k >> 2) * stride)[L.k & 3];
+    return L.k < NL28 ? v : 0u;
+}
+ZKP_DEV void row_store(uint4* p, uint64_t stride, uint32_t v, const RowLane& L) {
+    reinterpret_cast<uint32_t*>(p + (L.k >> 2) * stride)[L.k & 3] = L.k < NL28 ? v : 0u;
+}
+
+ZKP_DEV void g1_28_add_row(const uint4* srcA, const uint4* __restrict__ srcB, uint4* dst, uint64_t stride) {
+    const RowLane L = RowLane::make();
+    const int j = (int)(__lane_id() >> 4) & 3;
+    const bool odd = (j & 1) != 0, hi = (j & 2) != 0;
+    const uint4* mine = odd ? srcB : srcA;
+    const uint4* other = odd ? srcA : srcB;
+    const int zf = hi ? 12 : 8;
+    const uint32_t xy = row_load(mine + (hi ? 4 : 0) * stride, stride, L);
+    const uint32_t zo = row_load(other + zf * stride, stride, L);
+    const uint32_t zm = row_load(mine + zf * stride, stride, L);
+    const bool inf_a = row_bits(zm != 0, 0) == 0, inf_b = row_bits(zo != 0, 0) == 0;
+    const uint32_t m1 = fq28_mul_row(xy, zo, L);
+    const uint32_t d = row_sub4(rows_xor1(m1), m1, L);
+    const uint32_t m2 = fq28_mul_row(odd ? zo : d, odd ? zm : d, L);
+    const bool p_zero = row_bits(m2 != 0, 0) == 0 || row_bits(m2 != L.mod, 0) == 0;
+    if (inf_a || inf_b || p_zero) {
+        if (__lane_id() == 0) {
+            X28 a = X28::load_s(srcA, stride);
+            const X28 b = X28::load_s(srcB, stride);
+            g1_28_add(a, b);
+            a.store_s(dst, stride);
+        }
+        return;
+    }
+    const uint32_t pp = rows_bcast(m2, 0);
+    const uint32_t u1 = rows_bcast(m1, 0);
+    const uint32_t m3 = fq28_mul_row(hi ? u1 : (odd ? m2 : d), pp, L);
+    const uint32_t ppp = rows_bcast(m3, 0);
+    const uint32_t s1 = rows_bcast(m1, 2);
+    const uint32_t x3 = row_normalise(row_sub8w(row_sub4(m2, ppp, L), m3 + m3, L), L);
+    const uint32_t t = row_sub16(m3, x3, L);
+    const uint32_t lhs4 = hi ? (odd ? m2 : d) : s1;
+    const uint32_t rhs4 = (hi && !odd) ? t : ppp;
+    const uint32_t m4 = fq28_mul_row(lhs4, rhs4, L);
+    const uint32_t v = rows_bcast(m4, 0);
+    const uint32_t y3 = row_normalise(row_sub4(m4, v, L), L);
+    if (j == 2) {
+        row_store(dst, stride, x3, L);
+        row_store(dst + 4 * stride, stride, y3, L);
+    } else if (j == 1) {
+        row_store(dst + 8 * stride, stride, m3, L);
+    } else if (j == 3) {
+        row_store(dst + 12 * stride, stride, m4, L);
+    }
+}
+
+}
diff --git a/zkp-implementation_amd/csrc/msm.hpp b/zkp-implementation_amd/csrc/msm.hpp
--- a/zkp-implementation_amd/csrc/msm.hpp
+++ b/zkp-implementation_amd/csrc/msm.hpp
@@ -1,6 +1,7 @@
 #pragma once
 #include "g1.hpp"
 #include "g1_28.hpp"
+#include "g1_28_row.hpp"
 #include "fq28_inv.hpp"
 #include "msm_plan.hpp"
 
@@ -105,8 +106,11 @@
 }
 
 __global__ __launch_bounds__(1024) void msm_partprefix_kernel(uint32_t* __restrict__ cntA, MsmGeom g, SortGeom sg,
-                                                              uint32_t* __restrict__ tot) {
+                                                              uint32_t* __restrict__ tot, uint32_t* __restrict__ pstart,
+                                                              uint32_t* __restrict__ ghist, uint32_t* __restrict__ counters) {
     __shared__ uint32_t part[16][64];
+    __shared__ uint32_t t[SORT_MAX_PART + 1];
+    __shared__ bool last;
     const uint32_t w = blockIdx.y, h = threadIdx.x & 63, qg = threadIdx.x >> 6;
     const uint32_t hi = blockIdx.x * 64 + h;
     const bool live = hi < sg.nhi;
@@ -133,24 +137,29 @@
         }
         if (qg == 0) tot[(uint64_t)w * sg.nhi + hi] = total;
     }
-}
-
-__global__ __launch_bounds__(64) void msm_partstart_kernel(const uint32_t* __restrict__ tot, SortGeom sg,
-                                                           uint32_t* __restrict__ pstart, uint32_t* __restrict__ ghist,
-                                                           uint32_t* __restrict__ tail_barrier) {
-    __shared__ uint32_t t[SORT_MAX_PART + 1];
-    uint32_t* base = t;
-    const uint32_t w = blockIdx.x;
-    for (uint32_t k = threadIdx.x; k < 256; k += 64) {
+    __syncthreads();
+    uint32_t* ctr = counters + (uint64_t)w * PYR_BAR_STRIDE;
+    if (threadIdx.x == 0) {
+        __builtin_amdgcn_fence(__ATOMIC_RELEASE, "agent");
+        last = __hip_atomic_fetch_add(ctr + 1, 1u, __ATOMIC_RELAXED, __HIP_MEMORY_SCOPE_AGENT) == gridDim.x - 1;
+        if (last) {
+            __builtin_amdgcn_fence(__ATOMIC_ACQUIRE, "agent");
+            __hip_atomic_store(ctr + 1, 0u, __ATOMIC_RELAXED, __HIP_MEMORY_SCOPE_AGENT);
+        }
+    }
+    __syncthreads();
+    if (!last) return;
+    for (uint32_t k = threadIdx.x; k < 256; k += blockDim.x) {
         ghist[w * 256 + k] = 0;
-        ghist[(gridDim.x + w) * 256 + k] = 0;
-    }
-    if (threadIdx.x == 0) tail_barrier[w * PYR_BAR_STRIDE] = 0;
-    for (uint32_t k = threadIdx.x; k < sg.nhi; k += 64) t[k] = tot[(uint64_t)w * sg.nhi + k];
-    __syncthreads();
-    wave_exclusive_scan(t, base, sg.nhi, threadIdx.x);
-    __syncthreads();
-    for (uint32_t k = threadIdx.x; k <= sg.nhi; k += 64) pstart[(uint64_t)w * (sg.nhi + 1) + k] = base[k];
+        ghist[(gridDim.y + w) * 256 + k] = 0;
+    }
+    if (threadIdx.x == 0) ctr[0] = 0;
+    const uint32_t* tw = tot + (uint64_t)w * sg.nhi;
+    for (uint32_t k = threadIdx.x; k < sg.nhi; k += blockDim.x) t[k] = __hip_atomic_load(tw + k, __ATOMIC_RELAXED, __HIP_MEMORY_SCOPE_AGENT);
+    __syncthreads();
+    if (threadIdx.x < 64) wave_exclusive_scan(t, t, sg.nhi, threadIdx.x);
+    __syncthreads();
+    for (uint32_t k = threadIdx.x; k <= sg.nhi; k += blockDim.x) pstart[(uint64_t)w * (sg.nhi + 1) + k] = t[k];
 }
 
 #ifndef ZKP_BS_TILE
@@ -847,11 +856,26 @@
     g1_28_add_quad(src + it.a, src + it.b, (kind ? odd_out : pyr_out) + it.d, cap, j);
 }
 
+__global__ __launch_bounds__(MSM_THREADS) void msm_pyramid_row_kernel(const uint4* __restrict__ pyr_in,
+                                                                      uint4* pyr_out,
+                                                                      const uint4* __restrict__ odd_in,
+                                                                      uint4* __restrict__ odd_out, PyrLevel L) {
+    const uint32_t s = blockIdx.x * (MSM_THREADS / 64) + (threadIdx.x >> 6);
+    if (s >= L.half) return;
+    const uint32_t kind = blockIdx.y, w = blockIdx.z;
+    const uint64_t cap = (uint64_t)L.nwin * L.nb;
+    const PyrItem it = pyr_item(L.nb, L.level, L.half, kind, s, (uint64_t)w * L.nb);
+    const uint4* src = kind == 0 ? pyr_in : (it.src_is_pyr_out ? pyr_out : odd_in);
+    g1_28_add_row(src + it.a, src + it.b, (kind ? odd_out : pyr_out) + it.d, cap);
+}
+
 constexpr uint32_t MSM_TAIL_TIMEOUT = 0x80000000u;
 constexpr uint32_t MSM_FLAG_PENDING = 0x40000000u;
 constexpr uint32_t MSM_FLAG_PENDING_MASK = 0x40000000u;
 constexpr uint32_t PYR_TAIL_THREADS = 256;
-constexpr uint32_t PYR_TAIL_BLOCKS = 16;
+constexpr uint32_t PYR_TAIL_BLOCKS = 64;
+constexpr uint32_t PYR_TAIL_HALF = 16;
+constexpr uint32_t PYR_ROW_MAX_ADDS = 2048;
 constexpr uint32_t PYR_TAIL_SPIN_LIMIT = 1u << 24;
 __global__ __launch_bounds__(512) void msm_pyramid_tail_kernel(uint4* __restrict__ pyr0, uint4* __restrict__ pyr1,
                                                                uint4* __restrict__ odd0, uint4* __restrict__ odd1,
@@ -864,8 +888,7 @@
     const uint32_t w = blockIdx.y;
     const uint64_t wbase = (uint64_t)w * nb;
     const uint64_t cap = (uint64_t)gridDim.y * nb;
-    const int j = threadIdx.x & 3;
-    const uint32_t quad = blockIdx.x * (blockDim.x >> 2) + (threadIdx.x >> 2), nquad = gridDim.x * (blockDim.x >> 2);
+    const uint32_t wave = blockIdx.x * (blockDim.x >> 6) + (threadIdx.x >> 6), nwave = gridDim.x * (blockDim.x >> 6);
     uint32_t epoch = 0;
     for (uint32_t l = level0; l + 1 < c; l++) {
         const uint32_t half = nb >> (l + 1);
@@ -873,11 +896,11 @@
         uint4* pyr_out = (l & 1) ? pyr0 : pyr1;
         const uint4* odd_in = (l & 1) ? odd1 : odd0;
         uint4* odd_out = (l & 1) ? odd0 : odd1;
-        for (uint32_t item = quad; item < (l + 1) * half; item += nquad) {
+        for (uint32_t item = wave; item < (l + 1) * half; item += nwave) {
             const uint32_t kind = item / half, s = item % half;
             const PyrItem it = pyr_item(nb, l, half, kind, s, wbase);
             const uint4* src = kind == 0 ? pyr_in : (it.src_is_pyr_out ? pyr_out : odd_in);
-            g1_28_add_quad(src + it.a, src + it.b, (kind ? odd_out : pyr_out) + it.d, cap, j);
+            g1_28_add_row(src + it.a, src + it.b, (kind ? odd_out : pyr_out) + it.d, cap);
         }
         epoch++;
         __syncthreads();
@@ -932,6 +955,21 @@
     if (j == 0) __hip_atomic_store(flags + w, 0u, __ATOMIC_RELEASE, __HIP_MEMORY_SCOPE_SYSTEM);
 }
 
+__global__ __launch_bounds__(64) void fq28_row_selftest_kernel(const uint4* __restrict__ a, const uint4* __restrict__ b,
+                                                               uint4* __restrict__ out, uint64_t n, int op) {
+    const uint64_t i = blockIdx.x;
+    if (i >= n) return;
+    if (op == 0) {
+        const RowLane L = RowLane::make();
+        const uint32_t r = fq28_mul_row(row_load(a + 4 * i, 1, L), row_load(b + 4 * i, 1, L), L);
+        if (threadIdx.x < 16) row_store(out + 4 * i, 1, r, L);
+        if (threadIdx.x == 0) (Fq28::load(a + 4 * i) * Fq28::load(b + 4 * i)).store(out + 4 * (n + i));
+    } else {
+        g1_28_add_row(a + 16 * i, b + 16 * i, out + 16 * i, 1);
+        if (threadIdx.x < 4) g1_28_add_quad(a + 16 * i, b + 16 * i, out + 16 * (n + i), 1, (int)threadIdx.x);
+    }
+}
+
 __global__ __launch_bounds__(MSM_THREADS) void g1_fixed_base_kernel(const Fr* __restrict__ scalars, uint64_t n,
                                                                    const uint4* __restrict__ table,
                                                                    uint4* __restrict__ out_xy,
diff --git a/zkp-implementation_amd/csrc/msm_host.inc b/zkp-implementation_amd/csrc/msm_host.inc
--- a/zkp-implementation_amd/csrc/msm_host.inc
+++ b/zkp-implementation_amd/csrc/msm_host.inc
@@ -41,7 +41,10 @@
                  {"pyr1", &cx.pyr1, b.pyr1}, {"odd0", &cx.odd0, b.odd0}, {"odd1", &cx.odd1, b.odd1}, {"result", &cx.result, b.result}}};
     }
     int grow() {
+        const void* const result_was = cx.result.p;
+        const size_t result_cap_was = cx.result.cap;
         for (const auto& [name, buf, bytes] : buffers()) ZCHK(buf->ensure(bytes));
+        if (cx.result.p != result_was || cx.result.cap != result_cap_was) HIPCHK(hipMemsetAsync(cx.result.p, 0, cx.result.cap, st));
         ZCHK(cx.host_result.ensure(p.bytes.host_result, hipHostMallocPortable | hipHostMallocMapped));
         ptot = cx.counts.get() + W * g.nchunk * nhi;
         pstart = ptot + W * nhi;
@@ -153,9 +156,9 @@
         ProfScope ps("msm_sort", sst, true);
         hipLaunchKernelGGL(msm_parthist_kernel, dim3(g.nchunk, g.nwin), dim3(1024), 0, sst, cx.digits.get(), g, sg, cx.counts.get());
         MSM_TRACE(sst, ridx, "parthist");
-        hipLaunchKernelGGL(msm_partprefix_kernel, dim3((sg.nhi + 63) / 64, g.nwin), dim3(1024), 0, sst, cx.counts.get(), g, sg, ptot);
-        hipLaunchKernelGGL(msm_partstart_kernel, dim3(g.nwin), dim3(64), 0, sst, ptot, sg, pstart, ghist, cx.result.get());
-        MSM_TRACE(sst, ridx, "partprefix + partstart");
+        hipLaunchKernelGGL(msm_partprefix_kernel, dim3((sg.nhi + 63) / 64, g.nwin), dim3(1024), 0, sst, cx.counts.get(), g, sg, ptot, pstart,
+                           ghist, cx.result.get());
+        MSM_TRACE(sst, ridx, "partprefix");
         switch (partscatter_tile(sg.nhi)) {
             case PS_TILE_SMALL: launch_partscatter<PS_TILE_SMALL>(); break;
             case PS_TILE_MID: launch_partscatter<PS_TILE_MID>(); break;
@@ -172,7 +175,7 @@
     }
 
     void launch_accumulate(const RangeBuffers& rb, uint64_t off, size_t ridx) {
-        ProfScope ps("msm_accumulate", st, true);
+        ProfScope ps("msm_accumulate", st, true, true);
         const bool quad = !g.resume && !g.more && (uint64_t)g.n * g.nwin <= (1ull << 20);
         const uint32_t per_block = quad ? ACC_THREADS / 4 : ACC_THREADS;
         const uint32_t bucket_blocks = (uint32_t)((((uint64_t)g.nb << g.split_log) + per_block - 1) / per_block);
@@ -181,28 +184,32 @@
         const uint4* xy = static_cast<const uint4*>(bases->d_xy.p) + off * 8;
         uint4 *buckets = cx.buckets.get(), *pieces = cx.pieces.get(), *parts = cx.parts.get(), *carry = cx.pyr1.get();
         if (quad)
-            hipLaunchKernelGGL(msm_accumulate_quad_kernel, grid, dim3(ACC_THREADS), 0, st, xy, rb.sorted, rb.start, rb.perm, rb.over, rb.desc,
-                               p.desc_cap, bucket_blocks, extra_blocks, g, buckets, pieces, parts, clk_record(CLK_MSM_ACCUMULATE));
+            hipExtLaunchKernelGGL(msm_accumulate_quad_kernel, grid, dim3(ACC_THREADS), 0, st, ps.start(), nullptr, 0, xy, rb.sorted, rb.start,
+                                  rb.perm, rb.over, rb.desc, p.desc_cap, bucket_blocks, extra_blocks, g, buckets, pieces, parts,
+                                  clk_record(CLK_MSM_ACCUMULATE));
         else
-            hipLaunchKernelGGL(msm_accumulate_kernel, grid, dim3(ACC_THREADS), 0, st, xy, rb.sorted, rb.start, rb.perm, rb.over, rb.desc,
-                               p.desc_cap, bucket_blocks, extra_blocks, g, buckets, pieces, parts, carry, clk_record(CLK_MSM_ACCUMULATE));
+            hipExtLaunchKernelGGL(msm_accumulate_kernel, grid, dim3(ACC_THREADS), 0, st, ps.start(), nullptr, 0, xy, rb.sorted, rb.start, rb.perm,
+                                  rb.over, rb.desc, p.desc_cap, bucket_blocks, extra_blocks, g, buckets, pieces, parts, carry,
+                                  clk_record(CLK_MSM_ACCUMULATE));
         MSM_TRACE(st, ridx, "accumulate");
-        hipLaunchKernelGGL(msm_combine_kernel, dim3(std::min<uint32_t>(p.over_cap, 64), g.nwin), dim3(64), 0, st, rb.over, rb.over_b,
-                           rb.over_off, p.over_cap, p.desc_cap, g, pieces, buckets, carry);
+        hipExtLaunchKernelGGL(msm_combine_kernel, dim3(std::min<uint32_t>(p.over_cap, 64), g.nwin), dim3(64), 0, st, nullptr,
+                              g.split_log ? nullptr : ps.stop(), 0, rb.over, rb.over_b, rb.over_off, p.over_cap, p.desc_cap, g, pieces,
+                              buckets, carry);
         MSM_TRACE(st, ridx, "combine");
         const uint64_t cap = (uint64_t)g.nwin * g.nb;
         static const uint64_t lane_from = getenv("ZKP_FOLD_LANE_MIN") ? strtoull(getenv("ZKP_FOLD_LANE_MIN"), nullptr, 10) : FOLD_LANE_MIN_ADDS;
         for (uint32_t t = 0; t < g.split_log; t++) {
             const unsigned pairs = 1u << (g.split_log - 1 - t), per = cap * pairs >= lane_from ? MSM_THREADS : MSM_THREADS / 4;
-            hipLaunchKernelGGL(per == MSM_THREADS ? msm_fold_parts_lane_kernel : msm_fold_parts_kernel, dim3((unsigned)((cap + per - 1) / per), pairs),
-                               dim3(MSM_THREADS), 0, st, buckets, parts, cap, t);
+            hipExtLaunchKernelGGL(per == MSM_THREADS ? msm_fold_parts_lane_kernel : msm_fold_parts_kernel, dim3((unsigned)((cap + per - 1) / per), pairs),
+                                  dim3(MSM_THREADS), 0, st, nullptr, t + 1 == g.split_log ? ps.stop() : nullptr, 0, buckets, parts, cap, t);
         }
     }
 
     int reduce() {
         static const uint32_t tail_threads = getenv("ZKP_PYR_TAIL_THREADS") ? (uint32_t)atoi(getenv("ZKP_PYR_TAIL_THREADS")) : PYR_TAIL_THREADS;
         static const uint32_t tail_blocks = getenv("ZKP_PYR_TAIL_BLOCKS") ? (uint32_t)atoi(getenv("ZKP_PYR_TAIL_BLOCKS")) : PYR_TAIL_BLOCKS;
-        static const uint32_t tail_half = getenv("ZKP_PYR_TAIL_HALF") ? (uint32_t)atoi(getenv("ZKP_PYR_TAIL_HALF")) : 64u;
+        static const uint32_t tail_half = getenv("ZKP_PYR_TAIL_HALF") ? (uint32_t)atoi(getenv("ZKP_PYR_TAIL_HALF")) : PYR_TAIL_HALF;
+        static const uint64_t row_max = getenv("ZKP_PYR_ROW_MAX") ? strtoull(getenv("ZKP_PYR_ROW_MAX"), nullptr, 10) : PYR_ROW_MAX_ADDS;
         if (tail_threads < 64 || tail_threads > 512 || (tail_threads & 63) || !tail_blocks || tail_blocks > 256 || !tail_half)
             return fail(ZKP_E_ARG, "ZKP_PYR_TAIL_THREADS must be a multiple of 64 up to 512, ZKP_PYR_TAIL_BLOCKS 1..256, ZKP_PYR_TAIL_HALF >= 1");
         for (size_t w = 0; w < W; w++) __atomic_store_n(result_flags + w, MSM_FLAG_PENDING, __ATOMIC_RELEASE);
@@ -215,10 +222,12 @@
         if ((uint64_t)g.nwin * (tail_threads / 64) > max_waves) level_tail = g.c - 1;
         for (uint32_t l = 0; l < level_tail; l++) {
             const PyrLevel L{l, g.nb >> (l + 1), g.nb, g.nwin};
-            const bool quad = (uint64_t)L.half * (l + 1) * g.nwin <= (1u << 16);
-            const uint32_t per = quad ? MSM_THREADS / 4 : MSM_THREADS;
-            hipLaunchKernelGGL(quad ? msm_pyramid_quad_kernel : msm_pyramid_kernel, dim3((L.half + per - 1) / per, l + 1, g.nwin),
-                               dim3(MSM_THREADS), 0, st, pyr[l & 1], pyr[(l + 1) & 1], odd[l & 1], odd[(l + 1) & 1], L);
+            const uint64_t adds = (uint64_t)L.half * (l + 1) * g.nwin;
+            const bool row = adds <= row_max, quad = adds <= (1u << 16);
+            const uint32_t per = row ? MSM_THREADS / 64 : quad ? MSM_THREADS / 4 : MSM_THREADS;
+            hipLaunchKernelGGL(row ? msm_pyramid_row_kernel : quad ? msm_pyramid_quad_kernel : msm_pyramid_kernel,
+                               dim3((L.half + per - 1) / per, l + 1, g.nwin), dim3(MSM_THREADS), 0, st, pyr[l & 1], pyr[(l + 1) & 1],
+                               odd[l & 1], odd[(l + 1) & 1], L);
         }
         if (level_tail + 1 < g.c) {
             uint32_t tb = tail_blocks;
diff --git a/zkp-implementation_amd/zkp_hip/__init__.py b/zkp-implementation_amd/zkp_hip/__init__.py
--- a/zkp-implementation_amd/zkp_hip/__init__.py
+++ b/zkp-implementation_amd/zkp_hip/__init__.py
@@ -54,6 +54,7 @@
     "zkp_g1_mul": ([_VP, C.c_uint8, _VP, _VP, _VP], C.c_int),
     "zkp_g1_fixed_base_mul_dev": ([_VP, _SZ, _VP, _U8P, _VP], C.c_int),
     "zkp_selftest_fq_inverse_dev": ([_VP, _SZ, C.c_int, _VP, _VP], C.c_int),
+    "zkp_selftest_fq28_row_dev": ([_VP, _VP, _SZ, C.c_int, _VP, _VP], C.c_int),
     "zkp_srs_g1": ([_VP, _SZ, _VP], C.c_int),
     "zkp_ntt_fr": ([_VP, C.c_uint, C.c_int, _VP], C.c_int),
     "zkp_ntt_fr_dev": ([_VP, C.c_uint, _SZ, C.c_int, _VP, _VP], C.c_int),
@@ -318,6 +319,12 @@
                                            _stream_ptr(stream)))
 
 
+def selftest_fq28_row_dev(a_tensor, b_tensor, n, op, out_tensor, stream=None):
+    words = 16 if op == 0 else 64
+    _chk(lib().zkp_selftest_fq28_row_dev(_dev_ptr(a_tensor, 4 * words * n), _dev_ptr(b_tensor, 4 * words * n), n, op,
+                                         _dev_ptr(out_tensor, 8 * words * n), _stream_ptr(stream)))
+
+
 def msm_g1_dev(bases, scalars_tensor, n, stream=None):
     out = np.zeros(12, dtype=np.uint64)
     inf = C.c_uint8(0)
```

Result: no change. 448.9 million (median of 6 runs) (+0.6%).
